# facebook/facebook360_dep

Hardware: AMD Instinct MI355X
Metric: depth Mpix/s per GPU (full pyramid, 16-cam 2048^2 rig); % HBM-read roofline (higher is better)
Workload: dtype f32+f64; 1 GPU; BASELINE config 3: 16-camera 2048x2048 synthetic rig, 8-frame sequence, full 10-level pyramid per frame, per-level temporal filter (+-2 frames); the same sequence for every --gpus N (block partition, 8 frame(s) on this rank); rig=cfg2, cameras=16, frames=8, temporal_filter=True, halo_transport=local, parallelism=frames x1

## Files before the change

__graft_entry__.py:

```python
import os
import subprocess
import sys

ROOT = os.path.dirname(os.path.abspath(__file__))
CSRC = os.path.join(ROOT, "facebook360_dep_amd", "csrc")
LIB = os.path.join(ROOT, "facebook360_dep_amd", "libderp_hip.so")
HIPCC = os.environ.get("HIPCC", "/opt/rocm/bin/hipcc")
HIP_FLAGS = ["--offload-arch=gfx950", "-O3", "-std=c++17", "-ffp-contract=off", "-fno-slp-vectorize", "-fPIC", "-shared"]


def _stale(target, sources):
    if not os.path.exists(target):
        return True
    t = os.path.getmtime(target)
    return any(os.path.getmtime(s) > t for s in sources)


def build_hip(force=False):
    srcs = [os.path.join(CSRC, f) for f in ("derp_capi.hip", "derp_host.h", "derp_ctx.h", "derp_kernels.h", "derp_render.h", "derp_points.h", "derp_mesh.h", "derp_mesh_math.h", "derp_camera.h", "gcc_algos.h", "derp_render_api.h", "derp_rephoto_api.h", "derp_points_api.h", "derp_mesh_api.h", "derp_filters_api.h", "derp_debug_api.h", "derp_sequence.h", "derp_isp.h", "derp_sim.h", "derp_sim_math.h", "derp_geometric.h", "derp_geometric_api.h", "derp_sweep.h", "derp_sweep_api.h", "derp_align.h", "derp_align_api.h")]
    srcs.append(os.path.join(ROOT, "include", "derp_hip.h"))
    host = os.path.join(CSRC, "derp_images.cpp")
    simplify = os.path.join(CSRC, "derp_simplify.cpp")
    scene = os.path.join(CSRC, "derp_sim_scene.cpp")
    srcs += [host, simplify, scene, os.path.join(ROOT, "facebook360_dep_amd", "cli", "image_codecs.h")]
    if force or _stale(LIB, srcs):
        subprocess.check_call([HIPCC] + HIP_FLAGS + ["-o", LIB, os.path.join(CSRC, "derp_capi.hip"), host, simplify, scene, "-lz", "-ldl"])
    cli = os.path.join(ROOT, "facebook360_dep_amd", "cli")
    if os.path.isdir(cli) and os.path.exists(os.path.join(cli, "Makefile")):
        subprocess.check_call(["make", "-s", "-C", cli])
    return LIB


def build():
    build_hip()
    sys.path.insert(0, ROOT)
    from oracle import oracle_lib

    oracle_lib.build()
    import facebook360_dep_amd
    from facebook360_dep_amd import derp

    derp.lib()


def smoke():
    sys.path.insert(0, ROOT)
    import numpy as np

    from facebook360_dep_amd import derp, synth
    from tests import common

    n, res, widths = synth.config("tiny")
    rig = synth.make_rig(n, res)
    sizes = synth.level_sizes(res, res, widths)
    frame = synth.make_frame(rig, sizes)
    ref = common.oracle_pyramid(rig, sizes, frame, res, res, partial_coverage=True)
    g = derp.Derp(rig["cameras"], partial_coverage=1)
    print("smoke: device", g.device_name())
    g.set_pyramid(sizes, res, res)
    g.upload_frame(frame)
    g.process_pyramid()
    g.synchronize()
    worst = 0.0
    for d in range(n):
        got = g.download_disparity(0, d)
        bad, rel = common.compare_disparity(got, ref[0][d])
        worst = max(worst, rel)
        assert bad == 0, "smoke: %d pixels of camera %d differ from the oracle by more than 1e-4 relative" % (bad, d)
    print("smoke: OK, max relative disparity error vs oracle = %.3g" % worst)
    g.close()


if __name__ == "__main__":
    build()
    if len(sys.argv) > 1 and sys.argv[1] == "smoke":
        smoke()
```

facebook360_dep_amd/csrc/derp_capi.hip:

```cpp
#include <hip/hip_runtime.h>

#include <algorithm>
#include <cfloat>
#include <cmath>
#include <cstdarg>
#include <cstdio>
#include <cstdlib>
#include <cstring>
#include <map>
#include <memory>
#include <string>
#include <vector>

#include <rocprim/device/device_radix_sort.hpp>

#include "../../include/derp_hip.h"
#include "derp_host.h"
#include "derp_kernels.h"
#include "derp_mesh.h"
#include "derp_points.h"
#include "derp_render.h"
#include "derp_geometric.h"
#include "derp_sweep.h"
#include "derp_align.h"

using namespace derp;

#include "derp_ctx.h"

namespace {

struct Span {
  derp_ctx* c;
  int stage, level;
  hipEvent_t a = nullptr, b = nullptr;
  Span(derp_ctx* ctx, int st, int lv) : c(ctx), stage(st), level(lv) {
    if (c->profiling) {
      (void)hipEventCreate(&a);
      (void)hipEventCreate(&b);
      (void)hipEventRecord(a, c->stream);
    }
  }
  ~Span() {
    if (c->profiling && a) {
      (void)hipEventRecord(b, c->stream);
      c->spans.push_back({stage, level, a, b});
    }
  }
};

void drain_spans(derp_ctx* c) {
  for (auto& s : c->spans) {
    (void)hipEventSynchronize(s.b);
    float ms = 0;
    (void)hipEventElapsedTime(&ms, s.a, s.b);
    if (s.level >= 0 && s.level < kMaxLevels) {
      c->accMs[s.stage][s.level] += ms;
      c->accLaunch[s.stage][s.level] += 1;
    }
    (void)hipEventDestroy(s.a);
    (void)hipEventDestroy(s.b);
  }
  c->spans.clear();
}

size_t npx(const derp_ctx* c, int level) {
  return (size_t)c->LW[level] * c->LH[level];
}

unsigned long long* counter_slot(derp_ctx* c, int stage, int level) {
  return c->counters.as<unsigned long long>() + ((size_t)stage * kMaxLevels + level) * 4;
}

LevelView make_view(derp_ctx* c, int stage, int dst0, int nd) {
  LevelView V;
  const int L = c->cur;
  V.W = c->LW[L];
  V.H = c->LH[L];
  V.Wd = (double)V.W;
  V.Hd = (double)V.H;
  V.S = c->S;
  V.D = nd;
  V.level = L;
  V.numLevels = c->numLevels;
  V.dst0 = dst0;
  V.hasFg = c->opt.use_foreground_masks;
  const float scale = float(V.W) / c->heightFull;
  const float scaleVar = scale * scale;
  V.varNoiseFloor = std::max(c->opt.var_noise_floor * scaleVar, kMinVar);
  V.varHighThresh = c->opt.var_high_thresh;
  V.minDepthM = c->opt.min_depth_m;
  V.maxDepthM = c->opt.max_depth_m;
  V.randomProposals = c->opt.random_proposals;
  V.partialCoverage = c->opt.partial_coverage;
  V.xcdRotate = c->xcdRotate;
  V.camsSrc = c->camsSrc.as<Cam>();
  V.camsDst = c->camsDst.as<Cam>();
  V.dst2src = c->dst2src.as<int>();
  V.srcColor = c->frame().color[L].as<ushort4>();
  V.ownBias = c->w.ownBias.as<ushort4>();
  V.srcVar = c->w.srcVar.as<float>();
  V.srcFg = c->frame().fg[L].as<uint8_t>();
  V.rayDir = c->rayDir.as<double>();
  V.behind = c->behind.as<unsigned>();
  V.rayStride = (size_t)c->D * V.W * V.H;
  V.projWarp = c->projWarp.as<float2>();
  V.projColor = c->w.projColor.as<ushort4>();
  V.projBias = c->w.projBias.as<ushort4>();
  V.projColorT = c->w.projColorT.as<ushort4>();
  V.disparity = c->w.disparity.as<float>();
  V.cost = c->w.cost.as<float>();
  V.confidence = c->w.confidence.as<float>();
  V.bgDisp = c->frame().bg[L].as<float>();
  V.fovMask = c->fovMask.as<uint8_t>();
  V.pairCount = c->w.pairCount.as<uint8_t>();
  V.counters = counter_slot(c, stage, L);
#if DERP_BLOCK_TRACE
  V.blockTrace = nullptr;
#endif
  return V;
}
int block_trace_attach(derp_ctx* c, LevelView& V, int which, int gridX, int gridY) {
#if DERP_BLOCK_TRACE
  DevBuf& buf = c->blockTrace[which][V.level];
  const size_t bytes = (size_t)gridX * gridY * 2 * sizeof(unsigned long long);
  ALLOC(c, buf, bytes);
  HIPCHK(c, hipMemsetAsync(buf.as<unsigned long long>(), 0, bytes, c->stream));
  V.blockTrace = buf.as<unsigned long long>();
  c->blockTraceGrid[which][V.level][0] = gridX;
  c->blockTraceGrid[which][V.level][1] = gridY;
#else
  (void)c, (void)V, (void)which, (void)gridX, (void)gridY;
#endif
  return 0;
}

const dim3 kBlurBlk(64, 4, 1);
dim3 blur_grid(int ow, int oh, int planes) {
  return dim3((ow + 63) / 64, (oh + 4 * kBlurRows - 1) / (4 * kBlurRows), planes);
}

void lanczos_coeffs(float x, float* coeffs) {
  static const double s45 = 0.70710678118654752440084436210485;
  static const double cs[][2] = {{1, 0}, {-s45, -s45}, {0, 1}, {s45, -s45}, {-1, 0}, {s45, s45}, {0, -1}, {-s45, s45}};
  if (x < 1.1920928955078125e-07f) {
    for (int i = 0; i < 8; i++) {
      coeffs[i] = 0;
    }
    coeffs[3] = 1;
    return;
  }
  float sum = 0;
  const double y0 = -(x + 3) * M_PI * 0.25, s0 = std::sin(y0), c0 = std::cos(y0);
  for (int i = 0; i < 8; i++) {
    const double y = -(x + 3 - i) * M_PI * 0.25;
    coeffs[i] = (float)((cs[i][0] * s0 + cs[i][1] * c0) / (y * y));
    sum += coeffs[i];
  }
  sum = 1.f / sum;
  for (int i = 0; i < 8; i++) {
    coeffs[i] *= sum;
  }
}

int get_lanczos(derp_ctx* c, int ssize, int dsize, LanczosTab** out) {
  auto key = std::make_pair(ssize, dsize);
  auto it = c->lanczos.find(key);
  if (it != c->lanczos.end()) {
    *out = &it->second;
    return 0;
  }
  std::vector<int> ofs(dsize);
  std::vector<float> coef((size_t)dsize * 8);
  const double scale = (double)ssize / dsize;
  for (int d = 0; d < dsize; ++d) {
    float f = (float)((d + 0.5) * scale - 0.5);
    int s = (int)f;
    s -= (s > f);
    f -= s;
    ofs[d] = s;
    lanczos_coeffs(f, &coef[(size_t)d * 8]);
  }
  LanczosTab t;
  for (int d0 = 0; d0 < dsize; d0 += kLanczosH) {
    const int d1 = std::min(d0 + kLanczosH, dsize) - 1;
    const int lo = std::min(std::max(ofs[d0] - 3, 0), ssize - 1), hi = std::min(std::max(ofs[d1] + 4, 0), ssize - 1);
    t.tileSpan = std::max(t.tileSpan, hi - lo + 1);
    t.monotone = t.monotone && std::is_sorted(ofs.begin() + d0, ofs.begin() + d1 + 1);
  }
  ALLOC(c, t.ofs, ofs.size() * sizeof(int));
  ALLOC(c, t.coef, coef.size() * sizeof(float));
  HIPCHK(c, hipMemcpyAsync(t.ofs.p, ofs.data(), ofs.size() * sizeof(int), hipMemcpyHostToDevice, c->stream));
  HIPCHK(c, hipMemcpyAsync(t.coef.p, coef.data(), coef.size() * sizeof(float), hipMemcpyHostToDevice, c->stream));
  HIPCHK(c, hipStreamSynchronize(c->stream));
  *out = &(c->lanczos[key] = std::move(t));
  return 0;
}

int get_area_tab(derp_ctx* c, int ssize, int dsize, AreaTabDev** out, bool forceTable = false) {
  auto key = std::make_pair(forceTable ? -ssize : ssize, dsize);
  auto it = c->areaTabs.find(key);
  if (it != c->areaTabs.end()) {
    *out = &it->second;
    return 0;
  }
  AreaTabDev t;
  const double scale = (double)ssize / dsize;
  const int iscale = (int)std::nearbyint(scale);
  std::vector<int> start(dsize + 1, 0), si;
  std::vector<float> alpha;
  if (!forceTable && iscale >= 1 && std::abs(scale - iscale) < 2.220446049250313e-16) {
    t.iscale = iscale;
  } else {
    for (int dx = 0; dx < dsize; ++dx) {
      start[dx] = (int)si.size();
      const double fsx1 = dx * scale, fsx2 = fsx1 + scale;
      const double cellWidth = std::min(scale, ssize - fsx1);
      int sx1 = (int)std::ceil(fsx1), sx2 = (int)std::floor(fsx2);
      sx2 = std::min(sx2, ssize - 1);
      sx1 = std::min(sx1, sx2);
      if (sx1 - fsx1 > 1e-3) {
        si.push_back(sx1 - 1);
        alpha.push_back((float)((sx1 - fsx1) / cellWidth));
      }
      for (int sx = sx1; sx < sx2; ++sx) {
        si.push_back(sx);
        alpha.push_back(float(1.0 / cellWidth));
      }
      if (fsx2 - sx2 > 1e-3) {
        si.push_back(sx2);
        alpha.push_back((float)(std::min(std::min(fsx2 - sx2, 1.), cellWidth) / cellWidth));
      }
    }
    start[dsize] = (int)si.size();
  }
  if (si.empty()) {
    si.push_back(0);
    alpha.push_back(0.f);
  }
  ALLOC(c, t.start, start.size() * sizeof(int));
  ALLOC(c, t.si, si.size() * sizeof(int));
  ALLOC(c, t.alpha, alpha.size() * sizeof(float));
  HIPCHK(c, hipMemcpy(t.start.p, start.data(), start.size() * sizeof(int), hipMemcpyHostToDevice));
  HIPCHK(c, hipMemcpy(t.si.p, si.data(), si.size() * sizeof(int), hipMemcpyHostToDevice));
  HIPCHK(c, hipMemcpy(t.alpha.p, alpha.data(), alpha.size() * sizeof(float), hipMemcpyHostToDevice));
  *out = &(c->areaTabs[key] = std::move(t));
  return 0;
}

int resize_area_dev(derp_ctx* c, int kind, const void* src, int sw, int sh, void* dst, int dw, int dh, int threshold) {
  if (dw > sw || dh > sh) {
    if (kind < 2 || kind == 4) {
      return fail(c, "pyramid levels must not be larger than the full-size frame (%dx%d -> %dx%d)", sw, sh, dw, dh);
    }
    const dim3 g = grid2d(dw, dh, 1, kBlk2d);
    if (kind == 3) {
      hipLaunchKernelGGL(k_resize_linear_area_f32<3>, g, kBlk2d, 0, c->stream, (const float*)src, sw, sh, (float*)dst, dw, dh);
    } else {
      hipLaunchKernelGGL(k_resize_linear_area_f32<1>, g, kBlk2d, 0, c->stream, (const float*)src, sw, sh, (float*)dst, dw, dh);
    }
    KCHECK(c);
    return 0;
  }
  AreaTabDev *tx, *ty;
  TRY(get_area_tab(c, sw, dw, &tx));
  TRY(get_area_tab(c, sh, dh, &ty));
  if ((tx->iscale > 0) != (ty->iscale > 0)) {
    if (tx->iscale > 0) {
      TRY(get_area_tab(c, sw, dw, &tx, true));
    } else {
      TRY(get_area_tab(c, sh, dh, &ty, true));
    }
  }
  AreaAxis ax{tx->start.as<int>(), tx->si.as<int>(), tx->alpha.as<float>(), tx->iscale};
  AreaAxis ay{ty->start.as<int>(), ty->si.as<int>(), ty->alpha.as<float>(), ty->iscale};
  const dim3 g = grid2d(dw, dh, 1, kBlk2d);
  if (kind == 0) {
    hipLaunchKernelGGL(k_resize_area<0>, g, kBlk2d, 0, c->stream, src, sw, sh, dst, dw, dh, ax, ay, threshold);
  } else if (kind == 1) {
    hipLaunchKernelGGL(k_resize_area<1>, g, kBlk2d, 0, c->stream, src, sw, sh, dst, dw, dh, ax, ay, threshold);
  } else if (kind == 3) {
    hipLaunchKernelGGL(k_resize_area<3>, g, kBlk2d, 0, c->stream, src, sw, sh, dst, dw, dh, ax, ay, threshold);
  } else if (kind == 4) {
    hipLaunchKernelGGL(k_resize_area<4>, g, kBlk2d, 0, c->stream, src, sw, sh, dst, dw, dh, ax, ay, threshold);
  } else {
    hipLaunchKernelGGL(k_resize_area<2>, g, kBlk2d, 0, c->stream, src, sw, sh, dst, dw, dh, ax, ay, threshold);
  }
  KCHECK(c);
  return 0;
}

std::vector<int2> make_spiral(int w) {
  int x = 0, y = 0, dx = 0, dy = -1, t = w;
  const int samples = t * t;
  std::vector<int2> locs;
  for (int i = 0; i < samples; ++i) {
    const bool vx = (-w / 2 <= x) && (x <= w / 2), vy = (-w / 2 <= y) && (y <= w / 2);
    if (vx && vy) {
      locs.push_back(make_int2(x, y));
    }
    if (x == y || ((x < 0) && (x == -y)) || ((x > 0) && (x == 1 - y))) {
      t = dx;
      dx = -dy;
      dy = t;
    }
    x += dx;
    y += dy;
  }
  return locs;
}

int ensure_spiral(derp_ctx* c, int radius) {
  if (c->spiralRadius == radius) {
    return 0;
  }
  const std::vector<int2> s = make_spiral(radius * 2 + 1);
  ALLOC(c, c->spiral, s.size() * sizeof(int2));
  HIPCHK(c, hipMemcpy(c->spiral.p, s.data(), s.size() * sizeof(int2), hipMemcpyHostToDevice));
  c->spiralN = (int)s.size();
  c->spiralRadius = radius;
  return 0;
}

int upsample_lanczos_dev(derp_ctx* c, const float* in, int sw, int sh, float* out, int dw, int dh, int planes,
                         size_t inStride, size_t outStride) {
  if (sw == dw && sh == dh) {
    return fail(c, "upsample to identical size not supported");
  }
  LanczosTab *tx, *ty;
  TRY(get_lanczos(c, sw, dw, &tx));
  TRY(get_lanczos(c, sh, dh, &ty));
  if (ty->monotone && ty->tileSpan <= kLanczosRows) {
    hipLaunchKernelGGL(k_lanczos, dim3((dw + kLanczosW - 1) / kLanczosW, (dh + kLanczosH - 1) / kLanczosH, planes),
                       dim3(kLanczosW, 4), 0, c->stream, in, sw, sh, dw, dh, tx->ofs.as<int>(), tx->coef.as<float>(),
                       ty->ofs.as<int>(), ty->coef.as<float>(), out, inStride, outStride);
    KCHECK(c);
    return 0;
  }
  const size_t tmpStride = (size_t)dw * sh;
  ALLOC(c, c->w.lanczosTmp, tmpStride * planes * sizeof(float));
  hipLaunchKernelGGL(k_lanczos_h, grid2d(dw, sh, planes, kBlk2d), kBlk2d, 0, c->stream, in, sw, sh, dw,
                     tx->ofs.as<int>(), tx->coef.as<float>(), c->w.lanczosTmp.as<float>(), inStride, tmpStride);
  KCHECK(c);
  hipLaunchKernelGGL(k_lanczos_v, grid2d(dw, dh, planes, kBlk2d), kBlk2d, 0, c->stream, c->w.lanczosTmp.as<float>(), sh,
                     dw, dh, ty->ofs.as<int>(), ty->coef.as<float>(), out, tmpStride, outStride);
  KCHECK(c);
  return 0;
}

int upsample_masked_dev(derp_ctx* c, const float* in, const uint8_t* mask, int sw, int sh, const uint8_t* maskUp,
                        const float* bgUp, float* out, int dw, int dh, int planes = 1) {
  const float scale = float(dw) / float(sw);
  const int radius = (int)(scale * scale + 1);
  TRY(ensure_spiral(c, radius));
  ALLOC(c, c->w.lanczosTmp, (size_t)dw * dh * planes * sizeof(float));
  hipLaunchKernelGGL(k_upsample_nearest_masked, grid2d(dw, dh, planes, kBlk2d), kBlk2d, 0, c->stream, in, mask, sw, sh,
                     maskUp, dw, dh, c->w.lanczosTmp.as<float>());
  KCHECK(c);
  hipLaunchKernelGGL(k_spiral_fill, grid2d(dw, dh, planes, kBlk2d), kBlk2d, 0, c->stream, c->w.lanczosTmp.as<float>(), bgUp,
                     maskUp, dw, dh, c->spiral.as<int2>(), c->spiralN, out);
  KCHECK(c);
  return 0;
}

bool batch_needs_inverse_warps(const derp_ctx* c, int dst0, int nd) {
  std::vector<char> covered(c->S, 0);
  for (int d = dst0; d < dst0 + nd; ++d) {
    covered[c->dst2srcH[d]] = 1;
  }
  for (int s = 0; s < c->S; ++s) {
    if (!covered[s]) {
      return true;
    }
  }
  return false;
}

size_t table_bytes_per_dst(const derp_ctx* c, int W, int H, bool withInverse) {
  const size_t wp = (size_t)(W + 2 * kPadW) * (H + 2 * kPadW), cp = (size_t)(W + 2 * kPadC) * (H + 2 * kPadC);
  return (size_t)(c->S - 1) * (wp * sizeof(float2) + 2 * cp * sizeof(ushort4) + (withInverse ? (size_t)W * H * sizeof(float2) : 0) +
                               (DERP_RANDOM_TILED ? tiled_plane(W, H) * sizeof(ushort4) : 0));
}

int compute_fov_and_masks(derp_ctx* c, int level) {
  const int W = c->LW[level], H = c->LH[level];
  const size_t n = (size_t)W * H;
  {
    Span sp(c, ST_FOV, level);
    if (c->opt.rebuild_warp_tables || c->fovCachedLevel != level) {
      hipLaunchKernelGGL(k_fov_mask, grid2d(W, H, c->D, kBlk2d), kBlk2d, 0, c->stream, c->camsDst.as<Cam>(), W, H,
                         c->fovMask.as<uint8_t>());
      KCHECK(c);
      c->fovCachedLevel = level;
    }
    hipLaunchKernelGGL(k_and_masks, dim3(flat_grid(n), c->D), dim3(256), 0, c->stream, c->fovMask.as<uint8_t>(),
                       c->frame().fg[level].as<uint8_t>(), c->dst2src.as<int>(), 0, n, c->w.maskAnd.as<uint8_t>());
    KCHECK(c);
  }
  return 0;
}

int build_warp(derp_ctx* c, int dst0, int nd) {
  const int L = c->cur;
  Span sp(c, ST_PROJ_WARP, L);
  {
    const size_t n = (size_t)c->LW[L] * c->LH[L];
    ALLOC(c, c->rayDir, 3 * n * c->D * sizeof(double));
    ALLOC(c, c->behind, n * c->D * sizeof(unsigned));
  }
  LevelView V = make_view(c, ST_PROJ_WARP, dst0, nd);
  hipLaunchKernelGGL(k_proj_warp, grid2d(V.W + 2 * kPadW, V.H + 2 * kPadW, c->S, kBlk2d), kBlk2d, 0, c->stream, V,
                     c->projWarp.as<float2>());
  KCHECK(c);
  hipLaunchKernelGGL(k_pixel_rays, grid2d(V.W, V.H, nd, kBlk2d), kBlk2d, 0, c->stream, V, c->rayDir.as<double>(),
                     c->behind.as<unsigned>());
  KCHECK(c);
  c->w.colorTablesCleanLevel = -1;
  if (batch_needs_inverse_warps(c, dst0, nd)) {
    hipLaunchKernelGGL(k_proj_warp_inv, grid2d(V.W, V.H, nd, kBlk2d), kBlk2d, 0, c->stream, V, c->projWarpInv.as<float2>());
    KCHECK(c);
  }
  return 0;
}

int build_color_tables(derp_ctx* c, int dst0, int nd) {
  const int L = c->cur;
  LevelView V = make_view(c, ST_REPROJECT, dst0, nd);
  Span sp(c, ST_REPROJECT, L);
  const dim3 grid((V.W + kRbTile - 1) / kRbTile, (V.H + kRbTile - 1) / kRbTile, nd * (c->S - 1));
  ALLOC(c, c->w.tileSeen, (size_t)grid.x * grid.y * grid.z);
  const int skipBlank = c->w.colorTablesCleanLevel == L && nd == c->D && !c->noBlankSkip;
  const auto kernel = c->reprojectSerial ? k_reproject_bias : k_reproject_bias_front;
  hipLaunchKernelGGL(kernel, grid, dim3(256), 0, c->stream, V, c->projWarpInv.as<float2>(),
                     c->w.projColor.as<ushort4>(), c->w.projBias.as<ushort4>(), c->w.projColorT.as<ushort4>(),
                     c->w.tileSeen.as<uint8_t>(), skipBlank);
  KCHECK(c);
  c->w.colorTablesCleanLevel = nd == c->D ? L : -1;
  return 0;
}

int tiles_of(int W, int H, int& tilesX) {
  constexpr int B = kTileBlock;
  tilesX = ((W + 15) / 16 + B - 1) / B * B;
  const int tilesY = ((H + 15) / 16 + B - 1) / B * B;
  return tilesX * tilesY * (256 / kCostBlock);
}
constexpr size_t kCostLdsPerSrc = (size_t)kCostBlock * sizeof(SsdPair);
struct CostGrid {
  int blocks, bands, perBlock;
};
constexpr int kCostMaxBands = 4, kCostMaxTilesPerBlock = 4;
int cost_grid_blocks(int tiles, int bands, int perBlock) {
  const int items = (tiles + perBlock - 1) / perBlock, unit = 8 * bands;
  return (items + unit - 1) / unit * unit;
}
CostGrid cost_grid(const derp_ctx* c, int tiles, int tilesX, bool spread) {
  const auto pow2_floor = [](int v, int cap) {
    int p = 1;
    while (p * 2 <= std::min(v, cap)) {
      p *= 2;
    }
    return p;
  };
  CostGrid g;
  g.perBlock = c->costTilesPerBlock > 0 ? pow2_floor(c->costTilesPerBlock, kCostMaxTilesPerBlock) : 1;
  const int rowOfSquares = tilesX * (256 / kCostBlock) * kTileBlock;
  g.bands = c->xcdBands > 0 ? pow2_floor(c->xcdBands, kCostMaxBands)
                            : spread ? pow2_floor(std::max(1, tiles / (8 * rowOfSquares)), kCostMaxBands) : 1;
  g.blocks = cost_grid_blocks(tiles, g.bands, g.perBlock);
  return g;
}
size_t lds_for_waves(size_t needed, int waves, size_t ldsPerCu, size_t fixed) {
  if (waves <= 0 || waves >= 4) {
    return needed;
  }
  const size_t perBlock = ldsPerCu / (size_t)(4 * waves + 1) + 256;
  return std::max(needed, perBlock > fixed ? perBlock - fixed : needed);
}
constexpr size_t kCostLdsStatic = sizeof(PatchWin) * (kCostBlock / 64) + kAtanLutDoubles * sizeof(double);
bool cost_four_waves(const derp_ctx* c) {
  if (const char* e = getenv("DERP_COST_WAVES")) {
    return atoi(e) >= 4;
  }
  return 16 * (kCostLdsPerSrc * (size_t)c->S + kCostLdsStatic) <= c->ldsPerCu && c->S <= 16;
}

int run_brute_force(derp_ctx* c, int dst0, int nd) {
  const int L = c->cur;
  if (L != c->numLevels - 1) {
    return 0;
  }
  Span sp(c, ST_BRUTE, L);
  LevelView V = make_view(c, ST_BRUTE, dst0, nd);
  const size_t n = (size_t)V.W * V.H;
  ALLOC(c, c->w.bruteCost, (size_t)nd * kNumDepths * n * sizeof(float));
  ALLOC(c, c->w.bruteConf, (size_t)nd * kNumDepths * n * sizeof(float));
  const int tilesX = std::max(1, (V.W - 2 + 7) / 8), tilesY = std::max(1, (V.H - 2 + 7) / 8);
  const int tiles = tilesX * tilesY;
  const size_t lds = kCostLdsPerSrc * (size_t)(c->S);
  const int run = std::min(std::max(c->bruteRun, 1), kNumDepths);
  hipLaunchKernelGGL(k_brute_costs, dim3(tiles, (kNumDepths + run - 1) / run, nd), dim3(kCostBlock), lds, c->stream, V,
                     c->w.bruteCost.as<float>(), c->w.bruteConf.as<float>(), tilesX, tiles, run);
  KCHECK(c);
  hipLaunchKernelGGL(k_brute_select, grid2d(V.W, V.H, nd, kBlk2d), kBlk2d, 0, c->stream, V, c->w.bruteCost.as<float>(),
                     c->w.bruteConf.as<float>());
  KCHECK(c);
  hipLaunchKernelGGL(k_brute_margin, grid2d(V.W, V.H, nd, kBlk2d), kBlk2d, 0, c->stream, V);
  KCHECK(c);
  return 0;
}

int run_random_proposals(derp_ctx* c, int dst0, int nd) {
  const int L = c->cur;
  if (c->opt.random_proposals <= 0 || L == c->numLevels - 1) {
    return 0;
  }
  Span sp(c, ST_RANDOM, L);
  c->randomRanThisLevel = true;
  LevelView V = make_view(c, ST_RANDOM, dst0, nd);
  if (V.H > 2 && V.W > 2) {
    WorkSet& w = c->w;
    if (w.rankPowersP != V.randomProposals || w.rankPowersN < V.W) {
      const int count = *std::max_element(c->LW.begin(), c->LW.end());
      ALLOC(c, w.rankPowers, (size_t)count * sizeof(uint32_t));
      hipLaunchKernelGGL(k_minstd_powers, dim3(blocks_of(count, 256)), dim3(256), 0, c->stream, V.randomProposals, count,
                         w.rankPowers.as<uint32_t>());
      KCHECK(c);
      w.rankPowersP = V.randomProposals;
      w.rankPowersN = count;
    }
    hipLaunchKernelGGL(k_row_rank, dim3(V.H - 2, nd), dim3(256), 0, c->stream, V, w.rankPowers.as<uint32_t>(),
                       w.rank.as<int>());
    KCHECK(c);
  }
  int tilesX;
  const int tiles = tiles_of(V.W, V.H, tilesX);
  const size_t lds = lds_for_waves(kCostLdsPerSrc * (size_t)(c->S), c->randomWaves, c->ldsPerCu, kCostLdsStatic);
  const CostGrid cg = cost_grid(c, tiles, tilesX, true);
  TRY(block_trace_attach(c, V, 0, cg.blocks, nd));
  const bool four = cost_four_waves(c);
  const auto kernel = cg.perBlock > 1 ? (four ? k_random_proposals_walk : k_random_proposals_walk_w3)
                                      : (four ? k_random_proposals : k_random_proposals_w3);
  hipLaunchKernelGGL(kernel, dim3(cg.blocks, nd), dim3(kCostBlock), lds, c->stream, V, c->w.rank.as<int>(), tilesX, cg.bands, cg.perBlock);
  KCHECK(c);
  return 0;
}

int run_ping_pong(derp_ctx* c, int dst0, int nd) {
  const int L = c->cur;
  if (L == c->numLevels - 1) {
    return 0;
  }
  Span sp(c, ST_PINGPONG, L);
  LevelView V = make_view(c, ST_PINGPONG, dst0, nd);
  const size_t n = (size_t)V.W * V.H;
  int tilesX;
  const int tiles = tiles_of(V.W, V.H, tilesX);
  const size_t lds = lds_for_waves(kCostLdsPerSrc * (size_t)(c->S), c->ppWaves, c->ldsPerCu, kCostLdsStatic);
  const bool four = cost_four_waves(c);
  const CostGrid cg = cost_grid(c, tiles, tilesX, false);
  const auto kernel = cg.perBlock > 1
                          ? (c->ppCompact ? (four ? k_ping_pong_walk : k_ping_pong_walk_w3) : (four ? k_ping_pong_loop_walk : k_ping_pong_loop_walk_w3))
                          : (c->ppCompact ? (four ? k_ping_pong : k_ping_pong_w3) : (four ? k_ping_pong_loop : k_ping_pong_loop_w3));
  TRY(block_trace_attach(c, V, 1, cg.blocks, nd));
  float* dispBuf[2] = {c->w.disparity.as<float>(), c->w.dispRes.as<float>()};
  float* costBuf[2] = {c->w.cost.as<float>(), c->w.costRes.as<float>()};
  uint8_t* chgBuf[2] = {c->w.changed.as<uint8_t>(), c->w.changed.as<uint8_t>() + n * c->D};
  const int iterations = c->opt.ping_pong_iterations;
  for (int it = 1; it <= iterations; ++it) {
    const int from = (it - 1) & 1, to = it & 1;
    V.disparity = dispBuf[from];
    V.cost = costBuf[from];
    hipLaunchKernelGGL(kernel, dim3(cg.blocks, nd), dim3(kCostBlock), lds, c->stream, V,
                       it == 1 ? (const uint8_t*)nullptr : chgBuf[from], chgBuf[to], dispBuf[to], costBuf[to], tilesX,
                       (int)(it == 1 && c->randomRanThisLevel && !c->noMemo), cg.bands, cg.perBlock);
    KCHECK(c);
  }
  if (dst0 + nd >= c->D) {
    if (iterations > 0 && (iterations & 1)) {
      std::swap(c->w.disparity, c->w.dispRes);
      std::swap(c->w.cost, c->w.costRes);
    }
    c->randomRanThisLevel = false;
  }
  return 0;
}

int run_mismatches(derp_ctx* c) {
  const int L = c->cur;
  if (L > c->opt.mismatches_start_level || L == c->numLevels - 1) {
    return 0;
  }
  if (c->D != c->S) {
    return fail(c, "Check failed: rigDst.size() == rigSrc.size()  Mismatches only valid when considering all cameras");
  }
  for (int d = 0; d < c->D; ++d) {
    if (c->dst2srcH[d] != d) {
      return fail(c, "mismatch handling needs destinations in rig order (dst %d maps to src %d)", d, c->dst2srcH[d]);
    }
  }
  Span sp(c, ST_MISMATCH, L);
  c->randomRanThisLevel = false;
  LevelView V = make_view(c, ST_MISMATCH, 0, c->D);
  const size_t n = (size_t)V.W * V.H;
  hipLaunchKernelGGL(k_mismatch, dim3((V.W + 15) / 16, (V.H + 15) / 16, c->D), dim3(256), 256 * sizeof(float) * c->S,
                     c->stream, V, c->w.dispRes.as<float>(), c->w.mismatchMask.as<uint8_t>());
  KCHECK(c);
  HIPCHK(c, hipMemcpyAsync(c->w.disparity.p, c->w.dispRes.p, n * c->D * sizeof(float), hipMemcpyDeviceToDevice, c->stream));
  return 0;
}

int bilateral_radius(int level) {
  const float scale = std::pow(0.9f, level);
  return (int)std::max(std::ceil(5 * scale), float(1));
}

size_t bilateral_lds_bytes(int radius) {
  const size_t side = 16 + 2 * (size_t)radius;
  const size_t t = ((side + 15) & ~(size_t)15) * side;
  return t * 4 * sizeof(float) + ((t + 3) & ~(size_t)3);
}

constexpr size_t kBilateralMaxLds = 64 * 1024 - 256;

bool bilateral_fast_tap_ok(float sigma, float w0, float w1, float w2) {
  const float denom = 2.0f * (sigma * sigma);
  return w1 == 1.0f && w2 == 1.0f && w0 >= 0.0f && std::isfinite(w0) && denom > 0.0f && std::isfinite(denom);
}

bool temporal_fast_tap_ok(float sigma, float w0, float w1, float w2) {
  const float sig2 = sigma * sigma;
  const auto weight_ok = [](float w) { return w >= 0.0f && std::isfinite(w); };
  return weight_ok(w0) && weight_ok(w1) && weight_ok(w2) && sig2 > 0.0f && std::isfinite(sig2);
}

void launch_joint_bilateral_u16_tiled(derp_ctx* c, dim3 grid, const float* image, const void* guide, const uint8_t* mask,
                                      int W, int H, int radius, float sigma, float w0, float w1, float w2, float* out,
                                      size_t planeStride, size_t guideStride, const int* guideIndex) {
  const bool fast = bilateral_fast_tap_ok(sigma, w0, w1, w2) && bilateral_lds_bytes(radius) + 256 <= kBilateralMaxLds;
  const auto kernel = fast ? k_joint_bilateral<true, true> : k_joint_bilateral<true, false>;
  hipLaunchKernelGGL(kernel, grid, dim3(256), bilateral_lds_bytes(radius), c->stream, image, guide, mask, W, H, radius, sigma,
                     w0, w1, w2, out, planeStride, guideStride, guideIndex);
}

int run_bilateral(derp_ctx* c) {
  const int L = c->cur;
  Span sp(c, ST_BILATERAL, L);
  c->randomRanThisLevel = false;
  const int W = c->LW[L], H = c->LH[L];
  const size_t n = (size_t)W * H;
  const int radius = bilateral_radius(L);
  launch_joint_bilateral_u16_tiled(c, dim3((W + 15) / 16, (H + 15) / 16, c->D), c->w.disparity.as<float>(),
                                   (const void*)c->frame().color[L].as<ushort4>(), c->w.maskAnd.as<uint8_t>(), W, H, radius,
                                   0.005f, 0.5f, 1.0f, 1.0f, c->w.tmpF.as<float>(), n, n, c->dst2src.as<int>());
  KCHECK(c);
  std::swap(c->w.disparity, c->w.tmpF);
  return 0;
}

int run_median(derp_ctx* c, bool fuseMaskFov, float* levelOut = nullptr) {
  const int L = c->cur;
  Span sp(c, ST_MEDIAN, L);
  c->randomRanThisLevel = false;
  const int W = c->LW[L], H = c->LH[L];
  const size_t n = (size_t)W * H;
  hipLaunchKernelGGL(k_masked_median, grid2d(W, H, c->D, kBlk2d), kBlk2d, 0, c->stream, c->w.disparity.as<float>(),
                     c->opt.use_foreground_masks ? c->frame().bg[L].as<float>() : (const float*)nullptr,
                     c->w.maskAnd.as<uint8_t>(), W, H, 1, levelOut ? levelOut : c->w.tmpF.as<float>(), n,
                     fuseMaskFov ? c->fovMask.as<uint8_t>() : (const uint8_t*)nullptr);
  KCHECK(c);
  if (!levelOut) {
    std::swap(c->w.disparity, c->w.tmpF);
  }
  return 0;
}

int run_mask_fov(derp_ctx* c, float* levelOut = nullptr) {
  const int L = c->cur;
  Span sp(c, ST_MASKFOV, L);
  const size_t n = npx(c, L) * c->D;
  hipLaunchKernelGGL(k_mask_fov, dim3(flat_grid(n)), dim3(256), 0, c->stream, c->w.disparity.as<float>(),
                     c->fovMask.as<uint8_t>(), levelOut ? levelOut : c->w.disparity.as<float>(), n);
  KCHECK(c);
  return 0;
}

int check_level(derp_ctx* c, int level) {
  if (!c || c->numLevels == 0) {
    return fail(c, "derp_set_pyramid has not been called");
  }
  if (level < 0 || level >= c->numLevels) {
    return fail(c, "level %d out of range [0, %d)", level, c->numLevels);
  }
  if (c->LW[level] <= 0 || c->LH[level] <= 0) {
    return fail(c, "level %d was declared absent in derp_set_pyramid", level);
  }
  return 0;
}

int level_begin(derp_ctx* c, int level, bool buildAllTables) {
  TRY(check_level(c, level));
  if (c->S - 1 > kMaxSrc) {
    return fail(c, "too many source cameras (%d > %d)", c->S, kMaxSrc + 1);
  }
  c->cur = level;
  const int W = c->LW[level], H = c->LH[level];
  const size_t n = (size_t)W * H;
  if (W < 3 || H < 3) {
    return fail(c, "level %d is too small (%dx%d)", level, W, H);
  }
  TRY(compute_fov_and_masks(c, level));
  {
    Span sp(c, ST_VARIANCE, level);
    hipLaunchKernelGGL(k_variance_bias, blur_grid(W, H, c->S), kBlurBlk, 0, c->stream, c->frame().color[level].as<ushort4>(),
                       W, H, c->w.srcVar.as<float>(), c->w.ownBias.as<ushort4>());
    KCHECK(c);
  }
  HIPCHK(c, hipMemsetAsync(c->w.cost.p, 0, n * c->D * sizeof(float), c->stream));
  HIPCHK(c, hipMemsetAsync(c->w.confidence.p, 0, n * c->D * sizeof(float), c->stream));
  c->w.mismatchMaskHeld = level <= c->opt.mismatches_start_level && level != c->numLevels - 1;
  if (c->w.mismatchMaskHeld) {
    HIPCHK(c, hipMemsetAsync(c->w.mismatchMask.p, 0, n * c->D, c->stream));
  }
  if (level < c->numLevels - 1 && !c->frame().haveDisp[level + 1] && !buildAllTables) {
    return fail(c, "Missing disparity of level %d needed to start level %d", level + 1, level);
  }
  if (level < c->numLevels - 1 && c->frame().haveDisp[level + 1]) {
    Span sp(c, ST_UPSAMPLE, level);
    const int sw = c->LW[level + 1], sh = c->LH[level + 1];
    if (!c->opt.use_foreground_masks) {
      TRY(upsample_lanczos_dev(c, c->frame().disp[level + 1].as<float>(), sw, sh, c->w.disparity.as<float>(), W, H, c->D,
                               (size_t)sw * sh, n));
    } else {
      ALLOC(c, c->w.staging, (size_t)sw * sh * c->D);
      hipLaunchKernelGGL(k_fov_mask, grid2d(sw, sh, c->D, kBlk2d), kBlk2d, 0, c->stream, c->camsDst.as<Cam>(), sw, sh,
                         c->w.staging.as<uint8_t>());
      KCHECK(c);
      hipLaunchKernelGGL(k_and_masks, dim3(flat_grid((size_t)sw * sh), c->D), dim3(256), 0, c->stream,
                         c->w.staging.as<uint8_t>(), c->frame().fg[level + 1].as<uint8_t>(), c->dst2src.as<int>(), 0,
                         (size_t)sw * sh, c->w.staging.as<uint8_t>());
      KCHECK(c);
      TRY(upsample_masked_dev(c, c->frame().disp[level + 1].as<float>(), c->w.staging.as<uint8_t>(), sw, sh,
                              c->w.maskAnd.as<uint8_t>(), c->frame().bg[level].as<float>(), c->w.disparity.as<float>(), W, H, c->D));
    }
  } else {
    HIPCHK(c, hipMemsetAsync(c->w.disparity.p, 0, n * c->D * sizeof(float), c->stream));
  }
  const bool invAll = batch_needs_inverse_warps(c, 0, c->D);
  size_t per = table_bytes_per_dst(c, W, H, invAll);
  int DB = c->D;
  bool needInv = invAll;
  {
    const size_t wpAll = (size_t)(W + 2 * kPadW) * (H + 2 * kPadW) * (c->S - 1) * c->D * sizeof(float2);
    const size_t cpAll = (size_t)(W + 2 * kPadC) * (H + 2 * kPadC) * (c->S - 1) * c->D * sizeof(ushort4);
    const size_t ipAll = (size_t)W * H * (c->S - 1) * c->D * sizeof(float2);
    const bool resident = c->projWarp.bytes >= wpAll && c->w.projColor.bytes >= cpAll && c->w.projBias.bytes >= cpAll &&
        (!invAll || c->projWarpInv.bytes >= ipAll) && !getenv("DERP_TABLE_BUDGET_GB") &&
        (!DERP_RANDOM_TILED || c->w.projColorT.bytes >= tiled_plane(W, H) * (c->S - 1) * c->D * sizeof(ushort4));
    if (!resident) {
      size_t freeB = 0, totalB = 0;
      HIPCHK(c, hipMemGetInfo(&freeB, &totalB));
      size_t budget = freeB + c->projWarp.bytes + c->w.projColor.bytes + c->w.projBias.bytes + c->projWarpInv.bytes + c->w.projColorT.bytes;
      if (const char* e = getenv("DERP_TABLE_BUDGET_GB")) {
        budget = std::min<size_t>(budget, (size_t)(atof(e) * (1ull << 30)));
      } else {
        budget = (size_t)(budget * 0.85);
      }
      DB = (int)std::min<size_t>((size_t)c->D, budget / std::max<size_t>(per, 1));
      if (DB < c->D && !needInv) {
        needInv = true;
        per = table_bytes_per_dst(c, W, H, true);
        DB = (int)std::min<size_t>((size_t)c->D, budget / std::max<size_t>(per, 1));
      }
      if (DB < 1) {
        return fail(c, "projection tables for one destination (%zu bytes) exceed the table budget (%zu bytes)", per, budget);
      }
      const int batches = (c->D + DB - 1) / DB;
      DB = (c->D + batches - 1) / batches;
    }
  }
  c->DB = DB;
  const size_t wp = (size_t)(W + 2 * kPadW) * (H + 2 * kPadW), cp = (size_t)(W + 2 * kPadC) * (H + 2 * kPadC);
  ALLOC(c, c->projWarp, (size_t)DB * (c->S - 1) * wp * sizeof(float2));
  ALLOC(c, c->w.projColor, (size_t)DB * (c->S - 1) * cp * sizeof(ushort4));
  ALLOC(c, c->w.projBias, (size_t)DB * (c->S - 1) * cp * sizeof(ushort4));
  if (needInv) {
    ALLOC(c, c->projWarpInv, (size_t)DB * (c->S - 1) * n * sizeof(float2));
  }
  if (DERP_RANDOM_TILED) {
    ALLOC(c, c->w.projColorT, (size_t)DB * (c->S - 1) * tiled_plane(W, H) * sizeof(ushort4));
  }
  c->tablesValid = false;
  c->randomRanThisLevel = false;
  if (buildAllTables) {
    if (DB < c->D) {
      return fail(c, "stage-level API needs all destinations' tables resident (batch %d < %d)", DB, c->D);
    }
    if (c->opt.rebuild_warp_tables || c->warpCachedLevel != level) {
      TRY(build_warp(c, 0, c->D));
      c->warpCachedLevel = level;
    }
  }
  return 0;
}

int level_end(derp_ctx* c) {
  const int L = c->cur;
  HIPCHK(c, hipMemcpyAsync(c->frame().disp[L].p, c->w.disparity.p, npx(c, L) * c->D * sizeof(float),
                           hipMemcpyDeviceToDevice, c->stream));
  c->frame().haveDisp[L] = 1;
  return 0;
}

int process_level(derp_ctx* c, int level) {
  TRY(level_begin(c, level, false));
  for (int d0 = 0; d0 < c->D; d0 += c->DB) {
    const int nd = std::min(c->DB, c->D - d0);
    const bool single = (c->DB == c->D);
    if (!single || c->opt.rebuild_warp_tables || c->warpCachedLevel != level) {
      TRY(build_warp(c, d0, nd));
      c->warpCachedLevel = single ? level : -1;
    }
    TRY(build_color_tables(c, d0, nd));
    TRY(run_brute_force(c, d0, nd));
    TRY(run_random_proposals(c, d0, nd));
    TRY(run_ping_pong(c, d0, nd));
  }
  TRY(run_mismatches(c));
  if (c->opt.do_bilateral_filter) {
    TRY(run_bilateral(c));
  }
  float* levelOut = c->frame().disp[level].as<float>();
  if (c->opt.do_median_filter) {
    TRY(run_median(c, true, levelOut));
  } else {
    TRY(run_mask_fov(c, levelOut));
  }
  c->frame().haveDisp[level] = 1;
  return 0;
}

int need_current(derp_ctx* c, bool tables) {
  if (!c || c->cur < 0) {
    return fail(c, "derp_level_begin has not been called");
  }
  if (tables && !c->tablesValid) {
    return fail(c, "derp_stage_reproject_colors must run before this stage");
  }
  return 0;
}

template <typename T>
int upload_tmp(derp_ctx* c, DevBuf& buf, const T* host, size_t count) {
  ALLOC(c, buf, count * sizeof(T));
  HIPCHK(c, hipMemcpyAsync(buf.p, host, count * sizeof(T), hipMemcpyHostToDevice, c->stream));
  return 0;
}

int alloc_pyramid(derp_ctx* c, FramePyramid& f) {
  const int num_levels = c->numLevels;
  f.color.resize(num_levels);
  f.fg.resize(num_levels);
  f.bg.resize(num_levels);
  f.disp.resize(num_levels);
  f.haveBg.assign(num_levels, 0);
  f.haveDisp.assign(num_levels, 0);
  for (int l = 0; l < num_levels; ++l) {
    const size_t n = npx(c, l);
    if (n == 0) {
      continue;
    }
    ALLOC(c, f.color[l], n * c->S * sizeof(ushort4));
    ALLOC(c, f.fg[l], n * c->S);
    ALLOC(c, f.bg[l], n * c->D * sizeof(float));
    ALLOC(c, f.disp[l], n * c->D * sizeof(float));
    HIPCHK(c, hipMemsetAsync(f.fg[l].p, 1, n * c->S, c->stream));
    HIPCHK(c, hipMemsetAsync(f.bg[l].p, 0, n * c->D * sizeof(float), c->stream));
  }
  return 0;
}

int alloc_work_set(derp_ctx* c, WorkSet& w, size_t n) {
  ALLOC(c, w.srcVar, n * c->S * sizeof(float));
  ALLOC(c, w.ownBias, n * c->S * sizeof(ushort4));
  ALLOC(c, w.maskAnd, n * c->D);
  for (DevBuf* b : {&w.disparity, &w.cost, &w.confidence, &w.dispRes, &w.costRes, &w.tmpF, &w.rank}) {
    ALLOC(c, *b, n * c->D * sizeof(float));
  }
  ALLOC(c, w.changed, 2 * n * c->D);
  ALLOC(c, w.mismatchMask, n * c->D);
  ALLOC(c, w.pairCount, n * c->D);
  return 0;
}

int select_frame(derp_ctx* c, int slot) {
  if (slot < 0 || slot >= (int)c->frames.size()) {
    return fail(c, "frame slot %d out of range [0, %d)", slot, (int)c->frames.size());
  }
  if (slot != c->curSlot) {
    c->curSlot = slot;
    c->cur = -1;
  }
  return 0;
}

void lane_swap(derp_ctx* c, int i) {
  std::swap(c->stream, c->lanes[i]->stream);
  std::swap(c->w, c->lanes[i]->w);
}

int lanes_prepare(derp_ctx* c, int count, size_t n) {
  while ((int)c->lanes.size() < count) {
    c->lanes.emplace_back(new WorkLane);
    WorkLane& l = *c->lanes.back();
    if (hipStreamCreateWithFlags(&l.stream, hipStreamNonBlocking) != hipSuccess ||
        hipEventCreateWithFlags(&l.done, hipEventDisableTiming) != hipSuccess) {
      return fail(c, "work lane: hipStreamCreate / hipEventCreate failed");
    }
  }
  if (!c->laneReady) {
    HIPCHK(c, hipEventCreateWithFlags(&c->laneReady, hipEventDisableTiming));
  }
  for (int i = 0; i < count; ++i) {
    TRY(alloc_work_set(c, c->lanes[i]->w, n));
  }
  return 0;
}

int process_level_on_lane(derp_ctx* c, int i, int slot, int level) {
  if (i < 0) {
    TRY(select_frame(c, slot));
    return process_level(c, level);
  }
  HIPCHK(c, hipStreamWaitEvent(c->lanes[i]->stream, c->laneReady, 0));
  lane_swap(c, i);
  c->activeLane = i;
  int rc = select_frame(c, slot);
  if (!rc) {
    rc = process_level(c, level);
  }
  if (!rc && hipEventRecord(c->lanes[i]->done, c->stream) != hipSuccess) {
    rc = fail(c, "work lane: hipEventRecord failed");
  }
  lane_swap(c, i);
  c->activeLane = -1;
  c->cur = -1;
  return rc;
}

int temporal_launch(derp_ctx* c, const void* const* guides, const float* const* images, const uint8_t* const* masks, int n,
                    int centre, int W, int H, int planes, float sigma, int radius, float w0, float w1, float w2,
                    float* out, const int* dst2src) {
  if (n < 1 || centre < 0 || centre >= n) {
    return fail(c, "temporal window must hold at least the centre frame");
  }
  if (n > kMaxTemporalFrames) {
    ALLOC(c, c->temporalCarry, (size_t)planes * W * H * sizeof(float2));
  }
  for (int t0 = 0; t0 < n; t0 += kMaxTemporalFrames) {
    TemporalFrames F;
    F.n = std::min(kMaxTemporalFrames, n - t0);
    for (int t = 0; t < F.n; ++t) {
      F.guides[t] = reinterpret_cast<const ushort4*>(guides[t0 + t]);
      F.images[t] = images[t0 + t];
      F.masks[t] = masks[t0 + t];
    }
    F.refGuide = reinterpret_cast<const ushort4*>(guides[centre]);
    F.refImage = images[centre];
    F.refMask = masks[centre];
    F.carry = n > kMaxTemporalFrames ? c->temporalCarry.as<float2>() : nullptr;
    F.first = t0 == 0;
    F.last = t0 + F.n >= n;
    const size_t lds = 2 * ((((size_t)(32 + 2 * radius) * (8 + 2 * radius) * 9) + 15) & ~(size_t)15);
    if (radius >= 0 && lds <= 48 * 1024 && !c->noTemporalTile) {
      const bool fast = temporal_fast_tap_ok(sigma, w0, w1, w2) && !c->temporalGeneric;
      const auto kernel = !fast ? k_temporal_tiled<-1, false> : radius == 1 ? k_temporal_tiled<1, true> : k_temporal_tiled<-1, true>;
      hipLaunchKernelGGL(kernel, grid2d(W, H, planes, kBlk2d), kBlk2d, lds, c->stream, F, W, H, sigma, radius, w0, w1, w2, out,
                         dst2src);
    } else {
      hipLaunchKernelGGL(k_temporal, grid2d(W, H, planes, kBlk2d), kBlk2d, 0, c->stream, F, W, H, sigma, radius, w0, w1, w2,
                         out, dst2src);
    }
    KCHECK(c);
  }
  return 0;
}

}

extern "C" {

void derp_options_default(derp_options* o) {
  o->min_depth_m = 0.5f;
  o->max_depth_m = 1e4f;
  o->var_noise_floor = 4e-5f;
  o->var_high_thresh = 1e-3f;
  o->random_proposals = 2;
  o->ping_pong_iterations = 1;
  o->mismatches_start_level = -1;
  o->do_bilateral_filter = 1;
  o->do_median_filter = 1;
  o->use_foreground_masks = 0;
  o->partial_coverage = 0;
  o->rebuild_warp_tables = 1;
}

int derp_create(derp_ctx** out, int device, const derp_camera_desc* src, int n_src, const derp_camera_desc* dst,
                int n_dst) {
  if (!out) {
    return 1;
  }
  *out = nullptr;
  std::unique_ptr<derp_ctx> owner(new derp_ctx);
  derp_ctx* c = owner.get();
  derp_options_default(&c->opt);
  if (n_src <= 0 || n_dst <= 0) {
    return create_fail("no source / destination cameras!");
  }
  hipDeviceProp_t prop;
  TRY(open_device(device, "the depth path", &prop));
  c->device = device;
  if (prop.maxSharedMemoryPerMultiProcessor > 0) {
    c->ldsPerCu = prop.maxSharedMemoryPerMultiProcessor;
  }
  if (const char* e = getenv("DERP_XCD_ROTATE")) {
    c->xcdRotate = atoi(e);
  }
  if (const char* e = getenv("DERP_XCD_BANDS")) {
    c->xcdBands = atoi(e);
// ... 80 lines not shown
  (void)hipSetDevice(c->device);
  (void)hipStreamSynchronize(c->stream);
  for (auto& l : c->lanes) {
    (void)hipStreamSynchronize(l->stream);
  }
  drain_spans(c);
  for (auto& l : c->lanes) {
    (void)hipStreamDestroy(l->stream);
    (void)hipEventDestroy(l->done);
  }
  if (c->laneReady) {
    (void)hipEventDestroy(c->laneReady);
  }
  (void)hipStreamDestroy(c->stream);
  (void)hipStreamDestroy(c->copyStream);
  delete c;
}

const char* derp_last_error(const derp_ctx* c) {
  return c ? c->err.c_str() : g_create_error.c_str();
}

int derp_set_options(derp_ctx* c, const derp_options* o) {
  if (!c || !o) {
    return 1;
  }
  if (o->random_proposals < 0) {
    return fail(c, "Check failed: random_proposals >= 0");
  }
  c->opt = *o;
  return 0;
}

int derp_set_pyramid(derp_ctx* c, int num_levels, const int* widths, const int* heights, int width_full,
                     int height_full) {
  if (!c) {
    return 1;
  }
  if (num_levels <= 0 || num_levels > kMaxLevels) {
    return fail(c, "num_levels %d out of range (1..%d)", num_levels, kMaxLevels);
  }
  HIPCHK(c, hipSetDevice(c->device));
  c->numLevels = num_levels;
  c->widthFull = width_full;
  c->heightFull = height_full;
  c->LW.assign(widths, widths + num_levels);
  c->LH.assign(heights, heights + num_levels);
  c->frames.clear();
  c->frames.resize(1);
  c->curSlot = 0;
  TRY(alloc_pyramid(c, c->frame()));
  size_t nmax = 0;
  for (int l = 0; l < num_levels; ++l) {
    nmax = std::max(nmax, npx(c, l));
  }
  TRY(alloc_work_set(c, c->w, nmax));
  ALLOC(c, c->fovMask, nmax * c->D);
  c->cur = -1;
  c->warpCachedLevel = -1;
  c->fovCachedLevel = -1;
  HIPCHK(c, hipStreamSynchronize(c->stream));
  return 0;
}

int derp_set_frame_slots(derp_ctx* c, int n_slots) {
  if (!c || c->numLevels == 0) {
    return fail(c, "derp_set_pyramid has not been called");
  }
  if (n_slots < 1 || n_slots > 4096) {
    return fail(c, "n_slots %d out of range (1..4096)", n_slots);
  }
  HIPCHK(c, hipSetDevice(c->device));
  TRY(select_frame(c, 0));
  const int had = (int)c->frames.size();
  c->frames.resize(n_slots);
  for (int k = had; k < n_slots; ++k) {
    TRY(alloc_pyramid(c, c->frames[k]));
  }
  HIPCHK(c, hipStreamSynchronize(c->stream));
  return 0;
}

int derp_select_frame(derp_ctx* c, int slot) {
  if (!c || c->numLevels == 0) {
    return fail(c, "derp_set_pyramid has not been called");
  }
  return select_frame(c, slot);
}

int derp_frame_slots(const derp_ctx* c, int* n_slots, int* selected) {
  if (!c) {
    return 1;
  }
  if (n_slots) {
    *n_slots = (int)c->frames.size();
  }
  if (selected) {
    *selected = c->curSlot;
  }
  return 0;
}

int derp_bind_thread(derp_ctx* c) {
  return use_device(c);
}
void* derp_host_alloc(size_t bytes) {
  void* p = nullptr;
  if (bytes == 0 || hipHostMalloc(&p, bytes, hipHostMallocDefault) != hipSuccess) {
    (void)hipGetLastError();
    return nullptr;
  }
  return p;
}
void derp_host_free(void* p) {
  if (p) {
    (void)hipHostFree(p);
  }
}
int derp_host_register(void* p, size_t bytes) {
  if (!p || bytes == 0 || hipHostRegister(p, bytes, hipHostRegisterDefault) != hipSuccess) {
    (void)hipGetLastError();
    return 1;
  }
  return 0;
}
void derp_host_unregister(void* p) {
  if (p && hipHostUnregister(p) != hipSuccess) {
    (void)hipGetLastError();
  }
}

int derp_upload_color(derp_ctx* c, int level, int s, const uint16_t* bgr) {
  TRY(check_level(c, level));
  if (s < 0 || s >= c->S || !bgr) {
    return fail(c, "bad source index / null image");
  }
  HIPCHK(c, hipSetDevice(c->device));
  const size_t n = npx(c, level);
  TRY(upload_tmp(c, c->w.staging, bgr, n * 3));
  hipLaunchKernelGGL(k_bgr_to_bgrx, dim3(flat_grid(n)), dim3(256), 0, c->stream, c->w.staging.as<uint16_t>(),
                     c->frame().color[level].as<ushort4>() + (size_t)s * n, n);
  KCHECK(c);
  HIPCHK(c, hipStreamSynchronize(c->stream));
  return 0;
}

int derp_upload_foreground_mask(derp_ctx* c, int level, int s, const uint8_t* mask) {
  TRY(check_level(c, level));
  if (s < 0 || s >= c->S || !mask) {
    return fail(c, "bad source index / null mask");
  }
  HIPCHK(c, hipSetDevice(c->device));
  const size_t n = npx(c, level);
  HIPCHK(c, hipMemcpy(c->frame().fg[level].as<uint8_t>() + (size_t)s * n, mask, n, hipMemcpyHostToDevice));
  return 0;
}

int derp_upload_background_disparity(derp_ctx* c, int level, int d, const float* disp) {
  TRY(check_level(c, level));
  if (d < 0 || d >= c->D || !disp) {
    return fail(c, "bad destination index / null image");
  }
  HIPCHK(c, hipSetDevice(c->device));
  const size_t n = npx(c, level);
  HIPCHK(c, hipMemcpy(c->frame().bg[level].as<float>() + (size_t)d * n, disp, n * sizeof(float), hipMemcpyHostToDevice));
  c->frame().haveBg[level] = 1;
  return 0;
}

int derp_upload_disparity(derp_ctx* c, int level, int d, const float* disp) {
  TRY(check_level(c, level));
  if (d < 0 || d >= c->D || !disp) {
    return fail(c, "bad destination index / null image");
  }
  HIPCHK(c, hipSetDevice(c->device));
  const size_t n = npx(c, level);
  HIPCHK(c, hipMemcpy(c->frame().disp[level].as<float>() + (size_t)d * n, disp, n * sizeof(float), hipMemcpyHostToDevice));
  c->frame().haveDisp[level] = 1;
  return 0;
}

int derp_process_level(derp_ctx* c, int level) {
  TRY(use_device(c));
  return process_level(c, level);
}

int derp_process_pyramid(derp_ctx* c, int level_start, int level_end_) {
  TRY(use_device(c));
  if (level_start < level_end_) {
    return fail(c, "Check failed: level_start >= level_end (%d vs %d)", level_start, level_end_);
  }
  for (int level = level_start; level >= level_end_; --level) {
    TRY(process_level(c, level));
  }
  return 0;
}

int derp_synchronize(derp_ctx* c) {
  if (!c) {
    return 1;
  }
  HIPCHK(c, hipStreamSynchronize(c->stream));
  if (c->numLevels > 0 && !c->opt.partial_coverage && !c->opt.use_foreground_masks) {
    unsigned long long v[4];
    HIPCHK(c, hipMemcpy(v, counter_slot(c, ST_BRUTE, c->numLevels - 1), sizeof v, hipMemcpyDeviceToHost));
    if (v[2] != 0) {
      return fail(c, "Check failed: partialCoverage || useForegroundMasks  Insufficient coverage at %llu pixels", v[2]);
    }
  }
  return 0;
}

int derp_download_disparity(derp_ctx* c, int level, int d, float* disparity) {
  TRY(check_level(c, level));
  if (d < 0 || d >= c->D || !disparity) {
    return fail(c, "bad destination index / null output");
  }
  if (!c->frame().haveDisp[level]) {
    return fail(c, "level %d has not been processed", level);
  }
  const size_t n = npx(c, level);
  return download_sync(c, disparity, c->frame().disp[level].as<float>() + (size_t)d * n, n * sizeof(float));
}

int derp_download_cost(derp_ctx* c, int d, float* cost, float* confidence) {
  TRY(need_current(c, false));
  if (d < 0 || d >= c->D) {
    return fail(c, "bad destination index");
  }
  HIPCHK(c, hipStreamSynchronize(c->stream));
  const size_t n = npx(c, c->cur);
  if (cost) {
    HIPCHK(c, hipMemcpy(cost, c->w.cost.as<float>() + (size_t)d * n, n * sizeof(float), hipMemcpyDeviceToHost));
  }
  if (confidence) {
    HIPCHK(c, hipMemcpy(confidence, c->w.confidence.as<float>() + (size_t)d * n, n * sizeof(float), hipMemcpyDeviceToHost));
  }
  return 0;
}

int derp_level_begin(derp_ctx* c, int level) {
  TRY(use_device(c));
  return level_begin(c, level, true);
}
int derp_stage_reproject_colors(derp_ctx* c) {
  TRY(need_current(c, false));
  TRY(build_color_tables(c, 0, c->D));
  c->tablesValid = true;
  return 0;
}
int derp_stage_brute_force(derp_ctx* c) {
  TRY(need_current(c, true));
  return run_brute_force(c, 0, c->D);
}
int derp_stage_random_proposals(derp_ctx* c) {
  TRY(need_current(c, true));
  return run_random_proposals(c, 0, c->D);
}
int derp_stage_ping_pong(derp_ctx* c) {
  TRY(need_current(c, true));
  return run_ping_pong(c, 0, c->D);
}
int derp_stage_mismatches(derp_ctx* c) {
  TRY(need_current(c, false));
  return run_mismatches(c);
}
int derp_stage_bilateral_filter(derp_ctx* c) {
  TRY(need_current(c, false));
  return run_bilateral(c);
}
int derp_stage_median_filter(derp_ctx* c) {
  TRY(need_current(c, false));
  return run_median(c, false);
}
int derp_stage_mask_fov(derp_ctx* c) {
  TRY(need_current(c, false));
  return run_mask_fov(c);
}
int derp_level_end(derp_ctx* c) {
  TRY(need_current(c, false));
  return level_end(c);
}
int derp_set_level_disparity(derp_ctx* c, int d, const float* disp) {
  TRY(need_current(c, false));
  if (d < 0 || d >= c->D || !disp) {
    return fail(c, "bad destination index / null image");
  }
  const size_t n = npx(c, c->cur);
  HIPCHK(c, hipStreamSynchronize(c->stream));
  HIPCHK(c, hipMemcpy(c->w.disparity.as<float>() + (size_t)d * n, disp, n * sizeof(float), hipMemcpyHostToDevice));
  c->randomRanThisLevel = false;
  return 0;
}
int derp_get_level_disparity(derp_ctx* c, int d, float* disp) {
  TRY(need_current(c, false));
  if (d < 0 || d >= c->D || !disp) {
    return fail(c, "bad destination index / null output");
  }
  const size_t n = npx(c, c->cur);
  return download_sync(c, disp, c->w.disparity.as<float>() + (size_t)d * n, n * sizeof(float));
}

int derp_cost_map(derp_ctx* c, int d, const float* disp, float* cost, float* confidence) {
  TRY(need_current(c, true));
  if (d < 0 || d >= c->D || !disp || !cost || !confidence) {
    return fail(c, "bad arguments");
  }
  const int L = c->cur;
  const size_t n = npx(c, L);
  TRY(upload_tmp(c, c->w.staging, disp, n));
  ALLOC(c, c->w.stagingB, 2 * n * sizeof(float));
  HIPCHK(c, hipMemsetAsync(c->w.stagingB.p, 0xff, 2 * n * sizeof(float), c->stream));
  LevelView V = make_view(c, ST_PINGPONG, 0, c->D);
  int tilesX;
  const int tiles = tiles_of(V.W, V.H, tilesX);
  const size_t lds = kCostLdsPerSrc * (size_t)(c->S);
  hipLaunchKernelGGL(k_cost_map, dim3(tiles), dim3(kCostBlock), lds, c->stream, V, d, c->w.staging.as<float>(),
                     c->w.stagingB.as<float>(), c->w.stagingB.as<float>() + n, tilesX);
  KCHECK(c);
  HIPCHK(c, hipStreamSynchronize(c->stream));
  HIPCHK(c, hipMemcpy(cost, c->w.stagingB.p, n * sizeof(float), hipMemcpyDeviceToHost));
  HIPCHK(c, hipMemcpy(confidence, c->w.stagingB.as<float>() + n, n * sizeof(float), hipMemcpyDeviceToHost));
  return 0;
}

static int build_pyramid(derp_ctx* c, int kind, int index, int count, const void* host, size_t elem, int w, int h,
                         int threshold) {
  if (!c || c->numLevels == 0) {
    return fail(c, "derp_set_pyramid has not been called");
  }
  if (index < 0 || index >= count || !host || w <= 0 || h <= 0) {
    return fail(c, "bad camera index / null image");
  }
  HIPCHK(c, hipSetDevice(c->device));
  const size_t n = (size_t)w * h;
  ALLOC(c, c->fullFrame, n * elem);
  HIPCHK(c, hipMemcpyAsync(c->fullFrame.p, host, n * elem, hipMemcpyHostToDevice, c->stream));
  for (int l = 0; l < c->numLevels; ++l) {
    const size_t nl = npx(c, l);
    if (nl == 0) {
      continue;
    }
    void* dst = kind == 0 ? (void*)(c->frame().color[l].as<ushort4>() + (size_t)index * nl)
        : kind == 1       ? (void*)(c->frame().fg[l].as<uint8_t>() + (size_t)index * nl)
                          : (void*)(c->frame().bg[l].as<float>() + (size_t)index * nl);
    TRY(resize_area_dev(c, kind, c->fullFrame.p, w, h, dst, c->LW[l], c->LH[l], threshold));
    if (kind == 2) {
      c->frame().haveBg[l] = 1;
    }
  }
  HIPCHK(c, hipStreamSynchronize(c->stream));
  return 0;
}
int derp_build_pyramid_color(derp_ctx* c, int src, const uint16_t* bgr, int w, int h) {
  return build_pyramid(c, 0, src, c ? c->S : 0, bgr, 6, w, h, -1);
}
int derp_build_pyramid_foreground_mask(derp_ctx* c, int src, const uint8_t* mask, int w, int h, int threshold) {
  return build_pyramid(c, 1, src, c ? c->S : 0, mask, 1, w, h, threshold);
}
int derp_build_pyramid_background_disparity(derp_ctx* c, int dst, const float* disp, int w, int h) {
  return build_pyramid(c, 2, dst, c ? c->D : 0, disp, 4, w, h, -1);
}
int derp_download_level_color(derp_ctx* c, int level, int src, uint16_t* bgr) {
  TRY(check_level(c, level));
  if (src < 0 || src >= c->S || !bgr) {
    return fail(c, "bad source index / null output");
  }
  const size_t n = npx(c, level);
  ALLOC(c, c->w.staging, n * 6);
  hipLaunchKernelGGL(k_bgrx_to_bgr, dim3(flat_grid(n)), dim3(256), 0, c->stream,
                     c->frame().color[level].as<ushort4>() + (size_t)src * n, c->w.staging.as<uint16_t>(), n);
  KCHECK(c);
  return download_sync(c, bgr, c->w.staging.p, n * 6);
}
int derp_download_level_mask(derp_ctx* c, int level, int src, uint8_t* mask) {
  TRY(check_level(c, level));
  if (src < 0 || src >= c->S || !mask) {
    return fail(c, "bad source index / null output");
  }
  const size_t n = npx(c, level);
  return download_sync(c, mask, c->frame().fg[level].as<uint8_t>() + (size_t)src * n, n);
}
int derp_download_level_background(derp_ctx* c, int level, int dst, float* disp) {
  TRY(check_level(c, level));
  if (dst < 0 || dst >= c->D || !disp) {
    return fail(c, "bad destination index / null output");
  }
  const size_t n = npx(c, level);
  return download_sync(c, disp, c->frame().bg[level].as<float>() + (size_t)dst * n, n * 4);
}
int derp_download_mismatch_mask(derp_ctx* c, int d, uint8_t* out) {
  TRY(need_current(c, false));
  if (d < 0 || d >= c->D || !out) {
    return fail(c, "bad destination index / null output");
  }
  const size_t n = npx(c, c->cur);
  if (!c->w.mismatchMaskHeld) {
    memset(out, 0, n);
    return 0;
  }
  return download_sync(c, out, c->w.mismatchMask.as<uint8_t>() + (size_t)d * n, n);
}

}

#include "derp_render_api.h"
#include "derp_rephoto_api.h"
#include "derp_points_api.h"
#include "derp_mesh_api.h"
#include "derp_geometric_api.h"
#include "derp_sweep_api.h"
#include "derp_align_api.h"
#include "derp_filters_api.h"
#include "derp_debug_api.h"
#include "derp_sequence.h"
#include "derp_isp.h"
#include "derp_sim.h"

derp_ctx::derp_ctx() = default;
derp_ctx::~derp_ctx() = default;
```

facebook360_dep_amd/csrc/derp_ctx.h:

```cpp
#pragma once

namespace {

enum Stage {
  ST_FOV = 0,
  ST_VARIANCE,
  ST_OWN_BIAS,
  ST_UPSAMPLE,
  ST_PROJ_WARP,
  ST_REPROJECT,
  ST_PROJ_BIAS,
  ST_BRUTE,
  ST_RANDOM,
  ST_PINGPONG,
  ST_MISMATCH,
  ST_BILATERAL,
  ST_MEDIAN,
  ST_MASKFOV,
  ST_TEMPORAL,
  ST_LANES,
  ST_GC_PREPARE,
  ST_GC_SWEEP,
  ST_GC_CLEAN,
  ST_SWEEP_OVERLAPS,
  ST_SWEEP_EQUIRECT,
  ST_ALIGN_MAPS,
  ST_ALIGN_COLORS,
  ST_COUNT
};
const char* kStageNames[ST_COUNT] = {"fov_mask",  "variance",    "own_bias",         "upsample",  "proj_warp",
                                     "reproject", "proj_bias",   "brute_force",      "random_proposals",
                                     "ping_pong", "mismatches",  "bilateral",        "median",    "mask_fov",
                                     "temporal",  "lanes_wall", "gc_prepare",       "gc_sweep",  "gc_clean",
                                     "sweep_overlaps", "sweep_equirect", "align_maps",       "align_colors"};
constexpr int kMaxLevels = 24;

struct TimedSpan {
  int stage, level;
  hipEvent_t a, b;
};

struct LanczosTab {
  DevBuf ofs, coef;
  int tileSpan = 0;
  bool monotone = true;
};

struct AreaTabDev {
  DevBuf start, si, alpha;
  int iscale = 0;
};

struct WorkSet {
  DevBuf srcVar, ownBias, maskAnd, disparity, cost, confidence, dispRes, costRes, changed, tmpF, rank, mismatchMask, pairCount;
  DevBuf rankPowers;
  int rankPowersP = -1, rankPowersN = 0;
  DevBuf tileSeen;
  DevBuf projColor, projBias;
  DevBuf projColorT;
  DevBuf bruteCost, bruteConf, lanczosTmp, staging, stagingB;
  bool mismatchMaskHeld = false;
  int colorTablesCleanLevel = -1;
};

struct FramePyramid {
  std::vector<DevBuf> color, fg, bg, disp;
  std::vector<char> haveBg, haveDisp;
};

struct WorkLane {
  hipStream_t stream = nullptr;
  hipEvent_t done = nullptr;
  WorkSet w;
};

struct SmrState; struct RephotoState; struct PointsState; struct MeshState; struct GcState; struct SweepState; struct AlignState;

}

struct derp_ctx {
  derp_ctx();
  ~derp_ctx();
  int device = 0;
  hipStream_t stream = nullptr;
  hipStream_t copyStream = nullptr;
  DevBuf copyStaging;
  std::string err;
  std::string* errSink() {
    return &err;
  }
  derp_options opt;
  int S = 0, D = 0;
  std::vector<Cam> camsSrcH, camsDstH;
  std::vector<int> dst2srcH;
  std::vector<derp_camera_desc> descDstH;
  DevBuf camsSrc, camsDst, dst2src;

  int numLevels = 0, widthFull = 0, heightFull = 0;
  std::vector<int> LW, LH;
  std::vector<FramePyramid> frames;
  int curSlot = 0;
  FramePyramid& frame() {
    return frames[curSlot];
  }
  DevBuf fullFrame;
  DevBuf devMask;

  int cur = -1;
  int DB = 0;
  WorkSet w;
  DevBuf temporalCarry;
  DevBuf projWarp, projWarpInv;
  DevBuf rayDir, behind;
  int warpCachedLevel = -1;
  DevBuf fovMask;
  int fovCachedLevel = -1;
  bool randomRanThisLevel = false;
  bool tablesValid = false;
  std::map<std::pair<int, int>, LanczosTab> lanczos;
  std::map<std::pair<int, int>, AreaTabDev> areaTabs;
  DevBuf spiral;
  int spiralN = 0, spiralRadius = -1;
  std::vector<std::unique_ptr<WorkLane>> lanes;
  hipEvent_t laneReady = nullptr;
  int activeLane = -1;

  DevBuf counters;
  bool profiling = false;
  std::vector<TimedSpan> spans;
  double accMs[ST_COUNT][kMaxLevels] = {};
  int accLaunch[ST_COUNT][kMaxLevels] = {};
  int xcdRotate = 1;
  int xcdBands = 0, costTilesPerBlock = 0;
  DevBuf blockTrace[2][kMaxLevels];
  int blockTraceGrid[2][kMaxLevels][2] = {};
  bool noMemo = false;
  int bruteRun = 10;
  bool ppCompact = true;
  int randomWaves = 0, ppWaves = 0;
  size_t ldsPerCu = 160 * 1024;
  bool noTemporalTile = false;
  bool noBlankSkip = false;
  bool temporalGeneric = false, reprojectSerial = false;
  std::unique_ptr<SmrState> smr;
  std::unique_ptr<RephotoState> rephoto;
  std::unique_ptr<PointsState> points;
  std::unique_ptr<MeshState> mesh;
  std::unique_ptr<GcState> gc;
  std::unique_ptr<SweepState> sweep;
  std::unique_ptr<AlignState> align;
};

namespace {

int fail(derp_ctx* c, const char* fmt, ...) {
  va_list ap;
  va_start(ap, fmt);
  vfail(c ? &c->err : nullptr, fmt, ap);
  va_end(ap);
  return 1;
}

int use_device(derp_ctx* c) {
  if (!c) {
    return 1;
  }
  HIPCHK(c, hipSetDevice(c->device));
  return 0;
}

int check_camera(derp_ctx* c, int cam) {
  if (cam < 0 || cam >= c->D) {
    return fail(c, "bad camera index %d (the context has %d)", cam, c->D);
  }
  return 0;
}

}
```

facebook360_dep_amd/csrc/derp_filters_api.h:

```cpp
#pragma once

int derp_resize_area(derp_ctx* c, int kind, const void* src, int w, int h, void* dst, int dw, int dh) {
  if (!c || !src || !dst || kind < 0 || kind > 3 || w <= 0 || h <= 0 || dw <= 0 || dh <= 0) {
    return fail(c, "bad arguments");
  }
  HIPCHK(c, hipSetDevice(c->device));
  const size_t elem = kind == 0 ? 6 : kind == 1 ? 1 : kind == 3 ? 12 : 4, n = (size_t)w * h, nd = (size_t)dw * dh;
  DevBuf in, out, out3;
  TRY(upload_sync(c, in, src, n * elem));
  ALLOC(c, out, nd * (kind == 0 ? 8 : elem));
  TRY(resize_area_dev(c, kind, in.p, w, h, out.p, dw, dh, -1));
  if (kind == 0) {
    ALLOC(c, out3, nd * 6);
    hipLaunchKernelGGL(k_bgrx_to_bgr, dim3(flat_grid(nd)), dim3(256), 0, c->stream, out.as<ushort4>(),
                       out3.as<uint16_t>(), nd);
  }
  return download_sync(c, dst, kind == 0 ? out3.p : out.p, nd * elem);
}

int derp_generate_foreground_mask(derp_ctx* c, const uint16_t* template_bgr, const uint16_t* frame_bgr, int w, int h,
                                  int blur_radius, float threshold, int morph_closing_size, uint8_t* mask01) {
  if (!c || !template_bgr || !frame_bgr || !mask01 || w <= 0 || h <= 0 || blur_radius < 0 || blur_radius > 3 ||
      morph_closing_size < 0 || !(threshold >= 0)) {
    return fail(c, "bad arguments (blur_radius must be 0..3)");
// ... 8 lines not shown
  hipLaunchKernelGGL(k_bgr_to_bgrx, dim3(flat_grid(n)), dim3(256), 0, c->stream, raw.as<uint16_t>(), t4.as<ushort4>(), n);
  HIPCHK(c, hipStreamSynchronize(c->stream));
  TRY(upload_sync(c, raw, frame_bgr, n * 6));
  hipLaunchKernelGGL(k_bgr_to_bgrx, dim3(flat_grid(n)), dim3(256), 0, c->stream, raw.as<uint16_t>(), f4.as<ushort4>(), n);
  const ushort4 *tp = t4.as<ushort4>(), *fp = f4.as<ushort4>();
  if (blur_radius > 0) {
    ALLOC(c, tb, n * 8);
    ALLOC(c, fb, n * 8);
    hipLaunchKernelGGL(k_gauss_u16, grid2d(w, h, 1, kBlk2d), kBlk2d, 0, c->stream, t4.as<ushort4>(), tb.as<ushort4>(), w, h, blur_radius);
    hipLaunchKernelGGL(k_gauss_u16, grid2d(w, h, 1, kBlk2d), kBlk2d, 0, c->stream, f4.as<ushort4>(), fb.as<ushort4>(), w, h, blur_radius);
    tp = tb.as<ushort4>();
    fp = fb.as<ushort4>();
  }
  hipLaunchKernelGGL(k_fg_threshold, dim3(flat_grid(n)), dim3(256), 0, c->stream, tp, fp, n, threshold, m0.as<uint8_t>());
  if (morph_closing_size > 0) {
    ALLOC(c, m1, n);
    hipLaunchKernelGGL(k_morph_rect, grid2d(w, h, 1, kBlk2d), kBlk2d, 0, c->stream, m0.as<uint8_t>(), m1.as<uint8_t>(), w, h, morph_closing_size, 1);
    hipLaunchKernelGGL(k_morph_rect, grid2d(w, h, 1, kBlk2d), kBlk2d, 0, c->stream, m1.as<uint8_t>(), m0.as<uint8_t>(), w, h, morph_closing_size, 0);
  }
  return download_sync(c, mask01, m0.p, n);
}

int derp_layer_disparities(derp_ctx* c, const float* foreground, const float* background, size_t n, uint8_t* out) {
  if (!c || !foreground || !background || !out) {
    return fail(c, "bad arguments");
  }
  HIPCHK(c, hipSetDevice(c->device));
  DevBuf f, b, o;
  TRY(upload_sync(c, f, foreground, n * 4));
  TRY(upload_sync(c, b, background, n * 4));
  ALLOC(c, o, n);
  hipLaunchKernelGGL(k_layer_disparities, dim3(flat_grid(n)), dim3(256), 0, c->stream, f.as<float>(), b.as<float>(), n,
                     o.as<uint8_t>());
  return download_sync(c, out, o.p, n);
}
int derp_fov_mask(derp_ctx* c, int d, int w, int h, uint8_t* out) {
  if (!c || !out || d < 0 || d >= c->D || w <= 0 || h <= 0) {
    return fail(c, "bad arguments");
  }
  HIPCHK(c, hipSetDevice(c->device));
  DevBuf m;
  ALLOC(c, m, (size_t)w * h);
  hipLaunchKernelGGL(k_fov_mask, grid2d(w, h, 1, kBlk2d), kBlk2d, 0, c->stream, c->camsDst.as<Cam>() + d, w, h,
                     m.as<uint8_t>());
  return download_sync(c, out, m.p, (size_t)w * h);
}

int derp_upsample_disparity(derp_ctx* c, int d, const float* disp, int w, int h, const float* bg_disp_up,
                            const uint8_t* fg_mask, const uint8_t* fg_mask_up, int w_up, int h_up, int use_fg,
                            float* out) {
  if (!c || !disp || !out || d < 0 || d >= c->D) {
    return fail(c, "bad arguments");
  }
  HIPCHK(c, hipSetDevice(c->device));
  const size_t n = (size_t)w * h, nu = (size_t)w_up * h_up;
  DevBuf in, res, m, mu, bg, fov, fovu, idx;
  TRY(upload_sync(c, in, disp, n * 4));
  ALLOC(c, res, nu * 4);
  if (!use_fg) {
    TRY(upsample_lanczos_dev(c, in.as<float>(), w, h, res.as<float>(), w_up, h_up, 1, n, nu));
    return download_sync(c, out, res.p, nu * 4);
  }
  if (!bg_disp_up || !fg_mask || !fg_mask_up) {
    return fail(c, "foreground-mask upsample needs bg_disp_up, fg_mask and fg_mask_up");
  }
  const int zero = 0;
  TRY(upload_sync(c, m, fg_mask, n));
  TRY(upload_sync(c, mu, fg_mask_up, nu));
  TRY(upload_sync(c, bg, bg_disp_up, nu * 4));
  TRY(upload_sync(c, idx, &zero, sizeof(int)));
  ALLOC(c, fov, n);
  ALLOC(c, fovu, nu);
  hipLaunchKernelGGL(k_fov_mask, grid2d(w, h, 1, kBlk2d), kBlk2d, 0, c->stream, c->camsDst.as<Cam>() + d, w, h,
                     fov.as<uint8_t>());
  hipLaunchKernelGGL(k_fov_mask, grid2d(w_up, h_up, 1, kBlk2d), kBlk2d, 0, c->stream, c->camsDst.as<Cam>() + d, w_up,
                     h_up, fovu.as<uint8_t>());
  hipLaunchKernelGGL(k_and_masks, dim3(flat_grid(n), 1), dim3(256), 0, c->stream, fov.as<uint8_t>(), m.as<uint8_t>(),
                     idx.as<int>(), 0, n, fov.as<uint8_t>());
  hipLaunchKernelGGL(k_and_masks, dim3(flat_grid(nu), 1), dim3(256), 0, c->stream, fovu.as<uint8_t>(), mu.as<uint8_t>(),
                     idx.as<int>(), 0, nu, fovu.as<uint8_t>());
  TRY(upsample_masked_dev(c, in.as<float>(), fov.as<uint8_t>(), w, h, fovu.as<uint8_t>(), bg.as<float>(), res.as<float>(),
                          w_up, h_up));
  return download_sync(c, out, res.p, nu * 4);
}

template <bool GUIDE_U16>
static void launch_joint_bilateral(derp_ctx* c, const float* image, const void* guide, const uint8_t* mask, int w, int h,
                                   int radius, float sigma, float w0, float w1, float w2, float* out) {
  const size_t n = (size_t)w * h;
  const dim3 grid((w + 15) / 16, (h + 15) / 16, 1);
  if (bilateral_lds_bytes(radius) <= kBilateralMaxLds) {
    if (GUIDE_U16) {
      launch_joint_bilateral_u16_tiled(c, grid, image, guide, mask, w, h, radius, sigma, w0, w1, w2, out, n, n, nullptr);
    } else {
      hipLaunchKernelGGL(k_joint_bilateral<false>, grid, dim3(256), bilateral_lds_bytes(radius), c->stream, image, guide,
                         mask, w, h, radius, sigma, w0, w1, w2, out, n, n, (const int*)nullptr);
    }
  } else {
    hipLaunchKernelGGL(k_joint_bilateral_direct<GUIDE_U16>, grid, dim3(256), 0, c->stream, image, guide, mask, w, h,
                       radius, sigma, w0, w1, w2, out);
  }
}

int derp_joint_bilateral_u16(derp_ctx* c, const float* image, const uint16_t* guide, const uint8_t* mask, int w, int h,
                             int radius, float sigma, float w0, float w1, float w2, float* out) {
  if (!c || !image || !guide || !mask || !out || w <= 0 || h <= 0 || radius < 0 || radius > (1 << 30)) {
    return fail(c, "bad arguments (radius must be in [0, 2^30])");
  }
  HIPCHK(c, hipSetDevice(c->device));
  const size_t n = (size_t)w * h;
  DevBuf im, g3, g4, m, res;
  TRY(upload_sync(c, im, image, n * 4));
  TRY(upload_sync(c, g3, guide, n * 6));
  TRY(upload_sync(c, m, mask, n));
  ALLOC(c, g4, n * 8);
  ALLOC(c, res, n * 4);
  hipLaunchKernelGGL(k_bgr_to_bgrx, dim3(flat_grid(n)), dim3(256), 0, c->stream, g3.as<uint16_t>(), g4.as<ushort4>(), n);
  launch_joint_bilateral<true>(c, im.as<float>(), (const void*)g4.as<ushort4>(), m.as<uint8_t>(), w, h, radius, sigma, w0,
                               w1, w2, res.as<float>());
  return download_sync(c, out, res.p, n * 4);
}

int derp_joint_bilateral_f32(derp_ctx* c, const float* image, const float* guide, const uint8_t* mask, int w, int h,
                             int radius, float sigma, float w0, float w1, float w2, float* out) {
  if (!c || !image || !guide || !mask || !out || w <= 0 || h <= 0 || radius < 0 || radius > (1 << 30)) {
    return fail(c, "bad arguments (radius must be in [0, 2^30])");
  }
  HIPCHK(c, hipSetDevice(c->device));
  const size_t n = (size_t)w * h;
  DevBuf im, g, m, res;
  TRY(upload_sync(c, im, image, n * 4));
  TRY(upload_sync(c, g, guide, n * 12));
  TRY(upload_sync(c, m, mask, n));
  ALLOC(c, res, n * 4);
  launch_joint_bilateral<false>(c, im.as<float>(), (const void*)g.as<float>(), m.as<uint8_t>(), w, h, radius, sigma, w0, w1,
                                w2, res.as<float>());
  return download_sync(c, out, res.p, n * 4);
}

int derp_masked_median(derp_ctx* c, const float* image, const float* background, const uint8_t* mask, int w, int h,
                       int radius, float* out) {
  if (!c || !image || !mask || !out || radius < 1 || radius > 2) {
    return fail(c, "bad arguments (radius must be 1 or 2)");
  }
  HIPCHK(c, hipSetDevice(c->device));
  const size_t n = (size_t)w * h;
  DevBuf im, bg, m, res;
  TRY(upload_sync(c, im, image, n * 4));
  if (background) {
    TRY(upload_sync(c, bg, background, n * 4));
  }
  TRY(upload_sync(c, m, mask, n));
  ALLOC(c, res, n * 4);
  hipLaunchKernelGGL(k_masked_median, grid2d(w, h, 1, kBlk2d), kBlk2d, 0, c->stream, im.as<float>(),
                     background ? bg.as<float>() : (const float*)nullptr, m.as<uint8_t>(), w, h, radius,
                     res.as<float>(), n, (const uint8_t*)nullptr);
  return download_sync(c, out, res.p, n * 4);
}

int derp_temporal_filter_dev(derp_ctx* c, const void* const* guides, const float* const* disps,
                             const uint8_t* const* masks, int n_frames, int w, int h, int frame_offset, float sigma,
                             int space_radius, float w0, float w1, float w2, float* out_dev) {
  if (!c || n_frames < 1 || frame_offset < 0 || frame_offset >= n_frames) {
    return fail(c, "temporal window must hold at least one frame and contain the centre frame");
  }
  HIPCHK(c, hipSetDevice(c->device));
  return temporal_launch(c, guides, disps, masks, n_frames, frame_offset, w, h, 1, sigma, space_radius, w0, w1, w2, out_dev,
                         nullptr);
}

int derp_temporal_filter(derp_ctx* c, const uint16_t* const* guides, const float* const* disps,
                         const uint8_t* const* masks, int n_frames, int w, int h, int frame_offset, float sigma,
                         int space_radius, float w0, float w1, float w2, float* out) {
  if (!c || n_frames < 1) {
    return fail(c, "temporal window must hold at least one frame");
  }
  HIPCHK(c, hipSetDevice(c->device));
  const size_t n = (size_t)w * h;
  std::vector<DevBuf> g4(n_frames), im(n_frames), m(n_frames);
  DevBuf g3, res;
  std::vector<const void*> gp(n_frames);
  std::vector<const float*> ip(n_frames);
  std::vector<const uint8_t*> mp(n_frames);
  for (int t = 0; t < n_frames; ++t) {
    ALLOC(c, g4[t], n * 8);
    TRY(upload_sync(c, g3, guides[t], n * 6));
    hipLaunchKernelGGL(k_bgr_to_bgrx, dim3(flat_grid(n)), dim3(256), 0, c->stream, g3.as<uint16_t>(),
                       g4[t].as<ushort4>(), n);
    HIPCHK(c, hipStreamSynchronize(c->stream));
    TRY(upload_sync(c, im[t], disps[t], n * 4));
    TRY(upload_sync(c, m[t], masks[t], n));
    gp[t] = g4[t].p;
    ip[t] = im[t].as<float>();
    mp[t] = m[t].as<uint8_t>();
  }
  ALLOC(c, res, n * 4);
  TRY(derp_temporal_filter_dev(c, gp.data(), ip.data(), mp.data(), n_frames, w, h, frame_offset, sigma, space_radius, w0,
                               w1, w2, res.as<float>()));
  return download_sync(c, out, res.p, n * 4);
}
```

facebook360_dep_amd/csrc/derp_kernels.h:

```cpp
#pragma once
#include <hip/hip_runtime.h>
#include <math.h>
#include <stdint.h>

#include <type_traits>

#include "derp_camera.h"
#include "gcc_algos.h"

namespace derp {

#ifndef DERP_COST_MIN_WAVES
#define DERP_COST_MIN_WAVES 4
#endif
#ifndef DERP_RANDOM_MIN_WAVES
#define DERP_RANDOM_MIN_WAVES 4
#endif
#ifndef DERP_RANDOM_TILED
#define DERP_RANDOM_TILED 0
#endif
#ifndef DERP_MIX_HOT_ONLY
#define DERP_MIX_HOT_ONLY 0
#endif
#ifndef DERP_PHASE_TIMERS
// ... 1359 lines not shown
        at32(pt, (unsigned)tiled_index(tilesX, x + kPadC, y + kPadC)) = col;
      }
      continue;
    }
    const int oya = y == 0 ? 0 : y + kPadC, oyb = y == H - 1 ? OH - 1 : y + kPadC;
    for (int oy = oya; oy <= oyb; ++oy) {
      for (int ox = oxa; ox <= oxb; ++ox) {
        const unsigned o = (unsigned)(oy * OW + ox);
        at32(pc, o) = col;
        at32(pb, o) = bia;
        if (pt) {
          at32(pt, (unsigned)tiled_index(tilesX, ox, oy)) = col;
        }
      }
    }
  }
}

__device__ __forceinline__ float probe_disparity(int i, float minD, float maxD) {
  const double fraction = (double)i / (double)(kNumDepths - 1);
  return (float)(fraction * (double)minD + (1 - fraction) * (double)maxD);
}

__global__ void __launch_bounds__(kCostBlock, DERP_COST_MIN_WAVES)
    k_brute_costs(LevelView V, float* __restrict__ costs, float* __restrict__ confs, int tilesX, int tilesPerDst, int run) {
  const int i0 = blockIdx.y * run, i1 = min(i0 + run, kNumDepths);
  const int dl = blockIdx.z;
  const int d = V.dst0 + dl;
  const int iw = V.W - 2, ih = V.H - 2;
  const int lane = threadIdx.x & 63;
  const int sx = (int)(blockIdx.x % (unsigned)tilesX), sy = (int)(blockIdx.x / (unsigned)tilesX);
  const int x = 1 + sx * 8 + (lane & 7), y = 1 + sy * 8 + (lane >> 3);
  PatchWin* win;
  LdsPairs pairs = cost_wave_prologue(V, d, x - (int)(threadIdx.x & 7), y - (int)((threadIdx.x & 63) >> 3), win);
  unsigned nCost = 0, nPair = 0;
  if (x <= iw && y <= ih) {
    const int own = V.dst2src[d];
    const size_t n = (size_t)V.W * V.H, idx = (size_t)y * V.W + x;
    const float minDisparity = 1.0f / V.maxDepthM, maxDisparity = 1.0f / V.minDepthM;
    const bool fov = V.fovMask[(size_t)d * n + idx], fg = V.srcFg[(size_t)own * n + idx];
    const float nan = __builtin_nanf("");
    if (fov && fg) {
      PixCtx px;
      load_pixctx<false>(V, d, own, x, y, win, px);
      const unsigned cull = behind_sources(V, d, idx);
      const unsigned xy = (unsigned)x | ((unsigned)y << 16);
      for (int i = i0; i < i1; ++i) {
        unsigned q = xy;
        asm("" : "+v"(q) : "s"(i));
        const unsigned pidx = (q >> 16) * (unsigned)V.W + (q & 0xffffu);
        const float disparity = probe_disparity(i, minDisparity, maxDisparity);
        const bool closer = V.hasFg ? ((V.bgDisp + (size_t)d * n)[pidx] < disparity) : true;
        float2 r = make_float2(nan, nan);
        if (closer) {
          unsigned np = 0;
          r = compute_cost<false, true>(V, dl, own, px, disparity, pairs, np, cull, pidx);
          nPair += np;
          ++nCost;
        }
        const size_t o = ((size_t)dl * kNumDepths + i) * n;
        (costs + o)[pidx] = r.x;
        (confs + o)[pidx] = r.y;
      }
    } else {
      for (int i = i0; i < i1; ++i) {
        const size_t o = ((size_t)dl * kNumDepths + i) * n + idx;
        costs[o] = nan;
        confs[o] = nan;
      }
    }
  }
  flush_counters(V, nCost, nPair);
}

__global__ void k_brute_select(LevelView V, const float* __restrict__ costs, const float* __restrict__ confs) {
  const int dl = blockIdx.z;
  const int d = V.dst0 + dl;
  const int x = blockIdx.x * blockDim.x + threadIdx.x, y = blockIdx.y * blockDim.y + threadIdx.y;
  if (x < 1 || y < 1 || x >= V.W - 1 || y >= V.H - 1) {
    return;
  }
  const int own = V.dst2src[d];
  const size_t n = (size_t)V.W * V.H, idx = (size_t)y * V.W + x;
  float* disp = V.disparity + (size_t)d * n;
  if (!V.fovMask[(size_t)d * n + idx]) {
    disp[idx] = __builtin_nanf("");
    return;
  }
  if (!V.srcFg[(size_t)own * n + idx]) {
    disp[idx] = V.bgDisp[(size_t)d * n + idx];
    return;
  }
  float minCost = 3.402823466e+38f, minConf = 0;
  int best = -1;
  for (int i = 0; i < kNumDepths; ++i) {
    const size_t o = ((size_t)dl * kNumDepths + i) * n + idx;
    const float c = costs[o];
    if (c < minCost) {
      minCost = c;
      minConf = confs[o];
      best = i;
    }
  }
  const float minDisparity = 1.0f / V.maxDepthM, maxDisparity = 1.0f / V.minDepthM;
  if (best == -1) {
    atomicAdd(&V.counters[2], 1ull);
    disp[idx] = minDisparity;
  } else {
    disp[idx] = probe_disparity(best, minDisparity, maxDisparity);
  }
  V.cost[(size_t)d * n + idx] = minCost;
  V.confidence[(size_t)d * n + idx] = minConf;
}

__global__ void k_brute_margin(LevelView V) {
  const int d = V.dst0 + blockIdx.z;
  const int x = blockIdx.x * blockDim.x + threadIdx.x, y = blockIdx.y * blockDim.y + threadIdx.y;
  if (x >= V.W || y >= V.H) {
    return;
  }
  if (!(x < 1 || x >= V.W - 1 || y < 1 || y >= V.H - 1)) {
    return;
  }
  const int own = V.dst2src[d];
  const size_t n = (size_t)V.W * V.H, idx = (size_t)y * V.W + x;
  if (!V.srcFg[(size_t)own * n + idx]) {
    V.disparity[(size_t)d * n + idx] = V.bgDisp[(size_t)d * n + idx];
    return;
  }
  const int yy = min(max(y, 1), V.H - 2), xx = min(max(x, 1), V.W - 2);
  const size_t src = (size_t)yy * V.W + xx;
  V.disparity[(size_t)d * n + idx] = V.disparity[(size_t)d * n + src];
  V.cost[(size_t)d * n + idx] = V.cost[(size_t)d * n + src];
  V.confidence[(size_t)d * n + idx] = V.confidence[(size_t)d * n + src];
}

__device__ __forceinline__ bool random_gate(const LevelView& V, int d, int own, size_t idx) {
  const size_t n = (size_t)V.W * V.H;
  if (!V.fovMask[(size_t)d * n + idx] || !V.srcFg[(size_t)own * n + idx]) {
    return false;
  }
  const float varHighDev = 0.1f * V.varHighThresh;
  const float thresh = fmaxf(varHighDev, V.varNoiseFloor);
  return !(V.srcVar[(size_t)own * n + idx] < thresh);
}

__global__ void k_minstd_powers(int proposals, int count, uint32_t* __restrict__ powers) {
  const int k = blockIdx.x * blockDim.x + threadIdx.x;
  if (k < count) {
    powers[k] = minstd_jump(1u, (uint64_t)proposals * (uint64_t)k);
  }
}

__global__ void __launch_bounds__(256) k_row_rank(LevelView V, const uint32_t* __restrict__ powers, int* __restrict__ rank) {
  __shared__ int waveCount[2][4];
  const int d = V.dst0 + blockIdx.y, y = blockIdx.x + 1;
  const int own = V.dst2src[d];
  const size_t n = (size_t)V.W * V.H;
  const int lane = threadIdx.x & 63, wave = threadIdx.x >> 6;
  const uint32_t seed = minstd_seed(y * V.level);
  int before = 0;
  for (int xb = 1, step = 0; xb < V.W - 1; xb += 256, ++step) {
    const int x = xb + (int)threadIdx.x;
    const size_t idx = (size_t)y * V.W + x;
    const bool go = x < V.W - 1 && random_gate(V, d, own, idx);
    const unsigned long long ballot = __ballot(go);
    if (lane == 0) {
      waveCount[step & 1][wave] = __popcll(ballot);
    }
    __syncthreads();
    int k = before + __popcll(ballot & ((1ull << lane) - 1ull));
#pragma unroll
    for (int w = 0; w < 4; ++w) {
      const int t = waveCount[step & 1][w];
      k += w < wave ? t : 0;
      before += t;
    }
    if (go) {
      rank[(size_t)d * n + idx] = (int)minstd_mulmod(seed, powers[k]);
    }
  }
}

__device__ __forceinline__ void random_proposals_tile(const LevelView& V, const int* __restrict__ rank, int dl, int x, int y, bool go,
                                                      const PatchWin* win, LdsPairs& pairs) {
  const int d = V.dst0 + dl;
  const int own = V.dst2src[d];
  const size_t n = (size_t)V.W * V.H;
  const unsigned idx = (unsigned)y * (unsigned)V.W + (unsigned)x;
  float* disp = V.disparity + (size_t)d * n;
  unsigned nCost = 0, nPair = 0, nSlots = 0, nSlotsFirst = 0;
  PhaseTimers tm;
  const unsigned tk0 = phase_clock();
  if (go) {
    PixCtx px;
    load_pixctx<false>(V, d, own, x, y, win, px);
    const unsigned cull = behind_sources(V, d, idx);
    float currDisp = at32(disp, idx);
    float currCost = 0.f, costThresh = 0.f, amplitude = 0.f;
    const int spare = V.S - 1;
    const float maxDisp = 1.0f / V.minDepthM;
    uint32_t state = (uint32_t)at32(rank + (size_t)d * n, idx);
    for (int i = -1; i < V.randomProposals; ++i) {
      unsigned pi = idx;
      asm("" : "+v"(pi) : "s"(i));
      const float minDisp = V.hasFg ? at32(V.bgDisp + (size_t)d * n, pi) : (1.0f / V.maxDepthM);
      float propDisp = currDisp;
      if (i >= 0) {
        const float lo = fmaxf(minDisp, currDisp - amplitude), hi = fminf(maxDisp, currDisp + amplitude);
        propDisp = minstd_uniform(state, lo, hi);
      }
      unsigned np = 0;
      const float2 pr = compute_cost<true, true>(V, dl, own, px, propDisp, pairs, np, cull, pi, i < 0 ? &nSlotsFirst : &nSlots, &tm);
      nPair += np;
      bool take;
      if (i < 0) {
        costThresh = fminf(0.5f * pr.x, 5.0f);
        amplitude = (maxDisp - minDisp) / 2.0f;
        take = true;
      } else {
        take = pr.x < currCost && pr.x < costThresh;
        if (take) {
          amplitude /= 2.0f;
        }
      }
      if (take) {
        currCost = pr.x;
        currDisp = propDisp;
        pairs.set(spare, SsdPair{pr.y, __uint_as_float(np)});
      }
    }
    {
      unsigned pi = idx;
      asm("" : "+v"(pi) : "v"(currCost));
      const SsdPair best = pairs.get(spare);
      at32(V.confidence + (size_t)d * n, pi) = best.first;
      at32(V.pairCount + (size_t)d * n, pi) = (uint8_t)__float_as_uint(best.second);
      at32(disp, pi) = currDisp;
      at32(V.cost + (size_t)d * n, pi) = currCost;
    }
    nCost = 1u + (unsigned)max(V.randomProposals, 0);
  }
#if DERP_PHASE_TIMERS
  if ((threadIdx.x & 63) == 0) {
    const unsigned body = phase_clock() - tk0;
    atomicAdd(&V.counters[0], (unsigned long long)(DERP_PHASE_TIMERS == 1 ? tm.proj : body));
    atomicAdd(&V.counters[1], (unsigned long long)(DERP_PHASE_TIMERS == 1 ? tm.ssd : body - tm.inside));
    atomicAdd(&V.counters[3], (unsigned long long)(DERP_PHASE_TIMERS == 1 ? tm.select : 0u));
  }
  return;
#endif
  flush_counters(V, nCost, nPair);
#ifdef DERP_COUNT_UNION
  atomicAdd(&V.counters[3], (unsigned long long)nSlots);
  atomicAdd(&V.counters[2], (unsigned long long)nSlotsFirst);
#endif
}

template <bool WALK>
__device__ __forceinline__ void random_proposals_body(const LevelView& V, const int* __restrict__ rank, int tilesX, int bands,
                                                      int perBlock) {
  const unsigned long long bt0 = block_trace_begin();
  const int steps = WALK ? perBlock : 1;
  const int dl = blockIdx.y;
  const int d = V.dst0 + dl;
  PatchWin* win;
  LdsPairs pairs = cost_block_prologue(win);
  bool lutReady = false;
  for (int step = 0; step < steps; ++step) {
    int x, y;
    tile_pixel(cost_block_tile(blockIdx.x, gridDim.x, V.xcdRotate ? d : 0, bands, steps, step), tilesX, x, y);
    bool go = false;
    if (x >= 1 && y >= 1 && x < V.W - 1 && y < V.H - 1) {
      const int own = V.dst2src[d];
      const size_t n = (size_t)V.W * V.H;
      const unsigned idx = (unsigned)y * (unsigned)V.W + (unsigned)x;
      if ((V.fovMask + (size_t)d * n)[idx]) {
        if (!(V.srcFg + (size_t)own * n)[idx]) {
          (V.disparity + (size_t)d * n)[idx] = (V.bgDisp + (size_t)d * n)[idx];
        } else {
          go = random_gate(V, d, own, idx);
        }
      }
    }
    if (__ballot(go) == 0ull) {
      continue;
    }
    cost_tile_prologue(V, d, x - (int)(threadIdx.x & 7), y - (int)((threadIdx.x & 63) >> 3), win, pairs, lutReady);
    random_proposals_tile(V, rank, dl, x, y, go, win, pairs);
  }
  block_trace_end(V, bt0);
}

__global__ void __launch_bounds__(kCostBlock, DERP_RANDOM_MIN_WAVES)
    k_random_proposals(LevelView V, const int* __restrict__ rank, int tilesX, int bands, int perBlock) {
  random_proposals_body<false>(V, rank, tilesX, bands, perBlock);
}
__global__ void __launch_bounds__(kCostBlock, 3)
    k_random_proposals_w3(LevelView V, const int* __restrict__ rank, int tilesX, int bands, int perBlock) {
  random_proposals_body<false>(V, rank, tilesX, bands, perBlock);
}
__global__ void __launch_bounds__(kCostBlock, DERP_RANDOM_MIN_WAVES)
    k_random_proposals_walk(LevelView V, const int* __restrict__ rank, int tilesX, int bands, int perBlock) {
  random_proposals_body<true>(V, rank, tilesX, bands, perBlock);
}
__global__ void __launch_bounds__(kCostBlock, 3)
    k_random_proposals_walk_w3(LevelView V, const int* __restrict__ rank, int tilesX, int bands, int perBlock) {
  random_proposals_body<true>(V, rank, tilesX, bands, perBlock);
}

__constant__ int kCandidates[9][2] = {{0, 0}, {-1, 0}, {1, 0}, {0, -1}, {0, 1}, {-2, -2}, {2, -2}, {-2, 2}, {2, 2}};
constexpr int kCandOff[9][2] = {{0, 0}, {-1, 0}, {1, 0}, {0, -1}, {0, 1}, {-2, -2}, {2, -2}, {-2, 2}, {2, 2}};
constexpr unsigned cand_pack(int c) {
  unsigned p = 0;
  for (int k = 0; k < 9; ++k) {
    p |= (unsigned)(kCandOff[k][c] + 2) << (3 * k);
  }
  return p;
}
constexpr unsigned kCandPackX = cand_pack(0), kCandPackY = cand_pack(1);

#ifdef DERP_COUNT_PP_FILL
__device__ __forceinline__ unsigned pp_fill_entry() {
  return __builtin_ctzll(__ballot(1)) == (int)(threadIdx.x & 63) ? 64u : 0u;
}
#endif

__device__ __forceinline__ void ping_pong_candidates_loop(const LevelView& V, const uint8_t* __restrict__ changed, int dl, int x,
                                                          int y, const PatchWin* win, LdsPairs& pairs, int useMemo, float& outDisp,
                                                          float& outCost, unsigned& counts, unsigned& fillSlots, PhaseTimers& tm) {
  const int d = V.dst0 + dl;
  const int own = V.dst2src[d];
// ... 452 lines not shown
}

template <bool GUIDE_U16>
__device__ __forceinline__ float4 bilateral_texel(const void* __restrict__ guideV, size_t j, float value) {
  if (GUIDE_U16) {
    const ushort4 g = reinterpret_cast<const ushort4*>(guideV)[j];
    const float factor = 1 / 65535.0f;
    return make_float4(g.x * factor, g.y * factor, g.z * factor, value);
  }
  const float* g = reinterpret_cast<const float*>(guideV) + j * 3;
  const float factor = 1 / 1.0f;
  return make_float4(g[0] * factor, g[1] * factor, g[2] * factor, value);
}

__device__ __forceinline__ void bilateral_tap(float4 centre, float4 t, float weight0, float weight1, float weight2,
                                              double rcpDenom, const unsigned long long* expTab, float& sumWeight,
                                              float& weightedAvg) {
  const float d0 = centre.x - t.x, d1 = centre.y - t.y, d2 = centre.z - t.z;
  const float colorDiffSq = weight0 * (d0 * d0) + weight1 * (d1 * d1) + weight2 * (d2 * d2);
  const float weight = expf_glibc(div_by_const(div_by_const(-colorDiffSq, 1.0 / 3.0), rcpDenom), expTab);
  sumWeight += weight;
  weightedAvg += weight * t.w;
}

__device__ __forceinline__ void bilateral_tap_fast(float4 centre, float4 t, float weight0, double rcpDenom,
                                                   const unsigned long long* expTab, float& sumWeight, float& weightedAvg) {
  const float d0 = centre.x - t.x, d1 = centre.y - t.y, d2 = centre.z - t.z;
  const float colorDiffSq = weight0 * (d0 * d0) + (d1 * d1) + (d2 * d2);
  const float weight = expf_glibc_nonpos(div_by_const(div_by_const(-colorDiffSq, 1.0 / 3.0), rcpDenom), expTab);
  sumWeight += weight;
  weightedAvg += weight * t.w;
}

template <bool GUIDE_U16, bool FAST_TAP = false>
__global__ void __launch_bounds__(256)
    k_joint_bilateral(const float* __restrict__ image, const void* __restrict__ guideV,
                      const uint8_t* __restrict__ mask, int W, int H, int radius, float sigma, float weight0,
                      float weight1, float weight2, float* __restrict__ out, size_t planeStride, size_t guideStride,
                      const int* __restrict__ guideIndex) {
  static_assert(GUIDE_U16 || !FAST_TAP, "the fast tap's range argument needs the u16 guide");
  extern __shared__ float ldsTile[];
  __shared__ unsigned long long expTab[32];
  if (threadIdx.x < 32) {
    expTab[threadIdx.x] = kExp2fTab[threadIdx.x];
  }
  const int p = blockIdx.z;
  const int T = 16 + 2 * radius;
  const int P = (T + 15) & ~15;
  const int n = P * T;
  float4* tTex = reinterpret_cast<float4*>(ldsTile);
  uint8_t* tMask = reinterpret_cast<uint8_t*>(ldsTile + 4 * n);
  const float* img = image + (size_t)p * planeStride;
  const uint8_t* m = mask + (size_t)p * planeStride;
  const size_t gplane = (size_t)(guideIndex ? guideIndex[p] : p) * guideStride;
  const int x0 = blockIdx.x * 16 - radius, y0 = blockIdx.y * 16 - radius;
  int staged = 1;
  for (int k = threadIdx.x; k < T * T; k += 256) {
    const int ty = k / T, tx = k - ty * T;
    const int i = ty * P + tx;
    const int sx = min(max(x0 + tx, 0), W - 1), sy = min(max(y0 + ty, 0), H - 1);
    const size_t j = (size_t)sy * W + sx;
    const uint8_t mk = m[j];
    staged &= mk != 0;
    tMask[i] = mk;
    tTex[i] = bilateral_texel<GUIDE_U16>(guideV, gplane + j, img[j]);
  }
  bool fullMask = false;
  if (FAST_TAP) {
    fullMask = __syncthreads_and(staged) != 0;
  } else {
    __syncthreads();
  }
  const int lx = threadIdx.x & 15, ly = threadIdx.x >> 4;
  const int x = blockIdx.x * 16 + lx, y = blockIdx.y * 16 + ly;
  if (x >= W || y >= H) {
    return;
  }
  const int c = (ly + radius) * P + lx + radius;
  const float4 centre = tTex[c];
  float result = centre.w;
  if (tMask[c]) {
    const float denom = 2.0f * (sigma * sigma);
    const double rcpDenom = 1.0 / (double)denom;
    float sumWeight = 0.f, weightedAvg = 0.f;
    if (FAST_TAP && fullMask) {
      for (int v = -radius; v <= radius; ++v) {
        const int row = c + v * P;
        for (int u = -radius; u <= radius; ++u) {
          bilateral_tap_fast(centre, tTex[row + u], weight0, rcpDenom, expTab, sumWeight, weightedAvg);
        }
      }
    } else {
      for (int v = -radius; v <= radius; ++v) {
        const int row = c + v * P;
        for (int u = -radius; u <= radius; ++u) {
          const int j = row + u;
          if (!tMask[j]) {
            continue;
          }
          if (FAST_TAP) {
            bilateral_tap_fast(centre, tTex[j], weight0, rcpDenom, expTab, sumWeight, weightedAvg);
          } else {
            bilateral_tap(centre, tTex[j], weight0, weight1, weight2, rcpDenom, expTab, sumWeight, weightedAvg);
          }
        }
      }
    }
    if (sumWeight != 0.0f) {
      result = weightedAvg / sumWeight;
    }
  }
  out[(size_t)p * planeStride + (size_t)y * W + x] = result;
}

template <bool GUIDE_U16>
__global__ void __launch_bounds__(256)
    k_joint_bilateral_direct(const float* __restrict__ image, const void* __restrict__ guideV,
                             const uint8_t* __restrict__ mask, int W, int H, int radius, float sigma, float weight0,
                             float weight1, float weight2, float* __restrict__ out) {
  __shared__ unsigned long long expTab[32];
  if (threadIdx.x < 32) {
    expTab[threadIdx.x] = kExp2fTab[threadIdx.x];
  }
  __syncthreads();
  const int x = blockIdx.x * 16 + (threadIdx.x & 15), y = blockIdx.y * 16 + (threadIdx.x >> 4);
  if (x >= W || y >= H) {
    return;
  }
  const size_t idx = (size_t)y * W + x;
  float result = image[idx];
  if (mask[idx]) {
    const float4 centre = bilateral_texel<GUIDE_U16>(guideV, idx, result);
    const float denom = 2.0f * (sigma * sigma);
    const double rcpDenom = 1.0 / (double)denom;
    float sumWeight = 0.f, weightedAvg = 0.f;
    for (int v = -radius; v <= radius; ++v) {
      const size_t row = (size_t)min(max(y + v, 0), H - 1) * W;
      for (int u = -radius; u <= radius; ++u) {
        const size_t j = row + min(max(x + u, 0), W - 1);
        if (!mask[j]) {
          continue;
        }
        bilateral_tap(centre, bilateral_texel<GUIDE_U16>(guideV, j, image[j]), weight0, weight1, weight2, rcpDenom,
                      expTab, sumWeight, weightedAvg);
      }
    }
    if (sumWeight != 0.0f) {
      result = weightedAvg / sumWeight;
    }
  }
  out[idx] = result;
}

constexpr int kMedianBlkW = 32, kMedianBlkH = 8;
__device__ __forceinline__ void cswap(float& a, float& b) {
  const float lo = fminf(a, b), hi = fmaxf(a, b);
  a = lo;
  b = hi;
}

__global__ void k_masked_median(const float* __restrict__ image, const float* __restrict__ background,
                                const uint8_t* __restrict__ mask, int W, int H, int radius, float* __restrict__ out,
                                size_t planeStride, const uint8_t* __restrict__ fovForNan) {
  __shared__ float taps[kMedianBlkH + 2][kMedianBlkW + 2];
  const int p = blockIdx.z;
  const int x = blockIdx.x * blockDim.x + threadIdx.x, y = blockIdx.y * blockDim.y + threadIdx.y;
  const float* img = image + (size_t)p * planeStride;
  const uint8_t* m = mask + (size_t)p * planeStride;
  if (radius == 1) {
    const int tw = (int)blockDim.x + 2, th = (int)blockDim.y + 2;
    const int x0 = (int)(blockIdx.x * blockDim.x) - 1, y0 = (int)(blockIdx.y * blockDim.y) - 1;
    for (int i = threadIdx.y * blockDim.x + threadIdx.x; i < tw * th; i += blockDim.x * blockDim.y) {
      const int ty = i / tw, tx = i - ty * tw;
      const int yy = y0 + ty, xx = x0 + tx;
      float t = __builtin_nanf("");
      if (yy >= 0 && yy < H && xx >= 0 && xx < W) {
        const size_t q = (size_t)yy * W + xx;
        const float val = img[q];
        if (m[q] && val != 0) {
          t = val;
        }
      }
      taps[ty][tx] = t;
    }
    __syncthreads();
  }
  if (x >= W || y >= H) {
    return;
  }
  const size_t idx = (size_t)y * W + x;
  float result = 0.0f;
  if (!m[idx]) {
    if (background) {
      result = background[(size_t)p * planeStride + idx];
    }
  } else if (radius == 1) {
    const float inf = __builtin_inff();
    float v[9];
    int cnt = 0;
#pragma unroll
    for (int j = 0; j < 3; ++j) {
#pragma unroll
      for (int i = 0; i < 3; ++i) {
        const float val = taps[threadIdx.y + j][threadIdx.x + i];
        const bool valid = !isnan(val);
        cnt += valid;
        v[j * 3 + i] = valid ? val : inf;
      }
    }
    cswap(v[0], v[1]); cswap(v[3], v[4]); cswap(v[6], v[7]);
    cswap(v[1], v[2]); cswap(v[4], v[5]); cswap(v[7], v[8]);
    cswap(v[0], v[1]); cswap(v[3], v[4]); cswap(v[6], v[7]);
    cswap(v[0], v[3]); cswap(v[3], v[6]); cswap(v[0], v[3]);
    cswap(v[1], v[4]); cswap(v[4], v[7]); cswap(v[1], v[4]);
    cswap(v[2], v[5]); cswap(v[5], v[8]); cswap(v[2], v[5]);
    cswap(v[1], v[3]); cswap(v[5], v[7]); cswap(v[2], v[6]);
    cswap(v[4], v[6]); cswap(v[2], v[4]); cswap(v[2], v[3]);
    cswap(v[5], v[6]);
    if (cnt > 0) {
      const int h = cnt / 2;
      float lo = v[0], hi = v[0];
#pragma unroll
      for (int k = 0; k < 9; ++k) {
        lo = (k == h - 1) ? v[k] : lo;
        hi = (k == h) ? v[k] : hi;
      }
      result = (cnt & 1) ? hi : (float)(((double)(lo + hi)) / 2.0);
    }
  } else {
    float vals[25];
    int cnt = 0;
    for (int yy = y - radius; yy <= y + radius; ++yy) {
      for (int xx = x - radius; xx <= x + radius; ++xx) {
        if (0 > yy || yy >= H || 0 > xx || xx >= W) {
          continue;
        }
        const size_t j = (size_t)yy * W + xx;
        if (!m[j]) {
          continue;
        }
        const float v = img[j];
        if (isnan(v) || v == 0) {
          continue;
        }
        int k = cnt++;
        while (k > 0 && vals[k - 1] > v) {
          vals[k] = vals[k - 1];
          --k;
        }
        vals[k] = v;
      }
    }
    if (cnt > 0) {
      const int h = cnt / 2;
      if (cnt % 2 == 1) {
        result = vals[h];
      } else {
        result = (float)(((double)(vals[h - 1] + vals[h])) / 2.0);
      }
    }
  }
  if (fovForNan && !fovForNan[(size_t)p * planeStride + idx]) {
    result = __builtin_nanf("");
  }
  out[(size_t)p * planeStride + idx] = result;
}

__global__ void k_mask_fov(const float* disp, const uint8_t* __restrict__ fov, float* out, size_t n) {
  size_t i = (size_t)blockIdx.x * blockDim.x + threadIdx.x;
  const size_t step = (size_t)gridDim.x * blockDim.x;
  const bool inPlace = out == disp;
  for (; i < n; i += step) {
    if (!fov[i]) {
      out[i] = __builtin_nanf("");
    } else if (!inPlace) {
      out[i] = disp[i];
    }
  }
}

__global__ void k_and_masks(const uint8_t* fov, const uint8_t* srcFg, const int* __restrict__ dst2src, int dst0,
                            size_t n, uint8_t* out) {
  const int d = dst0 + blockIdx.y;
  size_t i = (size_t)blockIdx.x * blockDim.x + threadIdx.x;
  const size_t step = (size_t)gridDim.x * blockDim.x;
  for (; i < n; i += step) {
    out[(size_t)d * n + i] = fov[(size_t)d * n + i] & srcFg[(size_t)dst2src[d] * n + i];
  }
}

__global__ void k_lanczos_h(const float* __restrict__ in, int SW, int SH, int DW, const int* __restrict__ xofs,
                            const float* __restrict__ alpha, float* __restrict__ tmp, size_t inStride,
                            size_t tmpStride) {
  const int p = blockIdx.z;
  const int dx = blockIdx.x * blockDim.x + threadIdx.x, y = blockIdx.y * blockDim.y + threadIdx.y;
  if (dx >= DW || y >= SH) {
    return;
  }
  const float* S = in + (size_t)p * inStride + (size_t)y * SW;
  const float* a = alpha + (size_t)dx * 8;
  const int sx = xofs[dx] - 3;
  float v = 0;
#pragma unroll
  for (int j = 0; j < 8; ++j) {
    const int sxj = min(max(sx + j, 0), SW - 1);
    float sv = S[sxj];
    if (sv != sv) {
      sv = 1e-4f;
    }
    v += sv * a[j];
  }
  tmp[(size_t)p * tmpStride + (size_t)y * DW + dx] = v;
}
__global__ void k_lanczos_v(const float* __restrict__ tmp, int SH, int DW, int DH, const int* __restrict__ yofs,
                            const float* __restrict__ beta, float* __restrict__ out, size_t tmpStride,
                            size_t outStride) {
  const int p = blockIdx.z;
  const int x = blockIdx.x * blockDim.x + threadIdx.x, dy = blockIdx.y * blockDim.y + threadIdx.y;
  if (x >= DW || dy >= DH) {
    return;
  }
  const float* T = tmp + (size_t)p * tmpStride;
  const float* b = beta + (size_t)dy * 8;
  const int sy = yofs[dy] - 3;
  float r[8];
#pragma unroll
  for (int k = 0; k < 8; ++k) {
    const int syk = min(max(sy + k, 0), SH - 1);
    r[k] = T[(size_t)syk * DW + x];
  }
  out[(size_t)p * outStride + (size_t)dy * DW + x] =
      r[0] * b[0] + r[1] * b[1] + r[2] * b[2] + r[3] * b[3] + r[4] * b[4] + r[5] * b[5] + r[6] * b[6] + r[7] * b[7];
}
constexpr int kLanczosW = 64, kLanczosH = 32, kLanczosRows = 40;
__global__ void __launch_bounds__(256) k_lanczos(const float* __restrict__ in, int SW, int SH, int DW, int DH,
                                                 const int* __restrict__ xofs, const float* __restrict__ alpha,
                                                 const int* __restrict__ yofs, const float* __restrict__ beta,
                                                 float* __restrict__ out, size_t inStride, size_t outStride) {
  __shared__ float rows[kLanczosRows][kLanczosW];
  const int p = blockIdx.z;
  const int dx = blockIdx.x * kLanczosW + threadIdx.x;
  const int dy0 = blockIdx.y * kLanczosH, dy1 = min(dy0 + kLanczosH, DH) - 1;
  const int rowLo = min(max(yofs[dy0] - 3, 0), SH - 1), rowHi = min(max(yofs[dy1] + 4, 0), SH - 1);
  if (dx < DW) {
    const float* a = alpha + (size_t)dx * 8;
    const int sx = xofs[dx] - 3;
    for (int r = threadIdx.y; r <= rowHi - rowLo && r < kLanczosRows; r += blockDim.y) {
      const float* S = in + (size_t)p * inStride + (size_t)(rowLo + r) * SW;
      float v = 0;
#pragma unroll
      for (int j = 0; j < 8; ++j) {
        const int sxj = min(max(sx + j, 0), SW - 1);
        float sv = S[sxj];
        if (sv != sv) {
          sv = 1e-4f;
        }
        v += sv * a[j];
      }
      rows[r][threadIdx.x] = v;
    }
  }
  __syncthreads();
  if (dx >= DW) {
    return;
  }
  for (int dy = dy0 + threadIdx.y; dy <= dy1; dy += blockDim.y) {
    const float* b = beta + (size_t)dy * 8;
    const int sy = yofs[dy] - 3;
    float r[8];
#pragma unroll
    for (int k = 0; k < 8; ++k) {
      const int syk = min(max(sy + k, 0), SH - 1);
      r[k] = rows[min(syk - rowLo, kLanczosRows - 1)][threadIdx.x];
    }
    out[(size_t)p * outStride + (size_t)dy * DW + dx] =
        r[0] * b[0] + r[1] * b[1] + r[2] * b[2] + r[3] * b[3] + r[4] * b[4] + r[5] * b[5] + r[6] * b[6] + r[7] * b[7];
  }
}

__global__ void k_upsample_nearest_masked(const float* __restrict__ in, const uint8_t* __restrict__ mask, int SW,
                                          int SH, const uint8_t* __restrict__ maskUp, int DW, int DH,
                                          float* __restrict__ out) {
  const int x = blockIdx.x * blockDim.x + threadIdx.x, y = blockIdx.y * blockDim.y + threadIdx.y;
  if (x >= DW || y >= DH) {
    return;
  }
  {
    const size_t ps = (size_t)blockIdx.z * SW * SH, pd = (size_t)blockIdx.z * DW * DH;
    in += ps;
    mask += ps;
    maskUp += pd;
    out += pd;
  }
  const double ifx = (double)SW / DW, ify = (double)SH / DH;
  const int sx = min((int)floor(x * ifx), SW - 1), sy = min((int)floor(y * ify), SH - 1);
  float v = in[(size_t)sy * SW + sx];
  if (!mask[(size_t)sy * SW + sx] || !maskUp[(size_t)y * DW + x]) {
    v = __builtin_nanf("");
  }
  out[(size_t)y * DW + x] = v;
}
__global__ void k_spiral_fill(const float* __restrict__ dispUp, const float* __restrict__ bgUp,
                              const uint8_t* __restrict__ maskUp, int W, int H, const int2* __restrict__ spiral,
                              int nSpiral, float* __restrict__ out) {
  const int x = blockIdx.x * blockDim.x + threadIdx.x, y = blockIdx.y * blockDim.y + threadIdx.y;
  if (x >= W || y >= H) {
    return;
  }
  {
    const size_t pd = (size_t)blockIdx.z * W * H;
    dispUp += pd;
    bgUp += pd;
    maskUp += pd;
    out += pd;
  }
  const size_t idx = (size_t)y * W + x;
  float v = dispUp[idx];
  if (maskUp[idx] && !(v > 0)) {
    for (int k = 0; k < nSpiral; ++k) {
      const int xx = min(max(x + spiral[k].x, 0), W - 1), yy = min(max(y + spiral[k].y, 0), H - 1);
      const float c = dispUp[(size_t)yy * W + xx];
      if (c > 0) {
        v = c;
        break;
      }
    }
  }
  if (isnan(v) || v == 0) {
    v = bgUp[idx];
  }
  out[idx] = v;
}

struct AreaAxis {
  const int* start;
  const int* si;
  const float* alpha;
  int iscale;
};

template <int KIND>
__device__ __forceinline__ float area_src(const void* src, size_t pix, int c) {
  if (KIND == 0) {
    return (float)reinterpret_cast<const uint16_t*>(src)[pix * 3 + c];
  } else if (KIND == 4) {
    return (float)reinterpret_cast<const uint16_t*>(src)[pix * 4 + c];
  } else if (KIND == 1) {
    return (float)reinterpret_cast<const uint8_t*>(src)[pix];
  } else if (KIND == 3) {
    return reinterpret_cast<const float*>(src)[pix * 3 + c];
  } else {
    return reinterpret_cast<const float*>(src)[pix];
  }
}

__device__ __forceinline__ void linear_area_tap(int d, int ssize, int dsize, int& s0, float& f, bool& one) {
  const double inv_scale = (double)dsize / (double)ssize, scale = 1. / inv_scale;
  int sx = (int)floor((double)d * scale);
  float fx = (float)((double)(d + 1) - (double)(sx + 1) * inv_scale);
  fx = fx <= 0 ? 0.f : fx - floorf(fx);
  if (sx < 0) {
    fx = 0.f;
    sx = 0;
  }
  one = sx + 1 >= ssize;
  if (sx >= ssize - 1) {
    fx = 0.f;
    sx = ssize - 1;
  }
  s0 = sx;
  f = fx;
}
template <int CN>
__global__ void k_resize_linear_area_f32(const float* __restrict__ src, int SW, int SH, float* __restrict__ dst, int DW,
                                         int DH) {
  const int dx = blockIdx.x * blockDim.x + threadIdx.x, dy = blockIdx.y * blockDim.y + threadIdx.y;
  if (dx >= DW || dy >= DH) {
    return;
  }
  int sx, sy;
  float fx, fy;
  bool onex, oney;
  linear_area_tap(dx, SW, DW, sx, fx, onex);
  linear_area_tap(dy, SH, DH, sy, fy, oney);
  const int y0 = min(max(sy, 0), SH - 1), y1 = min(max(sy + 1, 0), SH - 1);
  const float a0 = 1.f - fx, a1 = fx, b0 = 1.f - fy, b1 = fy;
#pragma unroll
  for (int c = 0; c < CN; ++c) {
    const float* r0 = src + ((size_t)y0 * SW + sx) * CN + c;
    const float* r1 = src + ((size_t)y1 * SW + sx) * CN + c;
    const float h0 = onex ? r0[0] * 1.f : r0[0] * a0 + r0[CN] * a1;
    const float h1 = onex ? r1[0] * 1.f : r1[0] * a0 + r1[CN] * a1;
    dst[((size_t)dy * DW + dx) * CN + c] = h0 * b0 + h1 * b1;
  }
}

template <int KIND>
__global__ void k_resize_area(const void* __restrict__ src, int SW, int SH, void* __restrict__ dst, int DW, int DH,
                              AreaAxis ax, AreaAxis ay, int threshold) {
  const int dx = blockIdx.x * blockDim.x + threadIdx.x, dy = blockIdx.y * blockDim.y + threadIdx.y;
  if (dx >= DW || dy >= DH) {
    return;
  }
  constexpr int CN = KIND == 4 ? 4 : (KIND == 0 || KIND == 3) ? 3 : 1;
  float res[CN];
  if (SW == DW && SH == DH) {
    for (int c = 0; c < CN; ++c) {
      res[c] = area_src<KIND>(src, (size_t)dy * SW + dx, c);
    }
  } else if (ax.iscale > 0 && ay.iscale > 0) {
    if (ax.iscale == 2 && ay.iscale == 2 && KIND != 2 && KIND != 3) {
      for (int c = 0; c < CN; ++c) {
        const size_t p = (size_t)(2 * dy) * SW + 2 * dx;
        const int v = (int)area_src<KIND>(src, p, c) + (int)area_src<KIND>(src, p + 1, c) +
            (int)area_src<KIND>(src, p + SW, c) + (int)area_src<KIND>(src, p + SW + 1, c);
        res[c] = (float)((v + 2) >> 2);
      }
    } else {
      const float scale = 1.f / (float)(ax.iscale * ay.iscale);
      for (int c = 0; c < CN; ++c) {
        float sum = 0;
        for (int sy = 0; sy < ay.iscale; ++sy) {
          for (int sx = 0; sx < ax.iscale; ++sx) {
            sum += area_src<KIND>(src, (size_t)(dy * ay.iscale + sy) * SW + dx * ax.iscale + sx, c);
          }
        }
        res[c] = sum * scale;
      }
    }
// ... 815 lines not shown
```

facebook360_dep_amd/csrc/derp_sequence.h:

```cpp
#pragma once
#include <dlfcn.h>
#include <rccl/rccl.h>

namespace {

void seq_window(int t, int first, int last, int radius, int* lo, int* hi) {
  *lo = std::max(first, t - radius);
  *hi = std::min(last, t + radius);
}

int seq_owner(int first, int last, int world, int policy, int frame) {
  const int F = last - first + 1, i = frame - first;
  if (i < 0 || i >= F || world < 1) {
    return -1;
  }
  if (policy == DERP_SEQ_CYCLIC) {
    return i % world;
  }
  const int q = F / world, r = F % world;
  const int big = r * (q + 1);
  return i < big ? i / (q + 1) : r + (q ? (i - big) / q : 0);
}

std::vector<derp_seq_transfer> seq_plan(int first, int last, int world, int radius, int policy) {
// ... 22 lines not shown
  void* lib = nullptr;
  ncclResult_t (*GetUniqueId)(ncclUniqueId*) = nullptr;
  ncclResult_t (*CommInitRank)(ncclComm_t*, int, ncclUniqueId, int) = nullptr;
  ncclResult_t (*CommDestroy)(ncclComm_t) = nullptr;
  ncclResult_t (*GroupStart)() = nullptr;
  ncclResult_t (*GroupEnd)() = nullptr;
  ncclResult_t (*Send)(const void*, size_t, ncclDataType_t, int, ncclComm_t, hipStream_t) = nullptr;
  ncclResult_t (*Recv)(void*, size_t, ncclDataType_t, int, ncclComm_t, hipStream_t) = nullptr;
  const char* (*GetErrorString)(ncclResult_t) = nullptr;
  std::string error;
};

RcclApi* rccl_api() {
  static RcclApi api;
  if (api.lib || !api.error.empty()) {
    return &api;
  }
  for (const char* name : {"librccl.so.1", "librccl.so", "/opt/rocm/lib/librccl.so.1"}) {
    api.lib = dlopen(name, RTLD_NOW | RTLD_LOCAL);
    if (api.lib) {
      break;
    }
  }
  if (!api.lib) {
    api.error = std::string("cannot load librccl: ") + dlerror();
    return &api;
  }
  auto sym = [&](const char* n) {
    void* p = dlsym(api.lib, n);
    if (!p && api.error.empty()) {
      api.error = std::string("librccl lacks ") + n;
    }
    return p;
  };
  api.GetUniqueId = reinterpret_cast<decltype(api.GetUniqueId)>(sym("ncclGetUniqueId"));
  api.CommInitRank = reinterpret_cast<decltype(api.CommInitRank)>(sym("ncclCommInitRank"));
  api.CommDestroy = reinterpret_cast<decltype(api.CommDestroy)>(sym("ncclCommDestroy"));
  api.GroupStart = reinterpret_cast<decltype(api.GroupStart)>(sym("ncclGroupStart"));
  api.GroupEnd = reinterpret_cast<decltype(api.GroupEnd)>(sym("ncclGroupEnd"));
  api.Send = reinterpret_cast<decltype(api.Send)>(sym("ncclSend"));
  api.Recv = reinterpret_cast<decltype(api.Recv)>(sym("ncclRecv"));
  api.GetErrorString = reinterpret_cast<decltype(api.GetErrorString)>(sym("ncclGetErrorString"));
  if (!api.error.empty()) {
    api.lib = nullptr;
  }
  return &api;
}

enum { SEQ_NONE = 0, SEQ_LOOPBACK = 1, SEQ_RCCL = 2, SEQ_EXTERNAL = 3 };

}

struct derp_seq {
  derp_ctx* c = nullptr;
  int first = 0, last = 0, rank = 0, world = 1;
  derp_seq_options opt;
  std::vector<int> owned, halo;
  std::vector<derp_seq_transfer> plan;
  std::vector<std::vector<DevBuf>> haloColor, haloFg, haloDisp;
  std::vector<DevBuf> filtered;
  DevBuf fov, winMask;
  int transport = SEQ_NONE;
  std::vector<derp_seq*> peers;
  ncclComm_t comm = nullptr;
  unsigned long long bytesSent = 0, bytesRecv = 0;
  std::vector<std::pair<hipEvent_t, hipEvent_t>> exchangeSpans;
  double exchangeMs = 0;
  hipStream_t xStream = nullptr;
  hipEvent_t computedEv = nullptr, exchangedEv = nullptr;
  bool exchangePending = false;
  std::vector<std::pair<hipEvent_t, hipEvent_t>> waitSpans;
  double exchangeExposedMs = 0;
  int levelReady = -1;
  int levelExchanged = -1;
  int computeLevel = -1, computedFrames = 0;
  std::vector<int> computedAt, filteredAt;
  std::vector<uint64_t> uploaded;
  std::vector<hipEvent_t> filteredEv;
  int fovLevel = -1;
  bool streaming = false;
  int nSlots = 0;
  struct HostIn {
    const uint16_t* color = nullptr;
    const uint8_t* fg = nullptr;
    const float* bg = nullptr;
  };
  std::vector<std::vector<HostIn>> hostIn;
  std::vector<std::vector<float*>> hostDisp;
  std::vector<char> hostHave;
  std::vector<float*> hostRaw;
  struct SlotTag {
    int k = -1, colorLevel = -1, rawLevel = -1;
  };
  std::vector<SlotTag> slotTag;
  std::vector<int> edge;
  std::vector<std::vector<DevBuf>> edgeColor, edgeFg;
  std::vector<DevBuf> edgeRaw;
  std::vector<char> edgeStaged;
};

namespace {

int owned_index(const derp_seq* q, int frame) {
  auto it = std::lower_bound(q->owned.begin(), q->owned.end(), frame);
  return it != q->owned.end() && *it == frame ? (int)(it - q->owned.begin()) : -1;
}
int halo_index(const derp_seq* q, int frame) {
  auto it = std::lower_bound(q->halo.begin(), q->halo.end(), frame);
  return it != q->halo.end() && *it == frame ? (int)(it - q->halo.begin()) : -1;
}
int edge_index(const derp_seq* q, int frame) {
  auto it = std::lower_bound(q->edge.begin(), q->edge.end(), frame);
  return it != q->edge.end() && *it == frame ? (int)(it - q->edge.begin()) : -1;
}

int seq_buffer(derp_seq* q, int frame, int level, int kind, void** ptr, size_t* bytes) {
  derp_ctx* c = q->c;
  TRY(check_level(c, level));
  if (kind < 0 || kind > 2) {
    return fail(c, "unknown buffer kind %d", kind);
  }
  const size_t n = npx(c, level);
  const size_t sz = kind == 0 ? n * c->S * sizeof(ushort4) : kind == 1 ? n * c->S : n * c->D * sizeof(float);
  DevBuf* b = nullptr;
  const int oi = owned_index(q, frame);
  if (oi >= 0 && q->streaming) {
    const int ei = edge_index(q, frame);
    if (ei < 0) {
      return fail(c, "frame %d streams through the frame slots (resident_frames = %d) and is in no other rank's window: "
                     "it has no fixed device buffer", frame, q->nSlots);
    }
    b = kind == 0 ? &q->edgeColor[ei][level] : kind == 1 ? &q->edgeFg[ei][level] : &q->edgeRaw[ei];
    if (b->bytes < sz) {
      return fail(c, "edge buffer of frame %d level %d kind %d was not allocated", frame, level, kind);
    }
  } else if (oi >= 0) {
    FramePyramid& f = c->frames[oi];
    b = kind == 0 ? &f.color[level] : kind == 1 ? &f.fg[level] : &f.disp[level];
  } else {
    const int hi = halo_index(q, frame);
    if (hi < 0) {
      return fail(c, "frame %d is neither owned by rank %d nor in its temporal halo", frame, q->rank);
    }
    b = kind == 0 ? &q->haloColor[hi][level] : kind == 1 ? &q->haloFg[hi][level] : &q->haloDisp[hi][level];
    if (b->bytes < sz) {
      return fail(c, "halo buffer of frame %d level %d kind %d was not allocated", frame, level, kind);
    }
  }
  *ptr = b->p;
  *bytes = sz;
  return 0;
}

#define NCCLCHK(c, api, expr)                                                                    \
  do {                                                                                           \
    ncclResult_t r_ = (expr);                                                                    \
    if (r_ != ncclSuccess) {                                                                     \
      return fail(c, "RCCL error %s at %s:%d (%s)", (api)->GetErrorString(r_), __FILE__, __LINE__, #expr); \
    }                                                                                            \
  } while (0)

int seq_exchange_rccl(derp_seq* q, int level, int kind) {
  derp_ctx* c = q->c;
  RcclApi* api = rccl_api();
  NCCLCHK(c, api, api->GroupStart());
  int rc = 0;
  for (const derp_seq_transfer& tr : q->plan) {
    void* p;
    size_t bytes;
    ncclResult_t r = ncclSuccess;
    if (tr.from_rank == q->rank) {
      rc = seq_buffer(q, tr.frame, level, kind, &p, &bytes);
      if (!rc) {
        r = api->Send(p, bytes, ncclUint8, tr.to_rank, q->comm, q->xStream);
        q->bytesSent += bytes;
      }
    } else if (tr.to_rank == q->rank) {
      rc = seq_buffer(q, tr.frame, level, kind, &p, &bytes);
      if (!rc) {
        r = api->Recv(p, bytes, ncclUint8, tr.from_rank, q->comm, q->xStream);
        q->bytesRecv += bytes;
      }
    }
    if (!rc && r != ncclSuccess) {
      rc = fail(c, "RCCL error %s moving frame %d (%d -> %d)", api->GetErrorString(r), tr.frame, tr.from_rank, tr.to_rank);
    }
    if (rc) {
      break;
    }
  }
  const ncclResult_t e = api->GroupEnd();
  if (!rc && e != ncclSuccess) {
    rc = fail(c, "RCCL error %s at ncclGroupEnd", api->GetErrorString(e));
  }
  return rc;
}

int seq_stage_edges(derp_seq* q, int level);

int seq_exchange_loopback(derp_seq* q, int level, int kind) {
  derp_ctx* c = q->c;
  std::vector<char> synced(q->world, 0);
  for (const derp_seq_transfer& tr : q->plan) {
    if (tr.from_rank == q->rank) {
      void* p;
      size_t bytes;
      TRY(seq_buffer(q, tr.frame, level, kind, &p, &bytes));
      q->bytesSent += bytes;
    }
    if (tr.to_rank != q->rank) {
      continue;
    }
    derp_seq* peer = q->peers[tr.from_rank];
    if (!synced[tr.from_rank]) {
      if (kind != 2 && seq_stage_edges(peer, level)) {
        return fail(c, "loopback peer %d: %s", tr.from_rank, peer->c->err.c_str());
      }
      HIPCHK(c, hipStreamSynchronize(peer->c->stream));
      synced[tr.from_rank] = 1;
    }
    void *src, *dst;
    size_t bs, bd;
    if (seq_buffer(peer, tr.frame, level, kind, &src, &bs)) {
      return fail(c, "loopback peer %d: %s", tr.from_rank, peer->c->err.c_str());
    }
    TRY(seq_buffer(q, tr.frame, level, kind, &dst, &bd));
    HIPCHK(c, hipMemcpyAsync(dst, src, bd, hipMemcpyDeviceToDevice, q->xStream));
    q->bytesRecv += bd;
  }
  HIPCHK(c, hipStreamSynchronize(q->xStream));
  return 0;
}

int seq_exchange(derp_seq* q, int level, int kind) {
  derp_ctx* c = q->c;
  if (q->plan.empty() || q->transport == SEQ_EXTERNAL) {
    return 0;
  }
  if (q->transport == SEQ_NONE) {
    return fail(c, "derp_seq: world size %d but no transport attached (rccl / loopback / external)", q->world);
  }
  hipEvent_t ea = nullptr, eb = nullptr;
  HIPCHK(c, hipEventCreate(&ea));
  if (hipEventCreate(&eb) != hipSuccess) {
    (void)hipEventDestroy(ea);
    return fail(c, "hipEventCreate failed");
  }
  HIPCHK(c, hipEventRecord(q->computedEv, c->stream));
  HIPCHK(c, hipStreamWaitEvent(q->xStream, q->computedEv, 0));
  (void)hipEventRecord(ea, q->xStream);
  const int rc = q->transport == SEQ_RCCL ? seq_exchange_rccl(q, level, kind) : seq_exchange_loopback(q, level, kind);
  (void)hipEventRecord(eb, q->xStream);
  (void)hipEventRecord(q->exchangedEv, q->xStream);
  q->exchangeSpans.push_back({ea, eb});
  q->exchangePending = true;
  return rc;
}

int seq_join_exchange(derp_seq* q) {
  derp_ctx* c = q->c;
  if (!q->exchangePending) {
    return 0;
  }
  hipEvent_t reached = nullptr, done = nullptr;
  if (hipEventCreate(&reached) == hipSuccess && hipEventCreate(&done) == hipSuccess) {
    (void)hipEventRecord(reached, c->stream);
  }
  HIPCHK(c, hipStreamWaitEvent(c->stream, q->exchangedEv, 0));
  if (reached && done) {
    (void)hipEventRecord(done, c->stream);
    q->waitSpans.push_back({reached, done});
  }
  q->exchangePending = false;
  return 0;
}

void seq_drain_spans(derp_seq* q) {
  for (auto& s : q->exchangeSpans) {
    (void)hipEventSynchronize(s.second);
    float ms = 0;
    (void)hipEventElapsedTime(&ms, s.first, s.second);
    q->exchangeMs += ms;
    (void)hipEventDestroy(s.first);
    (void)hipEventDestroy(s.second);
  }
  q->exchangeSpans.clear();
  for (auto& s : q->waitSpans) {
    (void)hipEventSynchronize(s.second);
    float ms = 0;
    (void)hipEventElapsedTime(&ms, s.first, s.second);
    q->exchangeExposedMs += ms > 0 ? ms : 0;
    (void)hipEventDestroy(s.first);
    (void)hipEventDestroy(s.second);
  }
  q->waitSpans.clear();
}

int temporal_space_radius(const derp_seq* q, int level) {
  if (q->opt.space_radius != -1) {
    return q->opt.space_radius;
  }
  const float scale = std::pow(0.9f, level);
  return (int)std::max(std::ceil(1 * scale), float(1));
}

}
// ... 126 lines not shown
      }
    }
  }
  q->filtered.resize(q->streaming ? 1 : q->owned.size());
  q->computedAt.assign(q->owned.size(), -1);
  q->filteredAt.assign(q->owned.size(), -1);
  if (hipStreamCreateWithFlags(&q->xStream, hipStreamNonBlocking) != hipSuccess ||
      hipEventCreateWithFlags(&q->computedEv, hipEventDisableTiming) != hipSuccess ||
      hipEventCreateWithFlags(&q->exchangedEv, hipEventDisableTiming) != hipSuccess) {
    return fail(c, "hipStreamCreate / hipEventCreate failed");
  }
  q->filteredEv.assign(q->streaming ? 0 : q->owned.size(), nullptr);
  for (auto& e : q->filteredEv) {
    if (hipEventCreateWithFlags(&e, hipEventDisableTiming) != hipSuccess) {
      return fail(c, "hipEventCreate failed");
    }
  }
  for (auto& b : q->filtered) {
    if (b.ensure(nmax * c->D * sizeof(float))) {
      return fail(c, "out of device memory allocating the filtered level");
    }
  }
  if (q->streaming) {
    q->slotTag.assign(q->nSlots, derp_seq::SlotTag());
    q->hostIn.assign(nOwned, std::vector<derp_seq::HostIn>(nl));
    q->hostDisp.assign(nOwned, std::vector<float*>(nl, nullptr));
    q->hostHave.assign((size_t)nOwned * nl, 0);
    q->hostRaw.assign(nOwned, nullptr);
    for (int k = 0; k < nOwned; ++k) {
      if (q->opt.do_temporal_filter && hipHostMalloc((void**)&q->hostRaw[k], nmax * c->D * sizeof(float), hipHostMallocDefault) != hipSuccess) {
        q->hostRaw[k] = nullptr;
        return fail(c, "out of page-locked host memory for the raw level of frame %d", q->owned[k]);
      }
      for (int l = 0; l < nl; ++l) {
        const size_t n = npx(c, l);
        if (n && hipHostMalloc((void**)&q->hostDisp[k][l], n * c->D * sizeof(float), hipHostMallocDefault) != hipSuccess) {
          q->hostDisp[k][l] = nullptr;
          return fail(c, "out of page-locked host memory for the results of frame %d", q->owned[k]);
        }
      }
    }
    for (const derp_seq_transfer& tr : q->plan) {
      if (tr.from_rank == rank && (q->edge.empty() || q->edge.back() != tr.frame)) {
        q->edge.push_back(tr.frame);
      }
    }
    for (auto* vv : {&q->edgeColor, &q->edgeFg}) {
      vv->resize(q->edge.size());
      for (auto& v : *vv) {
        v.resize(nl);
      }
    }
    q->edgeRaw.resize(q->edge.size());
    for (size_t e = 0; e < q->edge.size(); ++e) {
      if (q->edgeRaw[e].ensure(nmax * c->D * sizeof(float))) {
        return fail(c, "out of device memory allocating the edge frames");
      }
      for (int l = 0; l < nl; ++l) {
        const size_t n = npx(c, l);
        if (n && (q->edgeColor[e][l].ensure(n * c->S * sizeof(ushort4)) ||
                  (q->opt.use_foreground_masks && q->edgeFg[e][l].ensure(n * c->S)))) {
          return fail(c, "out of device memory allocating the edge frames");
        }
      }
    }
  }
  if (q->fov.ensure(nmax * c->D) ||
      (q->opt.use_foreground_masks && q->winMask.ensure((size_t)(2 * q->opt.time_radius + 1) * nmax * c->D))) {
    return fail(c, "out of device memory allocating the temporal masks");
  }
  *out = owner.release();
  return 0;
}

void derp_seq_destroy(derp_seq* q) {
  if (!q) {
    return;
  }
  if (q->c) {
    (void)hipSetDevice(q->c->device);
    (void)hipStreamSynchronize(q->c->stream);
  }
  seq_drain_spans(q);
  if (q->comm) {
    (void)rccl_api()->CommDestroy(q->comm);
  }
  for (auto& e : q->filteredEv) {
    if (e) {
      (void)hipEventDestroy(e);
    }
  }
  if (q->xStream) {
    (void)hipStreamSynchronize(q->xStream);
    (void)hipStreamDestroy(q->xStream);
  }
  for (hipEvent_t e : {q->computedEv, q->exchangedEv}) {
    if (e) {
      (void)hipEventDestroy(e);
    }
  }
  for (auto& v : q->hostDisp) {
    for (float* p : v) {
      if (p) {
        (void)hipHostFree(p);
      }
    }
  }
  for (float* p : q->hostRaw) {
    if (p) {
      (void)hipHostFree(p);
    }
  }
  delete q;
}

int derp_seq_counts(const derp_seq* q, int* n_owned, int* n_halo) {
  if (!q) {
    return 1;
  }
  if (n_owned) {
    *n_owned = (int)q->owned.size();
  }
  if (n_halo) {
    *n_halo = (int)q->halo.size();
  }
  return 0;
}

int derp_seq_frames(const derp_seq* q, int halo, int* frames, int cap) {
  if (!q || !frames) {
    return 1;
  }
  const std::vector<int>& v = halo ? q->halo : q->owned;
  for (int i = 0; i < (int)v.size() && i < cap; ++i) {
    frames[i] = v[i];
  }
  return 0;
}

int derp_seq_frame_slot(const derp_seq* q, int frame) {
  return q ? owned_index(q, frame) : -1;
}

int derp_seq_buffer(derp_seq* q, int frame, int level, int kind, void** ptr, size_t* bytes) {
  if (!q || !ptr || !bytes) {
    return 1;
  }
  {
    const int jrc = seq_join_exchange(q);
    if (jrc) {
      return jrc;
    }
  }
  return seq_buffer(q, frame, level, kind, ptr, bytes);
}

int derp_seq_buffer_copy(derp_seq* q, int frame, int level, int kind, void* host, size_t bytes, int to_device) {
  if (!q || !host) {
    return 1;
  }
  derp_ctx* c = q->c;
  void* p;
  size_t sz;
  TRY(seq_buffer(q, frame, level, kind, &p, &sz));
  if (bytes != sz) {
    return fail(c, "buffer of frame %d level %d kind %d holds %zu bytes, not %zu", frame, level, kind, sz, bytes);
  }
  HIPCHK(c, hipSetDevice(c->device));
  TRY(seq_join_exchange(q));
  HIPCHK(c, hipStreamSynchronize(c->stream));
  HIPCHK(c, hipMemcpy(to_device ? p : host, to_device ? host : p, sz, to_device ? hipMemcpyHostToDevice : hipMemcpyDeviceToHost));
  return 0;
}

int derp_seq_attach_loopback(derp_seq* q, derp_seq* const* peers, int n) {
  if (!q || !peers || n != q->world) {
    return q ? fail(q->c, "loopback needs one derp_seq per rank (%d given, world %d)", n, q->world) : 1;
  }
  q->peers.assign(peers, peers + n);
  if (q->peers[q->rank] != q) {
    return fail(q->c, "peers[%d] must be this rank's own derp_seq", q->rank);
  }
  q->transport = SEQ_LOOPBACK;
  return 0;
}

int derp_seq_attach_external(derp_seq* q) {
  if (!q) {
    return 1;
  }
  q->transport = SEQ_EXTERNAL;
  return 0;
}

int derp_seq_attach_rccl(derp_seq* q, const void* unique_id, size_t bytes) {
  if (!q || !unique_id || bytes < sizeof(ncclUniqueId)) {
    return q ? fail(q->c, "derp_seq_attach_rccl needs the %zu-byte id from derp_rccl_unique_id", sizeof(ncclUniqueId)) : 1;
  }
  derp_ctx* c = q->c;
  RcclApi* api = rccl_api();
  if (!api->lib) {
    return fail(c, "%s", api->error.c_str());
  }
  HIPCHK(c, hipSetDevice(c->device));
  ncclUniqueId id;
  memcpy(&id, unique_id, sizeof id);
  if (q->comm) {
    (void)api->CommDestroy(q->comm);
    q->comm = nullptr;
  }
  NCCLCHK(c, api, api->CommInitRank(&q->comm, q->world, id, q->rank));
  q->transport = SEQ_RCCL;
  return 0;
}

int derp_seq_selftest(derp_seq* q, int words) {
  if (!q || words < 1) {
    return 1;
  }
  derp_ctx* c = q->c;
  if (q->transport != SEQ_RCCL) {
    return fail(c, "derp_seq_selftest exercises the RCCL transport; attach it first");
  }
  RcclApi* api = rccl_api();
  HIPCHK(c, hipSetDevice(c->device));
  DevBuf a, b;
  const size_t bytes = (size_t)words * 4;
  std::vector<uint32_t> h(words), got(words);
  const int next = (q->rank + 1) % q->world, prev = (q->rank + q->world - 1) % q->world;
  for (int i = 0; i < words; ++i) {
    h[i] = 0x9e3779b9u * (uint32_t)(i + 1) + (uint32_t)q->rank;
  }
  TRY(upload_sync(c, a, h.data(), bytes));
  ALLOC(c, b, bytes);
  HIPCHK(c, hipMemsetAsync(b.p, 0, bytes, c->stream));
  ncclResult_t r = api->GroupStart();
  if (r == ncclSuccess) {
    r = api->Send(a.p, bytes, ncclUint8, next, q->comm, c->stream);
  }
  if (r == ncclSuccess) {
    r = api->Recv(b.p, bytes, ncclUint8, prev, q->comm, c->stream);
  }
  const ncclResult_t e = api->GroupEnd();
  if (r == ncclSuccess) {
    r = e;
  }
  if (r != ncclSuccess) {
    return fail(c, "RCCL self-test: %s", api->GetErrorString(r));
  }
  TRY(download_sync(c, got.data(), b.p, bytes));
  for (int i = 0; i < words; ++i) {
    if (got[i] != 0x9e3779b9u * (uint32_t)(i + 1) + (uint32_t)prev) {
      return fail(c, "RCCL self-test: word %d from rank %d is %08x", i, prev, got[i]);
    }
  }
  return 0;
}

}
namespace {

int upload_color_plane(derp_ctx* c, DevBuf& dst, int s, const uint16_t* bgr, size_t n) {
  TRY(upload_tmp(c, c->w.staging, bgr, n * 3));
  hipLaunchKernelGGL(k_bgr_to_bgrx, dim3(flat_grid(n)), dim3(256), 0, c->stream, c->w.staging.as<uint16_t>(),
                     dst.as<ushort4>() + (size_t)s * n, n);
  KCHECK(c);
  HIPCHK(c, hipStreamSynchronize(c->stream));
  return 0;
}

int host_inputs_of(derp_seq* q, int k, int level, const derp_seq::HostIn** out) {
  const derp_seq::HostIn& h = q->hostIn[k][level];
  if (!h.color && !h.fg) {
    return fail(q->c, "frame %d level %d: no host inputs registered (derp_seq_host_inputs)", q->owned[k], level);
  }
  *out = &h;
  return 0;
}

int seq_stage_edges(derp_seq* q, int level) {
  derp_ctx* c = q->c;
  if (!q->streaming || q->edge.empty()) {
    return 0;
  }
  if (q->edgeStaged.empty()) {
    q->edgeStaged.assign(c->numLevels, 0);
  }
  if (q->edgeStaged[level]) {
    return 0;
  }
  HIPCHK(c, hipSetDevice(c->device));
  const size_t n = npx(c, level);
  for (size_t e = 0; e < q->edge.size(); ++e) {
    const derp_seq::HostIn* h;
    TRY(host_inputs_of(q, owned_index(q, q->edge[e]), level, &h));
    if (!h->color) {
      return fail(c, "frame %d level %d: only masks were registered, the colour images are needed", q->edge[e], level);
    }
    for (int s = 0; s < c->S; ++s) {
      TRY(upload_color_plane(c, q->edgeColor[e][level], s, h->color + (size_t)s * n * 3, n));
    }
    if (q->opt.use_foreground_masks) {
      if (!h->fg) {
        return fail(c, "frame %d level %d: temporal masking needs the foreground masks", q->edge[e], level);
      }
      HIPCHK(c, hipMemcpy(q->edgeFg[e][level].p, h->fg, n * c->S, hipMemcpyHostToDevice));
    }
  }
  q->edgeStaged[level] = 1;
  return 0;
}

int stream_in_level(derp_seq* q, int k, int level, bool forCompute) {
  derp_ctx* c = q->c;
  const derp_seq::HostIn* h;
  TRY(host_inputs_of(q, k, level, &h));
  if (!h->color) {
    return fail(c, "frame %d level %d: only masks were registered, the colour images are needed", q->owned[k], level);
  }
  const size_t n = npx(c, level);
  for (int s = 0; s < c->S; ++s) {
    TRY(upload_color_plane(c, c->frame().color[level], s, h->color + (size_t)s * n * 3, n));
  }
  if (h->fg) {
    HIPCHK(c, hipMemcpy(c->frame().fg[level].p, h->fg, n * c->S, hipMemcpyHostToDevice));
  }
  if (forCompute && h->bg) {
    HIPCHK(c, hipMemcpy(c->frame().bg[level].p, h->bg, n * c->D * sizeof(float), hipMemcpyHostToDevice));
    c->frame().haveBg[level] = 1;
  }
  return 0;
}

int stream_compute_frame(derp_seq* q, int level, int k) {
  derp_ctx* c = q->c;
  const int slot = k % q->nSlots;
  TRY(select_frame(c, slot));
  derp_seq::SlotTag& tag = q->slotTag[slot];
  if (tag.k != k || tag.colorLevel != level) {
    tag = derp_seq::SlotTag();
    TRY(stream_in_level(q, k, level, true));
  }
  const int up = level + 1;
  const bool seeded = up < c->numLevels && npx(c, up) != 0;
  if (seeded) {
    if (!q->hostHave[(size_t)k * c->numLevels + up]) {
      return fail(c, "Missing disparity of level %d needed to start level %d (frame %d)", up, level, q->owned[k]);
    }
    HIPCHK(c, hipMemcpy(c->frame().disp[up].p, q->hostDisp[k][up], npx(c, up) * c->D * sizeof(float), hipMemcpyHostToDevice));
    c->frame().haveDisp[up] = 1;
    if (c->opt.use_foreground_masks) {
      const derp_seq::HostIn* hu;
      TRY(host_inputs_of(q, k, up, &hu));
      if (hu->fg) {
        HIPCHK(c, hipMemcpy(c->frame().fg[up].p, hu->fg, npx(c, up) * c->S, hipMemcpyHostToDevice));
      }
    }
  }
  TRY(process_level(c, level));
  const size_t bytes = npx(c, level) * c->D * sizeof(float);
  float* out = q->opt.do_temporal_filter ? q->hostRaw[k] : q->hostDisp[k][level];
  HIPCHK(c, hipMemcpyAsync(out, c->frame().disp[level].p, bytes, hipMemcpyDeviceToHost, c->stream));
  const int ei = edge_index(q, q->owned[k]);
  if (ei >= 0) {
    HIPCHK(c, hipMemcpyAsync(q->edgeRaw[ei].p, c->frame().disp[level].p, bytes, hipMemcpyDeviceToDevice, c->stream));
  }
  HIPCHK(c, hipStreamSynchronize(c->stream));
  tag.k = k;
  tag.colorLevel = tag.rawLevel = level;
  if (!q->opt.do_temporal_filter) {
    q->hostHave[(size_t)k * c->numLevels + level] = 1;
  }
  return 0;
}

int stream_filter_level(derp_seq* q, int level, int W, int H, int radius) {
  derp_ctx* c = q->c;
  const size_t n = (size_t)W * H;
  for (int j = 0; j < (int)q->owned.size(); ++j) {
    const int t = q->owned[j];
    int lo, hi;
    seq_window(t, q->first, q->last, q->opt.time_radius, &lo, &hi);
    std::vector<const void*> wg(hi - lo + 1);
    std::vector<const float*> wi(hi - lo + 1);
    std::vector<const uint8_t*> wmk(hi - lo + 1);
    for (int u = lo; u <= hi; ++u) {
      const void *pc, *pd, *pm;
      const int ku = owned_index(q, u);
      if (ku >= 0) {
        const int slot = ku % q->nSlots;
        derp_seq::SlotTag& tag = q->slotTag[slot];
        if (tag.k != ku || tag.colorLevel != level || tag.rawLevel != level) {
          TRY(select_frame(c, slot));
          if (tag.k != ku || tag.colorLevel != level) {
            tag = derp_seq::SlotTag();
            TRY(stream_in_level(q, ku, level, false));
          }
          HIPCHK(c, hipMemcpy(c->frame().disp[level].p, q->hostRaw[ku], n * c->D * sizeof(float), hipMemcpyHostToDevice));
          tag.k = ku;
          tag.colorLevel = tag.rawLevel = level;
        }
        pc = c->frames[slot].color[level].p;
        pd = c->frames[slot].disp[level].p;
        pm = c->frames[slot].fg[level].p;
      } else {
        void* p;
        size_t b;
        TRY(seq_buffer(q, u, level, 0, &p, &b));
        pc = p;
        TRY(seq_buffer(q, u, level, 2, &p, &b));
        pd = p;
        pm = nullptr;
        if (q->opt.use_foreground_masks) {
          TRY(seq_buffer(q, u, level, 1, &p, &b));
          pm = p;
        }
      }
      if (q->opt.use_foreground_masks) {
        uint8_t* wm = q->winMask.as<uint8_t>() + (size_t)(u - lo) * n * c->D;
        hipLaunchKernelGGL(k_and_masks, dim3(flat_grid(n), c->D), dim3(256), 0, c->stream, q->fov.as<uint8_t>(),
                           (const uint8_t*)pm, c->dst2src.as<int>(), 0, n, wm);
        KCHECK(c);
        pm = wm;
      } else {
        pm = q->fov.p;
      }
      wg[u - lo] = pc;
      wi[u - lo] = reinterpret_cast<const float*>(pd);
      wmk[u - lo] = reinterpret_cast<const uint8_t*>(pm);
    }
    TRY(temporal_launch(c, wg.data(), wi.data(), wmk.data(), hi - lo + 1, t - lo, W, H, c->D, q->opt.sigma, radius,
                        q->opt.weight_b, q->opt.weight_g, q->opt.weight_b, q->filtered[0].as<float>(), c->dst2src.as<int>()));
    HIPCHK(c, hipMemcpyAsync(q->hostDisp[j][level], q->filtered[0].p, n * c->D * sizeof(float), hipMemcpyDeviceToHost,
                             c->stream));
    HIPCHK(c, hipStreamSynchronize(c->stream));
    q->hostHave[(size_t)j * c->numLevels + level] = 1;
  }
  return 0;
}

}
extern "C" {

int derp_seq_host_inputs(derp_seq* q, int frame, int level, const uint16_t* color_bgr, const uint8_t* fg_masks,
                         const float* background_disparity) {
  if (!q) {
    return 1;
  }
  derp_ctx* c = q->c;
  TRY(check_level(c, level));
  const int k = owned_index(q, frame);
  if (k < 0 || (!color_bgr && !fg_masks)) {
    return fail(c, k < 0 ? "frame %d is not owned by rank %d" : "frame %d: neither colour nor masks", frame, q->rank);
  }
  HIPCHK(c, hipSetDevice(c->device));
  if (q->streaming) {
    q->hostIn[k][level] = {color_bgr, fg_masks, background_disparity};
    if (!q->edgeStaged.empty() && edge_index(q, frame) >= 0) {
      q->edgeStaged[level] = 0;
    }
    for (derp_seq::SlotTag& tag : q->slotTag) {
      if (tag.k == k && tag.colorLevel == level) {
        tag = derp_seq::SlotTag();
      }
    }
    return 0;
  }
  const size_t n = npx(c, level);
  TRY(select_frame(c, k));
  for (int s = 0; color_bgr && s < c->S; ++s) {
    TRY(upload_color_plane(c, c->frame().color[level], s, color_bgr + (size_t)s * n * 3, n));
  }
  if (fg_masks) {
    HIPCHK(c, hipMemcpy(c->frame().fg[level].p, fg_masks, n * c->S, hipMemcpyHostToDevice));
  }
  if (background_disparity) {
    HIPCHK(c, hipMemcpy(c->frame().bg[level].p, background_disparity, n * c->D * sizeof(float), hipMemcpyHostToDevice));
    c->frame().haveBg[level] = 1;
  }
  return 0;
}

int derp_seq_upload_color_plane(derp_seq* q, int frame, int level, int s, const uint16_t* bgr) {
  if (!q) {
    return 1;
  }
  derp_ctx* c = q->c;
  TRY(check_level(c, level));
  const int k = owned_index(q, frame);
  if (k < 0 || s < 0 || s >= c->S || !bgr) {
    return fail(c, "bad frame / source index / null image");
  }
  if (q->streaming) {
    return fail(c, "out of core the frames stream from the buffers given to derp_seq_host_inputs");
  }
  HIPCHK(c, hipSetDevice(c->device));
  const size_t n = npx(c, level);
  ALLOC(c, c->copyStaging, n * 3 * sizeof(uint16_t));
  HIPCHK(c, hipMemcpyAsync(c->copyStaging.p, bgr, n * 3 * sizeof(uint16_t), hipMemcpyHostToDevice, c->copyStream));
  hipLaunchKernelGGL(k_bgr_to_bgrx, dim3(flat_grid(n)), dim3(256), 0, c->copyStream, c->copyStaging.as<uint16_t>(),
                     c->frames[k].color[level].as<ushort4>() + (size_t)s * n, n);
  KCHECK(c);
  HIPCHK(c, hipStreamSynchronize(c->copyStream));
  return 0;
}

int derp_seq_upload_disparity(derp_seq* q, int frame, int level, int d, const float* disp) {
  if (!q) {
    return 1;
  }
  derp_ctx* c = q->c;
  TRY(check_level(c, level));
  const int k = owned_index(q, frame);
  if (k < 0 || d < 0 || d >= c->D || !disp) {
    return fail(c, "bad frame / destination index / null image");
  }
  if (q->streaming) {
    memcpy(q->hostDisp[k][level] + (size_t)d * npx(c, level), disp, npx(c, level) * sizeof(float));
    q->hostHave[(size_t)k * c->numLevels + level] = 1;
    return 0;
  }
  TRY(select_frame(c, k));
  TRY(derp_upload_disparity(c, level, d, disp));
  if (q->uploaded.size() != q->owned.size() * (size_t)c->numLevels) {
    q->uploaded.assign(q->owned.size() * (size_t)c->numLevels, 0);
  }
  q->uploaded[(size_t)k * c->numLevels + level] |= 1ull << d;
  return 0;
}

int derp_seq_download_disparity(derp_seq* q, int frame, int level, int d, float* disp) {
  if (!q) {
    return 1;
  }
  derp_ctx* c = q->c;
  TRY(check_level(c, level));
  const int k = owned_index(q, frame);
  if (k < 0 || d < -1 || d >= c->D || !disp) {
    return fail(c, "bad frame / destination index / null output");
  }
  const size_t n = npx(c, level);
  if (q->streaming) {
    if (!q->hostHave[(size_t)k * c->numLevels + level]) {
      return fail(c, "level %d of frame %d has not been processed", level, frame);
    }
    memcpy(disp, q->hostDisp[k][level] + (size_t)std::max(d, 0) * n, (d < 0 ? c->D : 1) * n * sizeof(float));
    return 0;
  }
  HIPCHK(c, hipSetDevice(c->device));
  TRY(select_frame(c, k));
  if (d < 0) {
    if (!c->frame().haveDisp[level]) {
      return fail(c, "level %d has not been processed", level);
    }
    HIPCHK(c, hipStreamSynchronize(c->stream));
    HIPCHK(c, hipMemcpy(disp, c->frame().disp[level].p, n * c->D * sizeof(float), hipMemcpyDeviceToHost));
    return 0;
  }
  return derp_download_disparity(c, level, d, disp);
}

int derp_seq_exchange_inputs_level(derp_seq* q, int level) {
  if (!q) {
    return 1;
  }
  derp_ctx* c = q->c;
  HIPCHK(c, hipSetDevice(c->device));
  TRY(check_level(c, level));
  TRY(seq_stage_edges(q, level));
  TRY(seq_exchange(q, level, 0));
  if (q->opt.use_foreground_masks) {
    TRY(seq_exchange(q, level, 1));
  }
  return seq_join_exchange(q);
}

int derp_seq_exchange_inputs(derp_seq* q) {
  if (!q) {
    return 1;
  }
  derp_ctx* c = q->c;
  for (int l = 0; l < c->numLevels; ++l) {
    if (npx(c, l) == 0) {
      continue;
    }
    TRY(derp_seq_exchange_inputs_level(q, l));
  }
  return 0;
}

int derp_seq_level_compute_frame(derp_seq* q, int level, int frame) {
  if (!q) {
    return 1;
  }
  derp_ctx* c = q->c;
  HIPCHK(c, hipSetDevice(c->device));
  TRY(seq_join_exchange(q));
  const int k = owned_index(q, frame);
  if (k < 0) {
    return fail(c, "frame %d is not owned by rank %d", frame, q->rank);
  }
  if (q->computeLevel != level) {
    q->computeLevel = level;
    q->computedFrames = 0;
    q->levelReady = -1;
  }
  const int rebuild = c->opt.rebuild_warp_tables;
  c->opt.rebuild_warp_tables = q->computedFrames == 0 ? rebuild : 0;
  int rc;
  if (q->streaming) {
    rc = stream_compute_frame(q, level, k);
  } else {
    rc = select_frame(c, k);
    if (!rc) {
      rc = process_level(c, level);
    }
  }
  c->opt.rebuild_warp_tables = rebuild;
  TRY(rc);
  q->computedAt[k] = level;
  q->filteredAt[k] = -1;
  if (++q->computedFrames >= (int)q->owned.size()) {
    q->levelReady = level;
  }
  return 0;
}

int derp_seq_level_provided_frame(derp_seq* q, int level, int frame) {
  if (!q) {
    return 1;
  }
  derp_ctx* c = q->c;
  TRY(check_level(c, level));
  const int k = owned_index(q, frame);
  if (k < 0) {
    return fail(c, "frame %d is not owned by rank %d", frame, q->rank);
  }
  if (q->streaming) {
    return fail(c, "derp_seq_level_provided_frame needs the frames resident in HBM");
  }
  TRY(select_frame(c, k));
  const uint64_t all = c->D >= 64 ? ~0ull : (1ull << c->D) - 1;
  const size_t slotLevel = (size_t)k * c->numLevels + level;
  if (!c->frame().haveDisp[level] || q->uploaded.size() <= slotLevel || (q->uploaded[slotLevel] & all) != all) {
    return fail(c, "frame %d has no complete level %d disparity (derp_seq_upload_disparity of every destination first)", frame, level);
  }
  q->uploaded[slotLevel] = 0;
  if (q->computeLevel != level) {
    q->computeLevel = level;
    q->computedFrames = 0;
    q->levelReady = -1;
  }
  q->computedAt[k] = level;
  q->filteredAt[k] = -1;
  if (++q->computedFrames >= (int)q->owned.size()) {
    q->levelReady = level;
  }
  return 0;
}

int seq_lane_count(derp_seq* q, int level) {
  derp_ctx* c = q->c;
  const int maxLanes = getenv("DERP_SEQ_LANES") ? atoi(getenv("DERP_SEQ_LANES")) : 8;
  const int maxWidth = getenv("DERP_SEQ_LANE_MAX_WIDTH") ? atoi(getenv("DERP_SEQ_LANE_MAX_WIDTH")) : 256;
  if (q->streaming || maxLanes < 2 || (int)q->owned.size() < 2 || c->LW[level] > maxWidth || c->LH[level] > maxWidth ||
      getenv("DERP_TABLE_BUDGET_GB")) {
    return 0;
  }
  return std::min(maxLanes, (int)q->owned.size()) - 1;
}

int derp_seq_level_compute(derp_seq* q, int level) {
  if (!q) {
    return 1;
  }
  q->computeLevel = -1;
  derp_ctx* c = q->c;
  TRY(check_level(c, level));
  TRY(seq_join_exchange(q));
  const int lanes = seq_lane_count(q, level);
  if (lanes > 0) {
    HIPCHK(c, hipSetDevice(c->device));
    TRY(lanes_prepare(c, lanes, npx(c, level)));
    Span wall(c, ST_LANES, level);
    for (int k = 0; k < (int)q->owned.size(); ++k) {
      const int lane = k == 0 ? -1 : (k - 1) % lanes;
      if (q->computeLevel != level) {
        q->computeLevel = level;
        q->computedFrames = 0;
        q->levelReady = -1;
      }
      const int rebuild = c->opt.rebuild_warp_tables;
      c->opt.rebuild_warp_tables = k == 0 ? rebuild : 0;
      const int rc = process_level_on_lane(c, lane, k, level);
      c->opt.rebuild_warp_tables = rebuild;
      TRY(rc);
      if (k == 0) {
        if (c->DB != c->D) {
          return fail(c, "work lanes need every destination's tables in one batch (level %d: %d of %d)", level, c->DB, c->D);
        }
        HIPCHK(c, hipEventRecord(c->laneReady, c->stream));
      }
      q->computedAt[k] = level;
      q->filteredAt[k] = -1;
      ++q->computedFrames;
    }
    for (int i = 0; i < lanes; ++i) {
      HIPCHK(c, hipStreamWaitEvent(c->stream, c->lanes[i]->done, 0));
    }
    q->levelReady = level;
    return 0;
  }
  for (int t : q->owned) {
    TRY(derp_seq_level_compute_frame(q, level, t));
  }
  if (q->owned.empty()) {
    q->levelReady = level;
  }
  return 0;
}

int derp_seq_level_exchange(derp_seq* q, int level) {
  if (!q) {
    return 1;
  }
  derp_ctx* c = q->c;
  HIPCHK(c, hipSetDevice(c->device));
  if (!q->opt.do_temporal_filter) {
    return 0;
  }
  if (q->levelReady != level) {
    return fail(c, "derp_seq_level_exchange(%d): derp_seq_level_compute(%d) has not completed for every owned frame", level, level);
  }
  TRY(seq_exchange(q, level, 2));
  if (q->transport != SEQ_EXTERNAL) {
    q->levelExchanged = level;
  }
  if (q->streaming || getenv("DERP_SEQ_NO_OVERLAP")) {
    TRY(seq_join_exchange(q));
  }
  return 0;
}

int derp_seq_mark_exchanged(derp_seq* q, int level) {
  if (!q) {
    return 1;
  }
  q->levelExchanged = level;
  return 0;
}

namespace {
int seq_fov_masks(derp_seq* q, int level) {
  derp_ctx* c = q->c;
  if (q->fovLevel != level) {
    const int W = c->LW[level], H = c->LH[level];
    hipLaunchKernelGGL(k_fov_mask, grid2d(W, H, c->D, kBlk2d), kBlk2d, 0, c->stream, c->camsDst.as<Cam>(), W, H,
                       q->fov.as<uint8_t>());
    KCHECK(c);
    q->fovLevel = level;
  }
  return 0;
}
int seq_filter_frame(derp_seq* q, int level, int k) {
  derp_ctx* c = q->c;
  const int W = c->LW[level], H = c->LH[level];
  const size_t n = (size_t)W * H;
  const int radius = temporal_space_radius(q, level);
  const int t = q->owned[k];
  int lo, hi;
  seq_window(t, q->first, q->last, q->opt.time_radius, &lo, &hi);
  std::vector<const void*> wg(hi - lo + 1);
  std::vector<const float*> wi(hi - lo + 1);
  std::vector<const uint8_t*> wmk(hi - lo + 1);
  for (int u = lo; u <= hi; ++u) {
    void *pc, *pd, *pm;
    size_t b;
    TRY(seq_buffer(q, u, level, 0, &pc, &b));
    TRY(seq_buffer(q, u, level, 2, &pd, &b));
    if (q->opt.use_foreground_masks) {
      TRY(seq_buffer(q, u, level, 1, &pm, &b));
      uint8_t* wm = q->winMask.as<uint8_t>() + (size_t)(u - lo) * n * c->D;
      hipLaunchKernelGGL(k_and_masks, dim3(flat_grid(n), c->D), dim3(256), 0, c->stream, q->fov.as<uint8_t>(),
                         (const uint8_t*)pm, c->dst2src.as<int>(), 0, n, wm);
      KCHECK(c);
      pm = wm;
    } else {
      pm = q->fov.p;
    }
    wg[u - lo] = pc;
    wi[u - lo] = reinterpret_cast<const float*>(pd);
    wmk[u - lo] = reinterpret_cast<const uint8_t*>(pm);
  }
  TRY(temporal_launch(c, wg.data(), wi.data(), wmk.data(), hi - lo + 1, t - lo, W, H, c->D, q->opt.sigma, radius,
                      q->opt.weight_b, q->opt.weight_g, q->opt.weight_b, q->filtered[k].as<float>(), c->dst2src.as<int>()));
  q->filteredAt[k] = level;
  HIPCHK(c, hipEventRecord(q->filteredEv[k], c->stream));
  return 0;
}
}

int derp_seq_level_filter_frame(derp_seq* q, int level, int frame) {
  if (!q) {
    return 1;
  }
  derp_ctx* c = q->c;
  HIPCHK(c, hipSetDevice(c->device));
  TRY(check_level(c, level));
  const int k = owned_index(q, frame);
  if (k < 0) {
    return fail(c, "frame %d is not owned by rank %d", frame, q->rank);
  }
  if (!q->opt.do_temporal_filter || q->streaming) {
    return 2;
  }
  if (q->filteredAt[k] == level) {
    return 0;
  }
  int lo, hi;
  seq_window(frame, q->first, q->last, q->opt.time_radius, &lo, &hi);
  bool needsHalo = false;
  for (int u = lo; u <= hi; ++u) {
    const int ku = owned_index(q, u);
    if (ku >= 0 ? q->computedAt[ku] != level : q->levelExchanged != level) {
      return 2;
    }
    needsHalo |= ku < 0;
  }
  if (needsHalo) {
    TRY(seq_join_exchange(q));
  }
  Span sp(c, ST_TEMPORAL, level);
  TRY(seq_fov_masks(q, level));
  return seq_filter_frame(q, level, k);
}

int derp_seq_download_filtered(derp_seq* q, int frame, int level, int d, float* out) {
  if (!q) {
    return 1;
  }
  derp_ctx* c = q->c;
  TRY(check_level(c, level));
  const int k = owned_index(q, frame);
  if (k < 0 || d < -1 || d >= c->D || !out) {
    return fail(c, "bad frame / destination index / null output");
  }
  if (q->streaming || q->filteredAt[k] != level) {
    return fail(c, "frame %d has no filtered level %d in its scratch (derp_seq_level_filter_frame)", frame, level);
  }
  HIPCHK(c, hipSetDevice(c->device));
  const size_t n = npx(c, level);
  HIPCHK(c, hipStreamWaitEvent(c->copyStream, q->filteredEv[k], 0));
  HIPCHK(c, hipMemcpyAsync(out, q->filtered[k].as<float>() + (size_t)std::max(d, 0) * n, (d < 0 ? c->D : 1) * n * sizeof(float),
                           hipMemcpyDeviceToHost, c->copyStream));
  HIPCHK(c, hipStreamSynchronize(c->copyStream));
  return 0;
}

int derp_seq_level_filter(derp_seq* q, int level) {
  if (!q) {
    return 1;
  }
  derp_ctx* c = q->c;
  HIPCHK(c, hipSetDevice(c->device));
  TRY(check_level(c, level));
  if (!q->opt.do_temporal_filter) {
    return 0;
  }
  if (q->levelReady != level) {
    return fail(c, "derp_seq_level_filter(%d): derp_seq_level_compute(%d) has not completed for every owned frame", level, level);
  }
  if (!q->halo.empty() && q->levelExchanged != level) {
    return fail(c, "derp_seq_level_filter(%d): the halo frames' level has not been exchanged (derp_seq_level_exchange, or "
                   "derp_seq_mark_exchanged after an external transport moved it)", level);
  }
  const int W = c->LW[level], H = c->LH[level];
  const size_t n = (size_t)W * H;
  Span sp(c, ST_TEMPORAL, level);
  TRY(seq_fov_masks(q, level));
  if (q->streaming) {
    TRY(seq_join_exchange(q));
    const int radius = temporal_space_radius(q, level);
    TRY(stream_filter_level(q, level, W, H, radius));
    q->levelReady = -1;
    return 0;
  }
  for (int pass = 0; pass < 2; ++pass) {
    if (pass == 1) {
      TRY(seq_join_exchange(q));
    }
    for (int k = 0; k < (int)q->owned.size(); ++k) {
      if (q->filteredAt[k] == level) {
        continue;
      }
      int lo, hi;
      seq_window(q->owned[k], q->first, q->last, q->opt.time_radius, &lo, &hi);
      bool allOwned = true;
      for (int u = lo; allOwned && u <= hi; ++u) {
        allOwned = owned_index(q, u) >= 0;
      }
      if (pass == 1 || allOwned) {
        TRY(seq_filter_frame(q, level, k));
      }
    }
  }
  for (int k = 0; k < (int)q->owned.size(); ++k) {
    HIPCHK(c, hipMemcpyAsync(c->frames[k].disp[level].p, q->filtered[k].p, n * c->D * sizeof(float), hipMemcpyDeviceToDevice,
                             c->stream));
    q->computedAt[k] = -1;
  }
  q->levelReady = -1;
  return 0;
}

int derp_seq_run(derp_seq* q, int level_start, int level_end_) {
  if (!q) {
    return 1;
  }
  derp_ctx* c = q->c;
  if (level_start < level_end_) {
    return fail(c, "Check failed: level_start >= level_end (%d vs %d)", level_start, level_end_);
  }
  if (!q->plan.empty() && q->transport != SEQ_RCCL) {
    return fail(c, "derp_seq_run drives all three phases itself and needs the RCCL transport; with loopback / "
                   "external transports call derp_seq_level_compute / _exchange / _filter per level");
  }
  for (int level = level_start; level >= level_end_; --level) {
    TRY(derp_seq_level_compute(q, level));
    TRY(derp_seq_level_exchange(q, level));
    TRY(derp_seq_level_filter(q, level));
  }
  return 0;
}
// ... 45 lines not shown
```

Measured before the change: 530.0 Mpix/s.

## Skip all-pass fg mask ANDs, tile median strip, stage Lanczos inputs, batch row rank

Tracks per level whether the foreground mask buffers are still at their memset all-ones default. When they are, the k_and_masks pass is skipped and the FOV mask is used directly, both in the per-frame pipeline and in the temporal filter windows. It also adds a shared-memory strip kernel for the 3x3 masked median, stages Lanczos source tiles and coefficients in shared memory, and batches k_row_rank over eight 256-wide steps. The aim is to cut redundant HBM reads and kernel launches, at the cost of new state tracking that must invalidate correctly on every fg write path.

Result: no change. 534.0 Mpix/s (median of 6 runs) (+0.8%).

```diff
diff --git a/__graft_entry__.py b/__graft_entry__.py
--- a/__graft_entry__.py
+++ b/__graft_entry__.py
@@ -17,7 +17,7 @@
 
 
 def build_hip(force=False):
-    srcs = [os.path.join(CSRC, f) for f in ("derp_capi.hip", "derp_host.h", "derp_ctx.h", "derp_kernels.h", "derp_render.h", "derp_points.h", "derp_mesh.h", "derp_mesh_math.h", "derp_camera.h", "gcc_algos.h", "derp_render_api.h", "derp_rephoto_api.h", "derp_points_api.h", "derp_mesh_api.h", "derp_filters_api.h", "derp_debug_api.h", "derp_sequence.h", "derp_isp.h", "derp_sim.h", "derp_sim_math.h", "derp_geometric.h", "derp_geometric_api.h", "derp_sweep.h", "derp_sweep_api.h", "derp_align.h", "derp_align_api.h")]
+    srcs = [os.path.join(CSRC, f) for f in ("derp_capi.hip", "derp_host.h", "derp_ctx.h", "derp_fg_fill.h", "derp_kernels.h", "derp_render.h", "derp_points.h", "derp_mesh.h", "derp_mesh_math.h", "derp_camera.h", "gcc_algos.h", "derp_render_api.h", "derp_rephoto_api.h", "derp_points_api.h", "derp_mesh_api.h", "derp_filters_api.h", "derp_debug_api.h", "derp_sequence.h", "derp_isp.h", "derp_sim.h", "derp_sim_math.h", "derp_geometric.h", "derp_geometric_api.h", "derp_sweep.h", "derp_sweep_api.h", "derp_align.h", "derp_align_api.h")]
     srcs.append(os.path.join(ROOT, "include", "derp_hip.h"))
     host = os.path.join(CSRC, "derp_images.cpp")
     simplify = os.path.join(CSRC, "derp_simplify.cpp")
diff --git a/facebook360_dep_amd/csrc/derp_capi.hip b/facebook360_dep_amd/csrc/derp_capi.hip
--- a/facebook360_dep_amd/csrc/derp_capi.hip
+++ b/facebook360_dep_amd/csrc/derp_capi.hip
@@ -29,6 +29,11 @@
 #include "derp_ctx.h"
 
 namespace {
+
+const dim3 kMedianStripBlk(kMedianStripW, kMedianStripTy, 1);
+dim3 median_strip_grid(int w, int h, int planes) {
+  return dim3((w + kMedianStripW - 1) / kMedianStripW, (h + kMedianStripH - 1) / kMedianStripH, planes);
+}
 
 struct Span {
   derp_ctx* c;
@@ -188,6 +193,12 @@
     t.tileSpan = std::max(t.tileSpan, hi - lo + 1);
     t.monotone = t.monotone && std::is_sorted(ofs.begin() + d0, ofs.begin() + d1 + 1);
   }
+  for (int d0 = 0; d0 < dsize; d0 += kLanczosW) {
+    const int d1 = std::min(d0 + kLanczosW, dsize) - 1;
+    const int lo = std::min(std::max(ofs[d0] - 3, 0), ssize - 1), hi = std::min(std::max(ofs[d1] + 4, 0), ssize - 1);
+    t.tileSpanW = std::max(t.tileSpanW, hi - lo + 1);
+    t.monotoneW = t.monotoneW && std::is_sorted(ofs.begin() + d0, ofs.begin() + d1 + 1);
+  }
   ALLOC(c, t.ofs, ofs.size() * sizeof(int));
   ALLOC(c, t.coef, coef.size() * sizeof(float));
   HIPCHK(c, hipMemcpyAsync(t.ofs.p, ofs.data(), ofs.size() * sizeof(int), hipMemcpyHostToDevice, c->stream));
@@ -330,7 +341,7 @@
   LanczosTab *tx, *ty;
   TRY(get_lanczos(c, sw, dw, &tx));
   TRY(get_lanczos(c, sh, dh, &ty));
-  if (ty->monotone && ty->tileSpan <= kLanczosRows) {
+  if (ty->monotone && ty->tileSpan <= kLanczosRows && tx->monotoneW && tx->tileSpanW <= kLanczosCols) {
     hipLaunchKernelGGL(k_lanczos, dim3((dw + kLanczosW - 1) / kLanczosW, (dh + kLanczosH - 1) / kLanczosH, planes),
                        dim3(kLanczosW, 4), 0, c->stream, in, sw, sh, dw, dh, tx->ofs.as<int>(), tx->coef.as<float>(),
                        ty->ofs.as<int>(), ty->coef.as<float>(), out, inStride, outStride);
@@ -393,11 +404,18 @@
       KCHECK(c);
       c->fovCachedLevel = level;
     }
-    hipLaunchKernelGGL(k_and_masks, dim3(flat_grid(n), c->D), dim3(256), 0, c->stream, c->fovMask.as<uint8_t>(),
-                       c->frame().fg[level].as<uint8_t>(), c->dst2src.as<int>(), 0, n, c->w.maskAnd.as<uint8_t>());
-    KCHECK(c);
-  }
-  return 0;
+    c->w.maskIsFov = c->frame().fgFill.all_pass(level);
+    if (!c->w.maskIsFov) {
+      hipLaunchKernelGGL(k_and_masks, dim3(flat_grid(n), c->D), dim3(256), 0, c->stream, c->fovMask.as<uint8_t>(),
+                         c->frame().fg[level].as<uint8_t>(), c->dst2src.as<int>(), 0, n, c->w.maskAnd.as<uint8_t>());
+      KCHECK(c);
+    }
+  }
+  return 0;
+}
+
+const uint8_t* level_mask(derp_ctx* c) {
+  return c->w.maskIsFov ? c->fovMask.as<uint8_t>() : c->w.maskAnd.as<uint8_t>();
 }
 
 int build_warp(derp_ctx* c, int dst0, int nd) {
@@ -651,7 +669,7 @@
   const size_t n = (size_t)W * H;
   const int radius = bilateral_radius(L);
   launch_joint_bilateral_u16_tiled(c, dim3((W + 15) / 16, (H + 15) / 16, c->D), c->w.disparity.as<float>(),
-                                   (const void*)c->frame().color[L].as<ushort4>(), c->w.maskAnd.as<uint8_t>(), W, H, radius,
+                                   (const void*)c->frame().color[L].as<ushort4>(), level_mask(c), W, H, radius,
                                    0.005f, 0.5f, 1.0f, 1.0f, c->w.tmpF.as<float>(), n, n, c->dst2src.as<int>());
   KCHECK(c);
   std::swap(c->w.disparity, c->w.tmpF);
@@ -664,9 +682,10 @@
   c->randomRanThisLevel = false;
   const int W = c->LW[L], H = c->LH[L];
   const size_t n = (size_t)W * H;
-  hipLaunchKernelGGL(k_masked_median, grid2d(W, H, c->D, kBlk2d), kBlk2d, 0, c->stream, c->w.disparity.as<float>(),
+  hipLaunchKernelGGL(k_masked_median_strip, median_strip_grid(W, H, c->D), kMedianStripBlk, 0, c->stream,
+                     c->w.disparity.as<float>(),
                      c->opt.use_foreground_masks ? c->frame().bg[L].as<float>() : (const float*)nullptr,
-                     c->w.maskAnd.as<uint8_t>(), W, H, 1, levelOut ? levelOut : c->w.tmpF.as<float>(), n,
+                     level_mask(c), W, H, levelOut ? levelOut : c->w.tmpF.as<float>(), n,
                      fuseMaskFov ? c->fovMask.as<uint8_t>() : (const uint8_t*)nullptr);
   KCHECK(c);
   if (!levelOut) {
@@ -741,7 +760,7 @@
                          (size_t)sw * sh, c->w.staging.as<uint8_t>());
       KCHECK(c);
       TRY(upsample_masked_dev(c, c->frame().disp[level + 1].as<float>(), c->w.staging.as<uint8_t>(), sw, sh,
-                              c->w.maskAnd.as<uint8_t>(), c->frame().bg[level].as<float>(), c->w.disparity.as<float>(), W, H, c->D));
+                              level_mask(c), c->frame().bg[level].as<float>(), c->w.disparity.as<float>(), W, H, c->D));
     }
   } else {
     HIPCHK(c, hipMemsetAsync(c->w.disparity.p, 0, n * c->D * sizeof(float), c->stream));
@@ -865,6 +884,7 @@
   f.disp.resize(num_levels);
   f.haveBg.assign(num_levels, 0);
   f.haveDisp.assign(num_levels, 0);
+  f.fgFill.reset(num_levels);
   for (int l = 0; l < num_levels; ++l) {
     const size_t n = npx(c, l);
     if (n == 0) {
@@ -875,6 +895,7 @@
     ALLOC(c, f.bg[l], n * c->D * sizeof(float));
     ALLOC(c, f.disp[l], n * c->D * sizeof(float));
     HIPCHK(c, hipMemsetAsync(f.fg[l].p, 1, n * c->S, c->stream));
+    f.fgFill.filled(l);
     HIPCHK(c, hipMemsetAsync(f.bg[l].p, 0, n * c->D * sizeof(float), c->stream));
   }
   return 0;
@@ -1261,6 +1282,7 @@
   }
   HIPCHK(c, hipSetDevice(c->device));
   const size_t n = npx(c, level);
+  c->frame().fgFill.written(level);
   HIPCHK(c, hipMemcpy(c->frame().fg[level].as<uint8_t>() + (size_t)s * n, mask, n, hipMemcpyHostToDevice));
   return 0;
 }
@@ -1453,6 +1475,9 @@
     void* dst = kind == 0 ? (void*)(c->frame().color[l].as<ushort4>() + (size_t)index * nl)
         : kind == 1       ? (void*)(c->frame().fg[l].as<uint8_t>() + (size_t)index * nl)
                           : (void*)(c->frame().bg[l].as<float>() + (size_t)index * nl);
+    if (kind == 1) {
+      c->frame().fgFill.written(l);
+    }
     TRY(resize_area_dev(c, kind, c->fullFrame.p, w, h, dst, c->LW[l], c->LH[l], threshold));
     if (kind == 2) {
       c->frame().haveBg[l] = 1;
diff --git a/facebook360_dep_amd/csrc/derp_ctx.h b/facebook360_dep_amd/csrc/derp_ctx.h
--- a/facebook360_dep_amd/csrc/derp_ctx.h
+++ b/facebook360_dep_amd/csrc/derp_ctx.h
@@ -1,4 +1,6 @@
 #pragma once
+
+#include "derp_fg_fill.h"
 
 namespace {
 
@@ -44,6 +46,8 @@
   DevBuf ofs, coef;
   int tileSpan = 0;
   bool monotone = true;
+  int tileSpanW = 0;
+  bool monotoneW = true;
 };
 
 struct AreaTabDev {
@@ -60,12 +64,14 @@
   DevBuf projColorT;
   DevBuf bruteCost, bruteConf, lanczosTmp, staging, stagingB;
   bool mismatchMaskHeld = false;
+  bool maskIsFov = false;
   int colorTablesCleanLevel = -1;
 };
 
 struct FramePyramid {
   std::vector<DevBuf> color, fg, bg, disp;
   std::vector<char> haveBg, haveDisp;
+  FgFill fgFill;
 };
 
 struct WorkLane {
diff --git a/facebook360_dep_amd/csrc/derp_fg_fill.h b/facebook360_dep_amd/csrc/derp_fg_fill.h
--- /dev/null
+++ b/facebook360_dep_amd/csrc/derp_fg_fill.h
@@ -0,0 +1,37 @@
+#pragma once
+
+#include <cstddef>
+#include <vector>
+
+namespace derp {
+
+class FgFill {
+ public:
+  void reset(int levels) {
+    allPass_.assign(levels > 0 ? (size_t)levels : 0, 0);
+  }
+  void filled(int level) {
+    if (known(level)) {
+      allPass_[(size_t)level] = 1;
+    }
+  }
+  void written(int level) {
+    if (known(level)) {
+      allPass_[(size_t)level] = 0;
+    }
+  }
+  bool all_pass(int level) const {
+    return known(level) && allPass_[(size_t)level] != 0;
+  }
+  int levels() const {
+    return (int)allPass_.size();
+  }
+
+ private:
+  bool known(int level) const {
+    return level >= 0 && (size_t)level < allPass_.size();
+  }
+  std::vector<char> allPass_;
+};
+
+}
diff --git a/facebook360_dep_amd/csrc/derp_filters_api.h b/facebook360_dep_amd/csrc/derp_filters_api.h
--- a/facebook360_dep_amd/csrc/derp_filters_api.h
+++ b/facebook360_dep_amd/csrc/derp_filters_api.h
@@ -184,9 +184,15 @@
   }
   TRY(upload_sync(c, m, mask, n));
   ALLOC(c, res, n * 4);
-  hipLaunchKernelGGL(k_masked_median, grid2d(w, h, 1, kBlk2d), kBlk2d, 0, c->stream, im.as<float>(),
-                     background ? bg.as<float>() : (const float*)nullptr, m.as<uint8_t>(), w, h, radius,
-                     res.as<float>(), n, (const uint8_t*)nullptr);
+  if (radius == 1) {
+    hipLaunchKernelGGL(k_masked_median_strip, median_strip_grid(w, h, 1), kMedianStripBlk, 0, c->stream, im.as<float>(),
+                       background ? bg.as<float>() : (const float*)nullptr, m.as<uint8_t>(), w, h, res.as<float>(), n,
+                       (const uint8_t*)nullptr);
+  } else {
+    hipLaunchKernelGGL(k_masked_median, grid2d(w, h, 1, kBlk2d), kBlk2d, 0, c->stream, im.as<float>(),
+                       background ? bg.as<float>() : (const float*)nullptr, m.as<uint8_t>(), w, h, radius,
+                       res.as<float>(), n, (const uint8_t*)nullptr);
+  }
   return download_sync(c, out, res.p, n * 4);
 }
 
diff --git a/facebook360_dep_amd/csrc/derp_kernels.h b/facebook360_dep_amd/csrc/derp_kernels.h
--- a/facebook360_dep_amd/csrc/derp_kernels.h
+++ b/facebook360_dep_amd/csrc/derp_kernels.h
@@ -1535,32 +1535,67 @@
   }
 }
 
+constexpr int kRankSteps = 8;
 __global__ void __launch_bounds__(256) k_row_rank(LevelView V, const uint32_t* __restrict__ powers, int* __restrict__ rank) {
-  __shared__ int waveCount[2][4];
+  __shared__ int waveCount[2][kRankSteps][4];
   const int d = V.dst0 + blockIdx.y, y = blockIdx.x + 1;
   const int own = V.dst2src[d];
   const size_t n = (size_t)V.W * V.H;
   const int lane = threadIdx.x & 63, wave = threadIdx.x >> 6;
   const uint32_t seed = minstd_seed(y * V.level);
+  const float varHighDev = 0.1f * V.varHighThresh;
+  const float thresh = fmaxf(varHighDev, V.varNoiseFloor);
+  const uint8_t* fov = V.fovMask + (size_t)d * n + (size_t)y * V.W;
+  const uint8_t* fg = V.srcFg + (size_t)own * n + (size_t)y * V.W;
+  const float* var = V.srcVar + (size_t)own * n + (size_t)y * V.W;
+  int* rankRow = rank + (size_t)d * n + (size_t)y * V.W;
   int before = 0;
-  for (int xb = 1, step = 0; xb < V.W - 1; xb += 256, ++step) {
-    const int x = xb + (int)threadIdx.x;
-    const size_t idx = (size_t)y * V.W + x;
-    const bool go = x < V.W - 1 && random_gate(V, d, own, idx);
-    const unsigned long long ballot = __ballot(go);
-    if (lane == 0) {
-      waveCount[step & 1][wave] = __popcll(ballot);
+  for (int xb = 1, chunk = 0; xb < V.W - 1; xb += 256 * kRankSteps, ++chunk) {
+    uint8_t inFov[kRankSteps], inFg[kRankSteps];
+    float variance[kRankSteps];
+#pragma unroll
+    for (int s = 0; s < kRankSteps; ++s) {
+      const int xc = min(xb + s * 256 + (int)threadIdx.x, V.W - 2);
+      inFov[s] = fov[xc];
+      inFg[s] = fg[xc];
+      variance[s] = var[xc];
+    }
+    unsigned long long ballot[kRankSteps];
+#pragma unroll
+    for (int s = 0; s < kRankSteps; ++s) {
+      const int x = xb + s * 256 + (int)threadIdx.x;
+      const bool go = x < V.W - 1 && inFov[s] && inFg[s] && !(variance[s] < thresh);
+      ballot[s] = __ballot(go);
+      if (lane == 0) {
+        waveCount[chunk & 1][s][wave] = __popcll(ballot[s]);
+      }
     }
     __syncthreads();
-    int k = before + __popcll(ballot & ((1ull << lane) - 1ull));
-#pragma unroll
-    for (int w = 0; w < 4; ++w) {
-      const int t = waveCount[step & 1][w];
-      k += w < wave ? t : 0;
-      before += t;
-    }
-    if (go) {
-      rank[(size_t)d * n + idx] = (int)minstd_mulmod(seed, powers[k]);
+    uint32_t power[kRankSteps];
+#pragma unroll
+    for (int s = 0; s < kRankSteps; ++s) {
+      int k = before + __popcll(ballot[s] & ((1ull << lane) - 1ull));
+#pragma unroll
+      for (int w = 0; w < 4; ++w) {
+        const int t = waveCount[chunk & 1][s][w];
+        k += w < wave ? t : 0;
+        before += t;
+      }
+      power[s] = 1u;
+      if ((ballot[s] >> lane) & 1ull) {
+        power[s] = powers[k];
+      }
+    }
+#pragma unroll
+    for (int s = 0; s < kRankSteps; ++s) {
+      power[s] = minstd_mulmod(seed, power[s]);
+      asm volatile("" : "+v"(power[s]));
+    }
+#pragma unroll
+    for (int s = 0; s < kRankSteps; ++s) {
+      if ((ballot[s] >> lane) & 1ull) {
+        rankRow[xb + s * 256 + (int)threadIdx.x] = (int)power[s];
+      }
     }
   }
 }
@@ -2319,39 +2354,161 @@
   out[idx] = result;
 }
 
-constexpr int kMedianBlkW = 32, kMedianBlkH = 8;
 __device__ __forceinline__ void cswap(float& a, float& b) {
   const float lo = fminf(a, b), hi = fmaxf(a, b);
   a = lo;
   b = hi;
 }
 
+__device__ __forceinline__ float median9(const float (&t0)[3], const float (&t1)[3], const float (&t2)[3]) {
+  const float inf = __builtin_inff();
+  float v[9];
+  int cnt = 0;
+#pragma unroll
+  for (int i = 0; i < 3; ++i) {
+    const float val = t0[i];
+    const bool valid = !isnan(val);
+    cnt += valid;
+    v[i] = valid ? val : inf;
+  }
+#pragma unroll
+  for (int i = 0; i < 3; ++i) {
+    const float val = t1[i];
+    const bool valid = !isnan(val);
+    cnt += valid;
+    v[3 + i] = valid ? val : inf;
+  }
+#pragma unroll
+  for (int i = 0; i < 3; ++i) {
+    const float val = t2[i];
+    const bool valid = !isnan(val);
+    cnt += valid;
+    v[6 + i] = valid ? val : inf;
+  }
+  cswap(v[0], v[1]); cswap(v[3], v[4]); cswap(v[6], v[7]);
+  cswap(v[1], v[2]); cswap(v[4], v[5]); cswap(v[7], v[8]);
+  cswap(v[0], v[1]); cswap(v[3], v[4]); cswap(v[6], v[7]);
+  cswap(v[0], v[3]); cswap(v[3], v[6]); cswap(v[0], v[3]);
+  cswap(v[1], v[4]); cswap(v[4], v[7]); cswap(v[1], v[4]);
+  cswap(v[2], v[5]); cswap(v[5], v[8]); cswap(v[2], v[5]);
+  cswap(v[1], v[3]); cswap(v[5], v[7]); cswap(v[2], v[6]);
+  cswap(v[4], v[6]); cswap(v[2], v[4]); cswap(v[2], v[3]);
+  cswap(v[5], v[6]);
+  float result = 0.0f;
+  if (cnt > 0) {
+    const int h = cnt / 2;
+    float lo = v[0], hi = v[0];
+#pragma unroll
+    for (int k = 0; k < 9; ++k) {
+      lo = (k == h - 1) ? v[k] : lo;
+      hi = (k == h) ? v[k] : hi;
+    }
+    result = (cnt & 1) ? hi : (float)(((double)(lo + hi)) / 2.0);
+  }
+  return result;
+}
+
+constexpr int kMedianStripW = 64, kMedianStripTy = 4, kMedianStripR = 8;
+constexpr int kMedianStripH = kMedianStripTy * kMedianStripR;
+constexpr int kMedianStripTw = kMedianStripW + 2, kMedianStripTh = kMedianStripH + 2;
+constexpr int kMedianStripThreads = kMedianStripW * kMedianStripTy;
+constexpr int kMedianStripTrips = (kMedianStripTw * kMedianStripTh + kMedianStripThreads - 1) / kMedianStripThreads;
+__global__ void __launch_bounds__(kMedianStripThreads)
+    k_masked_median_strip(const float* __restrict__ image, const float* __restrict__ background,
+                          const uint8_t* __restrict__ mask, int W, int H, float* __restrict__ out, size_t planeStride,
+                          const uint8_t* __restrict__ fovForNan) {
+  __shared__ float taps[kMedianStripTh * kMedianStripTw];
+  __shared__ uint8_t inMask[kMedianStripTh * kMedianStripTw];
+  const int p = blockIdx.z;
+  const float* img = image + (size_t)p * planeStride;
+  const uint8_t* m = mask + (size_t)p * planeStride;
+  const int tid = threadIdx.y * kMedianStripW + threadIdx.x;
+  const int x0 = (int)blockIdx.x * kMedianStripW - 1, y0 = (int)blockIdx.y * kMedianStripH - 1;
+  const int x = (int)blockIdx.x * kMedianStripW + (int)threadIdx.x;
+  const int r0 = (int)threadIdx.y * kMedianStripR;
+  const int yFirst = (int)blockIdx.y * kMedianStripH + r0;
+  uint8_t inFov[kMedianStripR];
+  {
+    float val[kMedianStripTrips];
+    uint8_t mk[kMedianStripTrips];
+#pragma unroll
+    for (int k = 0; k < kMedianStripTrips; ++k) {
+      const int i = tid + k * kMedianStripThreads;
+      const int ty = i / kMedianStripTw, tx = i - ty * kMedianStripTw;
+      const size_t q = (size_t)min(max(y0 + ty, 0), H - 1) * W + min(max(x0 + tx, 0), W - 1);
+      val[k] = img[q];
+      mk[k] = m[q];
+    }
+#pragma unroll
+    for (int j = 0; j < kMedianStripR; ++j) {
+      inFov[j] = 1;
+      if (fovForNan) {
+        inFov[j] = fovForNan[(size_t)p * planeStride + (size_t)min(yFirst + j, H - 1) * W + min(x, W - 1)];
+      }
+    }
+#pragma unroll
+    for (int k = 0; k < kMedianStripTrips; ++k) {
+      const int i = tid + k * kMedianStripThreads;
+      const int ty = i / kMedianStripTw, tx = i - ty * kMedianStripTw;
+      const int yy = y0 + ty, xx = x0 + tx;
+      const bool in = yy >= 0 && yy < H && xx >= 0 && xx < W;
+      if (i < kMedianStripTw * kMedianStripTh) {
+        taps[i] = (in && mk[k] && val[k] != 0) ? val[k] : __builtin_nanf("");
+        inMask[i] = in ? mk[k] : (uint8_t)0;
+      }
+    }
+  }
+  __syncthreads();
+  const int rows = min(kMedianStripR, H - yFirst);
+  if (x >= W || rows <= 0) {
+    return;
+  }
+  const float* col = taps + threadIdx.x;
+  float a[3], b[3], c[3], result[kMedianStripR];
+  bool outside[kMedianStripR];
+#pragma unroll
+  for (int i = 0; i < 3; ++i) {
+    a[i] = col[(r0 + 0) * kMedianStripTw + i];
+    b[i] = col[(r0 + 1) * kMedianStripTw + i];
+  }
+#pragma unroll
+  for (int j = 0; j < kMedianStripR; ++j) {
+#pragma unroll
+    for (int i = 0; i < 3; ++i) {
+      c[i] = col[(r0 + j + 2) * kMedianStripTw + i];
+    }
+    outside[j] = !inMask[(r0 + j + 1) * kMedianStripTw + threadIdx.x + 1];
+    result[j] = outside[j] ? 0.0f : median9(a, b, c);
+#pragma unroll
+    for (int i = 0; i < 3; ++i) {
+      a[i] = b[i];
+      b[i] = c[i];
+    }
+  }
+  const size_t first = (size_t)p * planeStride + (size_t)yFirst * W + x;
+  if (background) {
+#pragma unroll
+    for (int j = 0; j < kMedianStripR; ++j) {
+      if (j < rows && outside[j]) {
+        result[j] = background[first + (size_t)j * W];
+      }
+    }
+  }
+#pragma unroll
+  for (int j = 0; j < kMedianStripR; ++j) {
+    if (j < rows) {
+      out[first + (size_t)j * W] = inFov[j] ? result[j] : __builtin_nanf("");
+    }
+  }
+}
+
 __global__ void k_masked_median(const float* __restrict__ image, const float* __restrict__ background,
                                 const uint8_t* __restrict__ mask, int W, int H, int radius, float* __restrict__ out,
                                 size_t planeStride, const uint8_t* __restrict__ fovForNan) {
-  __shared__ float taps[kMedianBlkH + 2][kMedianBlkW + 2];
   const int p = blockIdx.z;
   const int x = blockIdx.x * blockDim.x + threadIdx.x, y = blockIdx.y * blockDim.y + threadIdx.y;
   const float* img = image + (size_t)p * planeStride;
   const uint8_t* m = mask + (size_t)p * planeStride;
-  if (radius == 1) {
-    const int tw = (int)blockDim.x + 2, th = (int)blockDim.y + 2;
-    const int x0 = (int)(blockIdx.x * blockDim.x) - 1, y0 = (int)(blockIdx.y * blockDim.y) - 1;
-    for (int i = threadIdx.y * blockDim.x + threadIdx.x; i < tw * th; i += blockDim.x * blockDim.y) {
-      const int ty = i / tw, tx = i - ty * tw;
-      const int yy = y0 + ty, xx = x0 + tx;
-      float t = __builtin_nanf("");
-      if (yy >= 0 && yy < H && xx >= 0 && xx < W) {
-        const size_t q = (size_t)yy * W + xx;
-        const float val = img[q];
-        if (m[q] && val != 0) {
-          t = val;
-        }
-      }
-      taps[ty][tx] = t;
-    }
-    __syncthreads();
-  }
   if (x >= W || y >= H) {
     return;
   }
@@ -2360,39 +2517,6 @@
   if (!m[idx]) {
     if (background) {
       result = background[(size_t)p * planeStride + idx];
-    }
-  } else if (radius == 1) {
-    const float inf = __builtin_inff();
-    float v[9];
-    int cnt = 0;
-#pragma unroll
-    for (int j = 0; j < 3; ++j) {
-#pragma unroll
-      for (int i = 0; i < 3; ++i) {
-        const float val = taps[threadIdx.y + j][threadIdx.x + i];
-        const bool valid = !isnan(val);
-        cnt += valid;
-        v[j * 3 + i] = valid ? val : inf;
-      }
-    }
-    cswap(v[0], v[1]); cswap(v[3], v[4]); cswap(v[6], v[7]);
-    cswap(v[1], v[2]); cswap(v[4], v[5]); cswap(v[7], v[8]);
-    cswap(v[0], v[1]); cswap(v[3], v[4]); cswap(v[6], v[7]);
-    cswap(v[0], v[3]); cswap(v[3], v[6]); cswap(v[0], v[3]);
-    cswap(v[1], v[4]); cswap(v[4], v[7]); cswap(v[1], v[4]);
-    cswap(v[2], v[5]); cswap(v[5], v[8]); cswap(v[2], v[5]);
-    cswap(v[1], v[3]); cswap(v[5], v[7]); cswap(v[2], v[6]);
-    cswap(v[4], v[6]); cswap(v[2], v[4]); cswap(v[2], v[3]);
-    cswap(v[5], v[6]);
-    if (cnt > 0) {
-      const int h = cnt / 2;
-      float lo = v[0], hi = v[0];
-#pragma unroll
-      for (int k = 0; k < 9; ++k) {
-        lo = (k == h - 1) ? v[k] : lo;
-        hi = (k == h) ? v[k] : hi;
-      }
-      result = (cnt & 1) ? hi : (float)(((double)(lo + hi)) / 2.0);
     }
   } else {
     float vals[25];
@@ -2499,30 +2623,80 @@
   out[(size_t)p * outStride + (size_t)dy * DW + x] =
       r[0] * b[0] + r[1] * b[1] + r[2] * b[2] + r[3] * b[3] + r[4] * b[4] + r[5] * b[5] + r[6] * b[6] + r[7] * b[7];
 }
-constexpr int kLanczosW = 64, kLanczosH = 32, kLanczosRows = 40;
+constexpr int kLanczosW = 64, kLanczosH = 32, kLanczosRows = 40, kLanczosCols = kLanczosW + 8;
+constexpr int kLanczosTrips = (kLanczosRows * kLanczosCols + 255) / 256;
 __global__ void __launch_bounds__(256) k_lanczos(const float* __restrict__ in, int SW, int SH, int DW, int DH,
                                                  const int* __restrict__ xofs, const float* __restrict__ alpha,
                                                  const int* __restrict__ yofs, const float* __restrict__ beta,
                                                  float* __restrict__ out, size_t inStride, size_t outStride) {
+  __shared__ float raw[kLanczosRows * kLanczosCols];
   __shared__ float rows[kLanczosRows][kLanczosW];
+  __shared__ float betaT[kLanczosH * 8];
+  __shared__ int yofsT[kLanczosH];
+  static_assert(kLanczosH * 8 == 256, "one beta value per thread");
   const int p = blockIdx.z;
-  const int dx = blockIdx.x * kLanczosW + threadIdx.x;
+  const int dx0 = blockIdx.x * kLanczosW, dx1 = min(dx0 + kLanczosW, DW) - 1;
+  const int dx = dx0 + threadIdx.x;
   const int dy0 = blockIdx.y * kLanczosH, dy1 = min(dy0 + kLanczosH, DH) - 1;
   const int rowLo = min(max(yofs[dy0] - 3, 0), SH - 1), rowHi = min(max(yofs[dy1] + 4, 0), SH - 1);
+  const int colLo = min(max(xofs[dx0] - 3, 0), SW - 1), colHi = min(max(xofs[dx1] + 4, 0), SW - 1);
+  const int nR = min(rowHi - rowLo + 1, kLanczosRows), nC = min(colHi - colLo + 1, kLanczosCols);
+  float a[8];
+  int sx;
+  {
+    const int total = nR * nC, tid = threadIdx.y * kLanczosW + threadIdx.x;
+    {
+      const int dxc = min(dx, DW - 1);
+      sx = xofs[dxc] - 3;
+#pragma unroll
+      for (int j = 0; j < 8; ++j) {
+        a[j] = alpha[(size_t)dxc * 8 + j];
+      }
+    }
+    const float betaMine = beta[(size_t)min(dy0 + (tid >> 3), DH - 1) * 8 + (tid & 7)];
+    const int yofsMine = yofs[min(dy0 + (tid & (kLanczosH - 1)), DH - 1)];
+    const float* S = in + (size_t)p * inStride + (size_t)rowLo * SW + colLo;
+    const int qStep = 256 / nC, rStep = 256 - qStep * nC;
+    int r = tid / nC, cc = tid - r * nC;
+    float sv[kLanczosTrips];
+#pragma unroll
+    for (int k = 0; k < kLanczosTrips; ++k) {
+      if (k * 256 < total) {
+        const bool past = tid + k * 256 >= total;
+        sv[k] = S[(size_t)(past ? nR - 1 : r) * SW + (past ? nC - 1 : cc)];
+        r += qStep;
+        cc += rStep;
+        if (cc >= nC) {
+          cc -= nC;
+          ++r;
+        }
+      }
+    }
+#pragma unroll
+    for (int k = 0; k < kLanczosTrips; ++k) {
+      const int i = tid + k * 256;
+      if (i < total) {
+        raw[i] = sv[k] != sv[k] ? 1e-4f : sv[k];
+      }
+    }
+    betaT[tid] = betaMine;
+    if (tid < kLanczosH) {
+      yofsT[tid] = yofsMine;
+    }
+  }
+  __syncthreads();
   if (dx < DW) {
-    const float* a = alpha + (size_t)dx * 8;
-    const int sx = xofs[dx] - 3;
-    for (int r = threadIdx.y; r <= rowHi - rowLo && r < kLanczosRows; r += blockDim.y) {
-      const float* S = in + (size_t)p * inStride + (size_t)(rowLo + r) * SW;
+    int tap[8];
+#pragma unroll
+    for (int j = 0; j < 8; ++j) {
+      tap[j] = min(max(sx + j, 0), SW - 1) - colLo;
+    }
+    for (int r = threadIdx.y; r < nR; r += blockDim.y) {
+      const float* S = raw + r * nC;
       float v = 0;
 #pragma unroll
       for (int j = 0; j < 8; ++j) {
-        const int sxj = min(max(sx + j, 0), SW - 1);
-        float sv = S[sxj];
-        if (sv != sv) {
-          sv = 1e-4f;
-        }
-        v += sv * a[j];
+        v += S[tap[j]] * a[j];
       }
       rows[r][threadIdx.x] = v;
     }
@@ -2531,17 +2705,21 @@
   if (dx >= DW) {
     return;
   }
-  for (int dy = dy0 + threadIdx.y; dy <= dy1; dy += blockDim.y) {
-    const float* b = beta + (size_t)dy * 8;
-    const int sy = yofs[dy] - 3;
-    float r[8];
-#pragma unroll
-    for (int k = 0; k < 8; ++k) {
-      const int syk = min(max(sy + k, 0), SH - 1);
-      r[k] = rows[min(syk - rowLo, kLanczosRows - 1)][threadIdx.x];
-    }
-    out[(size_t)p * outStride + (size_t)dy * DW + dx] =
-        r[0] * b[0] + r[1] * b[1] + r[2] * b[2] + r[3] * b[3] + r[4] * b[4] + r[5] * b[5] + r[6] * b[6] + r[7] * b[7];
+#pragma unroll
+  for (int t = 0; t < kLanczosH / 4; ++t) {
+    const int ty = (int)threadIdx.y + t * 4, dy = dy0 + ty;
+    if (dy <= dy1) {
+      const float* b = betaT + ty * 8;
+      const int sy = yofsT[ty] - 3;
+      float r[8];
+#pragma unroll
+      for (int k = 0; k < 8; ++k) {
+        const int syk = min(max(sy + k, 0), SH - 1);
+        r[k] = rows[min(syk - rowLo, kLanczosRows - 1)][threadIdx.x];
+      }
+      out[(size_t)p * outStride + (size_t)dy * DW + dx] =
+          r[0] * b[0] + r[1] * b[1] + r[2] * b[2] + r[3] * b[3] + r[4] * b[4] + r[5] * b[5] + r[6] * b[6] + r[7] * b[7];
+    }
   }
 }
 
diff --git a/facebook360_dep_amd/csrc/derp_sequence.h b/facebook360_dep_amd/csrc/derp_sequence.h
--- a/facebook360_dep_amd/csrc/derp_sequence.h
+++ b/facebook360_dep_amd/csrc/derp_sequence.h
@@ -198,6 +198,17 @@
   return 0;
 }
 
+void seq_fg_exposed(derp_seq* q, int frame, int level, int kind) {
+  const int oi = owned_index(q, frame);
+  if (kind == 1 && oi >= 0 && !q->streaming) {
+    q->c->frames[oi].fgFill.written(level);
+  }
+}
+bool seq_fg_all_pass(derp_seq* q, int frame, int level) {
+  const int oi = owned_index(q, frame);
+  return oi >= 0 && !q->streaming && q->c->frames[oi].fgFill.all_pass(level);
+}
+
 #define NCCLCHK(c, api, expr)                                                                    \
   do {                                                                                           \
     ncclResult_t r_ = (expr);                                                                    \
@@ -630,7 +641,9 @@
       return jrc;
     }
   }
-  return seq_buffer(q, frame, level, kind, ptr, bytes);
+  TRY(seq_buffer(q, frame, level, kind, ptr, bytes));
+  seq_fg_exposed(q, frame, level, kind);
+  return 0;
 }
 
 int derp_seq_buffer_copy(derp_seq* q, int frame, int level, int kind, void* host, size_t bytes, int to_device) {
@@ -647,6 +660,9 @@
   HIPCHK(c, hipSetDevice(c->device));
   TRY(seq_join_exchange(q));
   HIPCHK(c, hipStreamSynchronize(c->stream));
+  if (to_device) {
+    seq_fg_exposed(q, frame, level, kind);
+  }
   HIPCHK(c, hipMemcpy(to_device ? p : host, to_device ? host : p, sz, to_device ? hipMemcpyHostToDevice : hipMemcpyDeviceToHost));
   return 0;
 }
@@ -801,6 +817,7 @@
     TRY(upload_color_plane(c, c->frame().color[level], s, h->color + (size_t)s * n * 3, n));
   }
   if (h->fg) {
+    c->frame().fgFill.written(level);
     HIPCHK(c, hipMemcpy(c->frame().fg[level].p, h->fg, n * c->S, hipMemcpyHostToDevice));
   }
   if (forCompute && h->bg) {
@@ -831,6 +848,7 @@
       const derp_seq::HostIn* hu;
       TRY(host_inputs_of(q, k, up, &hu));
       if (hu->fg) {
+        c->frame().fgFill.written(up);
         HIPCHK(c, hipMemcpy(c->frame().fg[up].p, hu->fg, npx(c, up) * c->S, hipMemcpyHostToDevice));
       }
     }
@@ -894,7 +912,10 @@
           pm = p;
         }
       }
-      if (q->opt.use_foreground_masks) {
+      const bool slotAllPass = ku >= 0 && c->frames[ku % q->nSlots].fgFill.all_pass(level);
+      if (q->opt.use_foreground_masks && slotAllPass) {
+        pm = q->fov.p;
+      } else if (q->opt.use_foreground_masks) {
         uint8_t* wm = q->winMask.as<uint8_t>() + (size_t)(u - lo) * n * c->D;
         hipLaunchKernelGGL(k_and_masks, dim3(flat_grid(n), c->D), dim3(256), 0, c->stream, q->fov.as<uint8_t>(),
                            (const uint8_t*)pm, c->dst2src.as<int>(), 0, n, wm);
@@ -950,6 +971,7 @@
     TRY(upload_color_plane(c, c->frame().color[level], s, color_bgr + (size_t)s * n * 3, n));
   }
   if (fg_masks) {
+    c->frame().fgFill.written(level);
     HIPCHK(c, hipMemcpy(c->frame().fg[level].p, fg_masks, n * c->S, hipMemcpyHostToDevice));
   }
   if (background_disparity) {
@@ -1256,7 +1278,9 @@
     size_t b;
     TRY(seq_buffer(q, u, level, 0, &pc, &b));
     TRY(seq_buffer(q, u, level, 2, &pd, &b));
-    if (q->opt.use_foreground_masks) {
+    if (q->opt.use_foreground_masks && seq_fg_all_pass(q, u, level)) {
+      pm = q->fov.p;
+    } else if (q->opt.use_foreground_masks) {
       TRY(seq_buffer(q, u, level, 1, &pm, &b));
       uint8_t* wm = q->winMask.as<uint8_t>() + (size_t)(u - lo) * n * c->D;
       hipLaunchKernelGGL(k_and_masks, dim3(flat_grid(n), c->D), dim3(256), 0, c->stream, q->fov.as<uint8_t>(),
```
